# mateomarin/two_towers

Hardware: AMD Instinct MI355X
Metric: training pairs/sec at global batch=8192, 1/2/4/8 GPUs; MRR@10 match (higher is better)
Workload: dtype bf16; 1 GPU; BASELINE configs[2]: EnhancedTwoTowerModel(300, 256), seq_len 64, batch 8192 per GPU, bf16, hard-negative mining k=5 + margin 0.2, dropout 0.1, Adam; global_batch=8192, seq_len=64, hidden=256, embedding_dim=300, parallelism=dp1, loss=hardneg_margin

## Files before the change

include/tt_hip.h:

```cpp
#ifndef TT_HIP_H
#define TT_HIP_H
#include <stdint.h>

#ifdef __cplusplus
extern "C" {
#endif

#define TT_OK 0
#define TT_EINVAL 1000
#define TT_DT_F32 0
#define TT_DT_BF16 1

const char* tt_version(void);
const char* tt_last_error(void);
int tt_set_option(const char* name, int value);
int tt_get_option(const char* name, int* value);

int tt_embed_gather(int dtype, const void* table, long vocab, int ep, const int32_t* ids, long n,
                    void* out, void* stream);

int tt_pack_rows(int dtype, const float* src, long n, int e, int ep, void* out, void* stream);
typedef struct {
  const float* src;
  const float* src2;
  void* dst;
  int rows, cols, dcols;
  long lds, ldd;
  int dst_bf16;
} tt_pack_job;
int tt_pack_multi(const tt_pack_job* jobs, int njobs, void* stream);

int tt_cast(int dtype, const float* x, long n, void* y, void* stream);

int tt_colsum(const float* x, long rows, int cols, long ld, float* out, int accumulate, void* stream);

typedef struct {
  const void* a[4];
  const void* b[4];
  void* c[4];
  const float* bias[4];
  int bshift[4];
  const void* a_hi[4];
  int a_split;
  uint32_t drop_row0;
} tt_gemm_batch;

int tt_gemm(int dtype, int out_dtype, int a_kouter, int b_kouter, int m, int n, int k,
            const tt_gemm_batch* batch, int nbatch, long lda, long ldb, long ldc, float alpha,
            int beta_accum, int relu, int seq_t, uint32_t drop_seed, float drop_p, int splits,
            float* splitk_ws, void* stream);
int tt_gemm_ct(int dtype, int out_dtype, int a_kouter, int b_kouter, int m, int n, int k,
               const tt_gemm_batch* batch, int nbatch, long lda, long ldb, long ldc, float alpha,
               int beta_accum, int relu, int seq_t, uint32_t drop_seed, float drop_p, int splits,
               float* splitk_ws, int c_trans, void* stream);
long tt_gemm_ws_size(int m, int n, int nbatch, int splits);
int tt_gemm_pick_splits(int m, int n, int k, int nbatch);
int tt_gemm_bres_form(int m, int n, int k, int nbatch, long lda, long ldc);
int tt_gemm_tall_form(int dtype, int out_dtype, int a_kouter, int b_kouter, int m, int n, int k, long lda,
                      long ldb, int splits, int extras);

typedef struct {
  const void* g;
  const void* whh;
  const float* bhn;
  void* y;
  void* x1;
  void* save;
  float* hstate;
  int dir;
  uint32_t drop_seed;
  int drop_col0;
  uint32_t drop_row0;
} tt_gru_fwd_rec;

int tt_gru_fwd(int dtype, const tt_gru_fwd_rec* recs, int nrec, int B, int T, int H, long ldg,
               long ldy, float drop_p, void* ws, long ws_bytes, void* stream);
int tt_gru_fwd_launches(int dtype, int T, int H);
long tt_gru_fwd_ws_size(int dtype, int nrec, int B, int T, int H, long ldg, long ldy);
int tt_gru_fwd_launches_for(int dtype, int nrec, int B, int T, int H, long ldg, long ldy);

typedef struct {
  const void* g; const void* whh; const float* bhn;
  void* y;
  void* hfinal;
  void* scratch;
  int dir;
} tt_gru_infer_rec;
int  tt_gru_fwd_infer(int dtype, const tt_gru_infer_rec* recs, int nrec, int B, int T, int H, long ldg,
                      long ldy, long ldf, void* ws, long ws_bytes, void* stream);
long tt_gru_infer_scratch_size(int dtype, int B, int T, int H, int final_only);

typedef struct {
  const void* save;
  const void* y;
  const void* dy;
  const float* dfinal;
  const void* whh;
  void* dgx;
  void* dgh;
  void* dhstate;
  float* dbias_part;
  int dir;
} tt_gru_bwd_rec;

int tt_gru_bwd(int dtype, const tt_gru_bwd_rec* recs, int nrec, int B, int T, int H, long ldy,
               long ldd, long ldf, void* stream);
int tt_gru_bwd_launches(int dtype, int T, int H);
int tt_gru_bwd_carry_on_chip(int dtype, int T, int H);
int tt_gru_bias_rows(int B);

int tt_gru_yprev_supported(int dtype, int nrec, int B, int T, int H, long ldg, long ldy);
int tt_gru_fwd_yprev(int dtype, const tt_gru_fwd_rec* recs, void* const* hfinal, int nrec, int B, int T, int H,
                     long ldg, long ldy, long ldf, float drop_p, void* ws, long ws_bytes, void* stream);
int tt_gru_bwd_yprev(int dtype, const tt_gru_bwd_rec* recs, int nrec, int B, int T, int H, long ldy,
                     long ldd, long ldf, void* stream);

typedef struct {
  const void* w1; const float* b1; const float* ln_g; const float* ln_b;
  const void* w2; const float* b2;
  const void* x;
  void* p1;
  float* mean;
  float* rstd;
  void* u;
  float* out;
} tt_head_fwd_io;

int tt_proj_head_fwd(int dtype, const tt_head_fwd_io* io, int ntower, int B, int h, float ln_eps,
                     void* stream);

typedef struct {
  const void* w1; const float* ln_g; const float* ln_b; const void* w2;
  const void* x; const void* p1; const float* mean; const float* rstd; const void* u;
  const float* dout;
  float* dx;
  float* dw1; float* db1; float* dg; float* dbeta; float* dw2; float* db2;
  void* ws;
} tt_head_bwd_io;

int tt_proj_head_bwd(int dtype, const tt_head_bwd_io* io, int ntower, int B, int h, float ln_eps,
                     void* stream);
long tt_proj_head_bwd_ws_size(int dtype, int B, int h);

typedef struct {
  const void* x;
  const void* w1; const float* b1; const float* ln_g; const float* ln_b;
  void* p1;
  float* mean;
  float* rstd;
  float* out;
} tt_head1_fwd_io;

int tt_proj_head1_fwd(int dtype, const tt_head1_fwd_io* io, long rows, int C, float ln_eps, float drop_p,
                      uint32_t drop_seed, void* stream);

typedef struct {
  const void* x; const void* w1; const float* ln_g; const float* ln_b;
  const void* p1; const float* mean; const float* rstd;
  const float* dout;
  float* dx;
  float* dw1; float* db1; float* dg; float* dbeta;
  void* ws;
} tt_head1_bwd_io;

int tt_proj_head1_bwd(int dtype, const tt_head1_bwd_io* io, long rows, int C, float drop_p, uint32_t drop_seed,
                      void* stream);
long tt_proj_head1_bwd_ws_size(int dtype, long rows, int C);

int tt_l2norm_fwd(int dtype, const float* x, long rows, int cols, float eps, void* y, float* y32,
                  float* norm, void* stream);
int tt_l2norm_bwd(const float* dy, const float* y32, const float* norm, long rows, int cols,
                  float eps, float* dx, int accumulate, void* stream);

int tt_infonce_fwd(int dtype, const void* qn, long bq, const void* dn, long nd, int h,
                   float inv_tau, float offdiag_sub, long label_offset, float* lse,
                   float* row_loss, void* ws, void* stream);
long tt_infonce_fwd_ws_size(long bq, long nd);
int tt_infonce_bwd(int dtype, const void* qn, long bq, const void* dn, long nd, int h,
                   float inv_tau, float offdiag_sub, long label_offset, const float* lse,
                   const float* gscale, float* dqn, float* ddn, void* ws, void* stream);
long tt_infonce_bwd_ws_size(int dtype, long bq, long nd, int h);

int tt_infonce_sym_fwd(int dtype, const void* qn, const void* dn, long n, int h, float inv_tau,
                       float* lse_row, float* lse_col, float* row_loss, void* ws, void* stream);
long tt_infonce_sym_fwd_ws_size(long n, int h);
int tt_infonce_sym_bwd(int dtype, const void* qn, const void* dn, long n, int h, float inv_tau,
                       const float* lse_row, const float* lse_col, const float* gscale,
                       float* dqn, float* ddn, void* ws, void* stream);
long tt_infonce_sym_bwd_ws_size(int dtype, long n, int h);

int tt_hardneg_topk(int dtype, const void* qn, long bq, const void* dn, long nd, int h,
                    long label_offset, int k, int32_t* idx, float* val, void* ws, void* stream);
long tt_hardneg_ws_size(int dtype, long bq, long nd, int h, int k);

int tt_search_topk(int dtype, const float* qn, long Q, const void* dn, long N, int h, int k,
                   int32_t* idx, float* val, void* ws, void* stream);
long tt_search_ws_size(int dtype, long Q, long N, int h, int k);

int tt_topk_max(void);
int tt_topk_rows(const float* S, long rows, long cols, long ld, long label_offset, int k,
                 int32_t* idx, float* val, void* ws, void* stream);
long tt_topk_rows_ws_size(long rows, long cols, int k);

int tt_margin_fwd(const float* qn, long bq, const float* dn, long nd, int h, long label_offset,
                  const int32_t* idx, int k, float margin, float* row_loss, void* stream);
int tt_margin_bwd(const float* qn, long bq, const float* dn, long nd, int h, long label_offset,
                  const int32_t* idx, int k, float margin, const float* gscale, float* dqn, float* ddn,
                  void* ws, void* stream);
long tt_margin_bwd_ws_size(long bq, long nd, int h, int k);

int tt_sum(const float* x, long n, float scale, float* out, void* stream);

int tt_adam_multi(float* const* params, const float* const* grads, float* const* exp_avg,
                  float* const* exp_avg_sq, const long* sizes, int ntensors, float lr, float beta1,
                  float beta2, float eps, float weight_decay, int step, const int32_t* skip, void* stream);
int tt_adamw_multi(float* const* params, const float* const* grads, float* const* exp_avg,
                   float* const* exp_avg_sq, const long* sizes, int ntensors, float lr, float beta1,
                   float beta2, float eps, float weight_decay, int step, const int32_t* skip, void* stream);

int tt_grad_norm_multi(const float* const* grads, const long* sizes, int ntensors, int accumulate,
                       float* sumsq, void* ws, void* stream);
long tt_grad_norm_ws_size(const long* sizes, int ntensors);
int tt_clip_scale_multi(float* const* grads, const long* sizes, int ntensors, const float* sumsq,
                        float max_norm, float* total_norm_out, void* stream);

#ifdef __cplusplus
}
#endif
#endif
```

two_towers_amd/_lib.py:

```python
from __future__ import annotations

import contextlib
import ctypes
import os
from ctypes import POINTER, c_float, c_int, c_long, c_uint32, c_void_p

import torch

_HERE = os.path.dirname(os.path.abspath(__file__))
LIB_PATH = os.environ.get("TT_HIP_LIB", os.path.join(_HERE, "lib", "libtt_hip.so"))

DT_F32 = 0
DT_BF16 = 1
TT_EINVAL = 1000


class TTError(RuntimeError):
    pass


class GruTimeoutError(TTError):
    """A column-split GRU forward launch gave up waiting for one of its member workgroups
    (tt_gru_fwd's status word): that launch's outputs are invalid."""


class GemmBatch(ctypes.Structure):
    _fields_ = [
        ("a", c_void_p * 4),
        ("b", c_void_p * 4),
        ("c", c_void_p * 4),
        ("bias", c_void_p * 4),
        ("bshift", c_int * 4),
        ("a_hi", c_void_p * 4),
        ("a_split", c_int),
        ("drop_row0", c_uint32),
    ]


class PackJob(ctypes.Structure):
    _fields_ = [
        ("src", c_void_p),
        ("src2", c_void_p),
        ("dst", c_void_p),
        ("rows", c_int),
        ("cols", c_int),
        ("dcols", c_int),
        ("lds", c_long),
        ("ldd", c_long),
        ("dst_bf16", c_int),
    ]


class GruFwdRec(ctypes.Structure):
    _fields_ = [
        ("g", c_void_p), ("whh", c_void_p), ("bhn", c_void_p), ("y", c_void_p), ("x1", c_void_p),
        ("save", c_void_p), ("hstate", c_void_p), ("dir", c_int), ("drop_seed", c_uint32),
        ("drop_col0", c_int), ("drop_row0", c_uint32),
    ]


class GruInferRec(ctypes.Structure):
    _fields_ = [
        ("g", c_void_p), ("whh", c_void_p), ("bhn", c_void_p), ("y", c_void_p), ("hfinal", c_void_p),
        ("scratch", c_void_p), ("dir", c_int),
    ]


class GruBwdRec(ctypes.Structure):
    _fields_ = [
        ("save", c_void_p), ("y", c_void_p), ("dy", c_void_p), ("dfinal", c_void_p), ("whh", c_void_p),
        ("dgx", c_void_p), ("dgh", c_void_p), ("dhstate", c_void_p), ("dbias_part", c_void_p),
        ("dir", c_int),
    ]


class HeadFwdIO(ctypes.Structure):
    _fields_ = [
        ("w1", c_void_p), ("b1", c_void_p), ("ln_g", c_void_p), ("ln_b", c_void_p), ("w2", c_void_p),
        ("b2", c_void_p), ("x", c_void_p), ("p1", c_void_p), ("mean", c_void_p), ("rstd", c_void_p),
        ("u", c_void_p), ("out", c_void_p),
    ]


class HeadBwdIO(ctypes.Structure):
    _fields_ = [
        ("w1", c_void_p), ("ln_g", c_void_p), ("ln_b", c_void_p), ("w2", c_void_p), ("x", c_void_p),
        ("p1", c_void_p), ("mean", c_void_p), ("rstd", c_void_p), ("u", c_void_p), ("dout", c_void_p),
        ("dx", c_void_p), ("dw1", c_void_p), ("db1", c_void_p), ("dg", c_void_p), ("dbeta", c_void_p),
        ("dw2", c_void_p), ("db2", c_void_p), ("ws", c_void_p),
    ]


class Head1FwdIO(ctypes.Structure):
    _fields_ = [
        ("x", c_void_p), ("w1", c_void_p), ("b1", c_void_p), ("ln_g", c_void_p), ("ln_b", c_void_p),
        ("p1", c_void_p), ("mean", c_void_p), ("rstd", c_void_p), ("out", c_void_p),
    ]


class Head1BwdIO(ctypes.Structure):
    _fields_ = [
        ("x", c_void_p), ("w1", c_void_p), ("ln_g", c_void_p), ("ln_b", c_void_p), ("p1", c_void_p),
        ("mean", c_void_p), ("rstd", c_void_p), ("dout", c_void_p), ("dx", c_void_p), ("dw1", c_void_p),
        ("db1", c_void_p), ("dg", c_void_p), ("dbeta", c_void_p), ("ws", c_void_p),
    ]


_SIGS = {
    "tt_version": (ctypes.c_char_p, []),
    "tt_last_error": (ctypes.c_char_p, []),
    "tt_set_option": (c_int, [ctypes.c_char_p, c_int]),
    "tt_get_option": (c_int, [ctypes.c_char_p, POINTER(c_int)]),
    "tt_embed_gather": (c_int, [c_int, c_void_p, c_long, c_int, c_void_p, c_long, c_void_p, c_void_p]),
    "tt_pack_rows": (c_int, [c_int, c_void_p, c_long, c_int, c_int, c_void_p, c_void_p]),
    "tt_pack_multi": (c_int, [c_void_p, c_int, c_void_p]),
    "tt_cast": (c_int, [c_int, c_void_p, c_long, c_void_p, c_void_p]),
    "tt_colsum": (c_int, [c_void_p, c_long, c_int, c_long, c_void_p, c_int, c_void_p]),
    "tt_gemm": (c_int, [c_int, c_int, c_int, c_int, c_int, c_int, c_int, POINTER(GemmBatch), c_int, c_long,
                        c_long, c_long, c_float, c_int, c_int, c_int, c_uint32, c_float, c_int, c_void_p,
                        c_void_p]),
    "tt_gemm_ct": (c_int, [c_int, c_int, c_int, c_int, c_int, c_int, c_int, POINTER(GemmBatch), c_int, c_long,
                           c_long, c_long, c_float, c_int, c_int, c_int, c_uint32, c_float, c_int, c_void_p,
                           c_int, c_void_p]),
    "tt_gemm_ws_size": (c_long, [c_int, c_int, c_int, c_int]),
    "tt_gemm_pick_splits": (c_int, [c_int, c_int, c_int, c_int]),
    "tt_gemm_bres_form": (c_int, [c_int, c_int, c_int, c_int, c_long, c_long]),
    "tt_gemm_tall_form": (c_int, [c_int, c_int, c_int, c_int, c_int, c_int, c_int, c_long, c_long, c_int, c_int]),
    "tt_gru_fwd": (c_int, [c_int, POINTER(GruFwdRec), c_int, c_int, c_int, c_int, c_long, c_long, c_float,
                           c_void_p, c_long, c_void_p]),
    "tt_gru_bwd": (c_int, [c_int, POINTER(GruBwdRec), c_int, c_int, c_int, c_int, c_long, c_long, c_long,
                           c_void_p]),
    "tt_gru_bias_rows": (c_int, [c_int]),
    "tt_gru_bwd_launches": (c_int, [c_int, c_int, c_int]),
    "tt_gru_bwd_carry_on_chip": (c_int, [c_int, c_int, c_int]),
    "tt_gru_fwd_launches": (c_int, [c_int, c_int, c_int]),
    "tt_gru_fwd_ws_size": (c_long, [c_int, c_int, c_int, c_int, c_int, c_long, c_long]),
    "tt_gru_fwd_launches_for": (c_int, [c_int, c_int, c_int, c_int, c_int, c_long, c_long]),
    "tt_gru_fwd_infer": (c_int, [c_int, POINTER(GruInferRec), c_int, c_int, c_int, c_int, c_long, c_long, c_long,
                                 c_void_p, c_long, c_void_p]),
    "tt_gru_infer_scratch_size": (c_long, [c_int, c_int, c_int, c_int, c_int]),
    "tt_gru_yprev_supported": (c_int, [c_int, c_int, c_int, c_int, c_int, c_long, c_long]),
    "tt_gru_fwd_yprev": (c_int, [c_int, POINTER(GruFwdRec), POINTER(c_void_p), c_int, c_int, c_int, c_int, c_long,
                                 c_long, c_long, c_float, c_void_p, c_long, c_void_p]),
    "tt_gru_bwd_yprev": (c_int, [c_int, POINTER(GruBwdRec), c_int, c_int, c_int, c_int, c_long, c_long, c_long,
                                 c_void_p]),
    "tt_proj_head_fwd": (c_int, [c_int, POINTER(HeadFwdIO), c_int, c_int, c_int, c_float, c_void_p]),
    "tt_proj_head_bwd": (c_int, [c_int, POINTER(HeadBwdIO), c_int, c_int, c_int, c_float, c_void_p]),
    "tt_proj_head_bwd_ws_size": (c_long, [c_int, c_int, c_int]),
    "tt_proj_head1_fwd": (c_int, [c_int, POINTER(Head1FwdIO), c_long, c_int, c_float, c_float, c_uint32,
                                  c_void_p]),
    "tt_proj_head1_bwd": (c_int, [c_int, POINTER(Head1BwdIO), c_long, c_int, c_float, c_uint32, c_void_p]),
    "tt_proj_head1_bwd_ws_size": (c_long, [c_int, c_long, c_int]),
    "tt_l2norm_fwd": (c_int, [c_int, c_void_p, c_long, c_int, c_float, c_void_p, c_void_p, c_void_p, c_void_p]),
    "tt_l2norm_bwd": (c_int, [c_void_p, c_void_p, c_void_p, c_long, c_int, c_float, c_void_p, c_int, c_void_p]),
    "tt_infonce_fwd": (c_int, [c_int, c_void_p, c_long, c_void_p, c_long, c_int, c_float, c_float, c_long,
                               c_void_p, c_void_p, c_void_p, c_void_p]),
    "tt_infonce_fwd_ws_size": (c_long, [c_long, c_long]),
    "tt_infonce_bwd": (c_int, [c_int, c_void_p, c_long, c_void_p, c_long, c_int, c_float, c_float, c_long,
                               c_void_p, c_void_p, c_void_p, c_void_p, c_void_p, c_void_p]),
    "tt_infonce_bwd_ws_size": (c_long, [c_int, c_long, c_long, c_int]),
    "tt_infonce_sym_fwd": (c_int, [c_int, c_void_p, c_void_p, c_long, c_int, c_float, c_void_p, c_void_p, c_void_p,
                                   c_void_p, c_void_p]),
    "tt_infonce_sym_fwd_ws_size": (c_long, [c_long, c_int]),
    "tt_infonce_sym_bwd": (c_int, [c_int, c_void_p, c_void_p, c_long, c_int, c_float, c_void_p, c_void_p, c_void_p,
                                   c_void_p, c_void_p, c_void_p, c_void_p]),
    "tt_infonce_sym_bwd_ws_size": (c_long, [c_int, c_long, c_int]),
    "tt_hardneg_topk": (c_int, [c_int, c_void_p, c_long, c_void_p, c_long, c_int, c_long, c_int, c_void_p,
                                c_void_p, c_void_p, c_void_p]),
    "tt_hardneg_ws_size": (c_long, [c_int, c_long, c_long, c_int, c_int]),
    "tt_search_topk": (c_int, [c_int, c_void_p, c_long, c_void_p, c_long, c_int, c_int, c_void_p, c_void_p,
                               c_void_p, c_void_p]),
    "tt_search_ws_size": (c_long, [c_int, c_long, c_long, c_int, c_int]),
    "tt_topk_max": (c_int, []),
    "tt_topk_rows": (c_int, [c_void_p, c_long, c_long, c_long, c_long, c_int, c_void_p, c_void_p, c_void_p,
                             c_void_p]),
    "tt_topk_rows_ws_size": (c_long, [c_long, c_long, c_int]),
    "tt_margin_fwd": (c_int, [c_void_p, c_long, c_void_p, c_long, c_int, c_long, c_void_p, c_int, c_float,
                              c_void_p, c_void_p]),
    "tt_margin_bwd": (c_int, [c_void_p, c_long, c_void_p, c_long, c_int, c_long, c_void_p, c_int, c_float,
                              c_void_p, c_void_p, c_void_p, c_void_p, c_void_p]),
    "tt_margin_bwd_ws_size": (c_long, [c_long, c_long, c_int, c_int]),
    "tt_sum": (c_int, [c_void_p, c_long, c_float, c_void_p, c_void_p]),
    "tt_adam_multi": (c_int, [POINTER(c_void_p), POINTER(c_void_p), POINTER(c_void_p), POINTER(c_void_p),
                              POINTER(c_long), c_int, c_float, c_float, c_float, c_float, c_float, c_int,
                              c_void_p, c_void_p]),
    "tt_adamw_multi": (c_int, [POINTER(c_void_p), POINTER(c_void_p), POINTER(c_void_p), POINTER(c_void_p),
                               POINTER(c_long), c_int, c_float, c_float, c_float, c_float, c_float, c_int,
                               c_void_p, c_void_p]),
    "tt_grad_norm_multi": (c_int, [POINTER(c_void_p), POINTER(c_long), c_int, c_int, c_void_p, c_void_p, c_void_p]),
    "tt_grad_norm_ws_size": (c_long, [POINTER(c_long), c_int]),
    "tt_clip_scale_multi": (c_int, [POINTER(c_void_p), POINTER(c_long), c_int, c_void_p, c_float, c_void_p,
                                    c_void_p]),
}

EXPORTED = tuple(_SIGS)

_lib = None
_load_error: str | None = None


def load():
    global _lib, _load_error
    if _lib is not None:
        return _lib
    if _load_error is not None:
        raise TTError(_load_error)
    if not os.path.exists(LIB_PATH):
        _load_error = (f"two_towers_amd: native library not found at {LIB_PATH}; "
                       "build it with `python -c 'import __graft_entry__ as g; g.build()'` (hipcc, gfx950)")
        raise TTError(_load_error)
    lib = ctypes.CDLL(LIB_PATH, mode=ctypes.RTLD_GLOBAL)
    for name, (res, args) in _SIGS.items():
        fn = getattr(lib, name)
        fn.restype = res
        fn.argtypes = args
    _lib = lib
    return lib


def check(rc: int, what: str = ""):
    if rc != 0:
        msg = _lib.tt_last_error().decode(errors="replace") if _lib is not None else ""
        raise TTError(f"{what or 'tt_hip'} failed (rc={rc}): {msg}")


def call(name: str, *args):
    lib = load()
    check(getattr(lib, name)(*args), name)


_topk_max: int | None = None


def topk_max() -> int:
    global _topk_max
    if _topk_max is None:
        _topk_max = int(load().tt_topk_max())
    return _topk_max


def get_option(name: str) -> int:
    v = c_int(0)
    call("tt_get_option", name.encode(), ctypes.byref(v))
    return v.value


def set_option(name: str, value: int) -> int:
    old = get_option(name)
    call("tt_set_option", name.encode(), int(value))
    return old


@contextlib.contextmanager
def option(name: str, value: int):
    torch.cuda.synchronize()
    old = set_option(name, value)
    try:
        yield
    finally:
        torch.cuda.synchronize()
        set_option(name, old)


def ptr(t: torch.Tensor | None) -> int | None:
    if t is None:
        return None
    return t.data_ptr()


def stream_ptr(device: torch.device | None = None) -> int:
    return torch.cuda.current_stream(device).cuda_stream


def require_gpu(*tensors: torch.Tensor):
    load()
    for t in tensors:
        if t is not None and t.device.type != "cuda":
            raise TTError(
                "two_towers_amd runs only on an AMD GPU (HIP, gfx950); got a tensor on "
                f"'{t.device}'. There is deliberately no CPU fallback: move the model and "
                "inputs to the GPU (`.to('cuda')`).")


def dtype_code(dt: torch.dtype) -> int:
    if dt == torch.float32:
        return DT_F32
    if dt == torch.bfloat16:
        return DT_BF16
    raise TTError(f"unsupported compute dtype {dt}; use torch.float32 or torch.bfloat16")
```

two_towers_amd/csrc/tt_api.h:

```cpp
#pragma once
#include <hip/hip_runtime.h>
#include <stdio.h>
#include <string.h>

#include "../../include/tt_hip.h"

namespace tt {
void set_error(const char* fmt, ...);

enum Opt {
  OPT_GRU_STEP,
  OPT_GRU_DEPTH,
  OPT_GRU_BWD_ROWS,
  OPT_GRU_BWD_BIG,
  OPT_GRU_BWD_STREAMS,
  OPT_GEMM_PERSIST,
  OPT_GEMM_A3,
  OPT_GEMM_REGSTAGE,
  OPT_GEMM_STREAM_OUT,
  OPT_HN_GEMM,
  OPT_GRU_BWD_PERSIST,
  OPT_GRU_FWD_STEP_ROWS,
  OPT_INFONCE_FLASH,
  OPT_HN_MAP,
  OPT_GEMM_SKEW,
  OPT_GEMM_PERSIST_MAXK,
  OPT_GRU_FWD_XC,
  OPT_GRU_XC_SKIP,
  OPT_GRU_XC_SPINS,
  OPT_GRU_BWD_SKEW,
  OPT_GRU_FWD_SKEW,
  OPT_GEMM_BRES,
  OPT_GRU_XC_COOP,
  OPT_GEMM_BUF,
  OPT_GEMM_ORDER,
  OPT_GRU_STEP_RING,
  OPT_GRU_FWD_XS,
  OPT_HN_SCAN_GEMM,
  OPT_GEMM_IEPI,
  OPT_BRES_ROWS,
  OPT_HN_SCAN_V,
  OPT_GEMM_W4,
  OPT_BRES_FORM,
  OPT_WGRAD_TALL,
  OPT_GRU_YPREV,
  OPT_N
};
int opt(Opt o);
int tt_hn_scan_gemm(const void* q, long bq, const void* d, long nd, int h, long label_off, float* cm, long nch,
                    hipStream_t st);
}

#define TT_CHECK_ARG(cond, ...)            \
  do {                                     \
    if (!(cond)) {                         \
      tt::set_error(__VA_ARGS__);          \
      return TT_EINVAL;                    \
    }                                      \
  } while (0)

#define TT_CHECK_LAUNCH(what)                                                        \
  do {                                                                               \
    hipError_t e_ = hipGetLastError();                                               \
    if (e_ != hipSuccess) {                                                          \
      tt::set_error("%s: %s", what, hipGetErrorString(e_));                          \
      return (int)e_;                                                                \
    }                                                                                \
  } while (0)

#define TT_CHECK_HIP(expr)                                                           \
  do {                                                                               \
    hipError_t e_ = (expr);                                                          \
    if (e_ != hipSuccess) {                                                          \
      tt::set_error("%s: %s", #expr, hipGetErrorString(e_));                         \
      return (int)e_;                                                                \
    }                                                                                \
  } while (0)

#define TT_PROPAGATE(expr)     \
  do {                         \
    int rc_ = (expr);          \
    if (rc_ != 0) return rc_;  \
  } while (0)

static inline int tt_ceil_div(long a, long b) { return (int)((a + b - 1) / b); }
```

two_towers_amd/csrc/tt_common.h:

```cpp
#pragma once
#include <hip/hip_runtime.h>
#include <stdint.h>

#define TT_F32 0
#define TT_BF16 1

typedef uint16_t bf16_t;
typedef short bf16x8 __attribute__((ext_vector_type(8)));
typedef short bf16x4 __attribute__((ext_vector_type(4)));
typedef float f32x4 __attribute__((ext_vector_type(4)));

#define TT_DEV __device__ __forceinline__

TT_DEV float bf2f(bf16_t b) { return __uint_as_float(((uint32_t)b) << 16); }
TT_DEV bf16_t f2bf(float f) { __bf16 h = (__bf16)f; return __builtin_bit_cast(bf16_t, h); }

template <typename T> struct Elt;
template <> struct Elt<float> {
  static constexpr int EPC = 4;
  TT_DEV static float ld(const float* p) { return *p; }
  TT_DEV static void st(float* p, float v) { *p = v; }
  TT_DEV static float cvt(float v) { return v; }
};
template <> struct Elt<bf16_t> {
// ... 2 lines not shown
  TT_DEV static void st(bf16_t* p, float v) { *p = f2bf(v); }
  TT_DEV static bf16_t cvt(float v) { return f2bf(v); }
};

TT_DEV void ld8(const float* p, float (&f)[8]) {
  const float4 a = *reinterpret_cast<const float4*>(p), b = *reinterpret_cast<const float4*>(p + 4);
  f[0] = a.x; f[1] = a.y; f[2] = a.z; f[3] = a.w; f[4] = b.x; f[5] = b.y; f[6] = b.z; f[7] = b.w;
}
TT_DEV void ld8(const bf16_t* p, float (&f)[8]) {
  const uint4 u = *reinterpret_cast<const uint4*>(p);
  const uint32_t w[4] = {u.x, u.y, u.z, u.w};
#pragma unroll
  for (int i = 0; i < 4; ++i) {
    f[2 * i] = __uint_as_float(w[i] << 16);
    f[2 * i + 1] = __uint_as_float(w[i] & 0xFFFF0000u);
  }
}
TT_DEV void st8(float* p, const float (&f)[8]) {
  *reinterpret_cast<float4*>(p) = make_float4(f[0], f[1], f[2], f[3]);
  *reinterpret_cast<float4*>(p + 4) = make_float4(f[4], f[5], f[6], f[7]);
}
TT_DEV void st8(bf16_t* p, const float (&f)[8]) {
  uint32_t w[4];
#pragma unroll
  for (int i = 0; i < 4; ++i) w[i] = (uint32_t)f2bf(f[2 * i]) | ((uint32_t)f2bf(f[2 * i + 1]) << 16);
  *reinterpret_cast<uint4*>(p) = make_uint4(w[0], w[1], w[2], w[3]);
}

typedef unsigned tt_u32x4 __attribute__((vector_size(16)));
TT_DEV __amdgpu_buffer_rsrc_t tt_rsrc(const void* base) {
  return __builtin_amdgcn_make_buffer_rsrc(const_cast<void*>(base), (short)0, 0x7fffffff, 0x00020000);
}
TT_DEV uint4 pack8bf(const float (&f)[8]) {
  uint32_t w[4];
#pragma unroll
  for (int i = 0; i < 4; ++i) w[i] = (uint32_t)f2bf(f[2 * i]) | ((uint32_t)f2bf(f[2 * i + 1]) << 16);
  return make_uint4(w[0], w[1], w[2], w[3]);
}
TT_DEV void st16_buf(__amdgpu_buffer_rsrc_t r, uint32_t voff, int soff, uint4 v) {
  tt_u32x4 w = {v.x, v.y, v.z, v.w};
  __builtin_amdgcn_raw_buffer_store_b128(w, r, (int)(voff + (uint32_t)soff), 0, 0);
}
TT_DEV void st16_buf_sc1(__amdgpu_buffer_rsrc_t r, uint32_t voff, int soff, uint4 v) {
  tt_u32x4 w = {v.x, v.y, v.z, v.w};
  __builtin_amdgcn_raw_buffer_store_b128(w, r, (int)(voff + (uint32_t)soff), 0, 16);
}
TT_DEV __amdgpu_buffer_rsrc_t tt_rsrc_n(const void* base, bool on) {
  return __builtin_amdgcn_make_buffer_rsrc(const_cast<void*>(base), (short)0, on ? 0x7fffffff : 0, 0x00020000);
}
template <int AUX = 0>
TT_DEV uint4 ld16_buf(__amdgpu_buffer_rsrc_t r, uint32_t voff, int soff) {
  const tt_u32x4 v = __builtin_amdgcn_raw_buffer_load_b128(r, (int)voff, soff, AUX);
  return make_uint4(v[0], v[1], v[2], v[3]);
}
template <int AUX>
TT_DEV void st16_buf_aux(__amdgpu_buffer_rsrc_t r, int off, uint4 v) {
  tt_u32x4 w = {v.x, v.y, v.z, v.w};
  __builtin_amdgcn_raw_buffer_store_b128(w, r, off, 0, AUX);
}
TT_DEV void st16_sc1(__amdgpu_buffer_rsrc_t r, int off, uint4 v) {
  tt_u32x4 w = {v.x, v.y, v.z, v.w};
  __builtin_amdgcn_raw_buffer_store_b128(w, r, off, 0, 16);
}
TT_DEV void st8_sc1(__amdgpu_buffer_rsrc_t r, int off, const float (&f)[8], float*) {
  st16_sc1(r, off, make_uint4(__float_as_uint(f[0]), __float_as_uint(f[1]), __float_as_uint(f[2]), __float_as_uint(f[3])));
  st16_sc1(r, off + 16, make_uint4(__float_as_uint(f[4]), __float_as_uint(f[5]), __float_as_uint(f[6]), __float_as_uint(f[7])));
}
TT_DEV void st8_sc1(__amdgpu_buffer_rsrc_t r, int off, const float (&f)[8], bf16_t*) {
  uint32_t w[4];
#pragma unroll
  for (int i = 0; i < 4; ++i) w[i] = (uint32_t)f2bf(f[2 * i]) | ((uint32_t)f2bf(f[2 * i + 1]) << 16);
  st16_sc1(r, off, make_uint4(w[0], w[1], w[2], w[3]));
}

TT_DEV uint32_t dpp_ror8(uint32_t x) {
  return (uint32_t)__builtin_amdgcn_mov_dpp((int)x, 0x128 , 0xF, 0xF, false);
}
TT_DEV void row_pair(const uint4& v0, const uint4& v1, uint4& da, uint4& db) {
  const bool lo = (threadIdx.x & 8) == 0;
  uint4 s = lo ? v1 : v0, r;
  r.x = dpp_ror8(s.x);
  r.y = dpp_ror8(s.y);
  r.z = dpp_ror8(s.z);
  r.w = dpp_ror8(s.w);
  da = lo ? v0 : r;
  db = lo ? r : v1;
}

template <typename T>
struct Raw8 {
  uint4 a, b;
  TT_DEV void load(const T* p) {
    a = *reinterpret_cast<const uint4*>(p);
    if constexpr (sizeof(T) == 4) b = *reinterpret_cast<const uint4*>(p + 4);
  }
  TT_DEV void zero() { a = b = make_uint4(0, 0, 0, 0); }
  TT_DEV void get(float (&f)[8]) const {
    if constexpr (sizeof(T) == 4) {
      f[0] = __uint_as_float(a.x); f[1] = __uint_as_float(a.y); f[2] = __uint_as_float(a.z); f[3] = __uint_as_float(a.w);
      f[4] = __uint_as_float(b.x); f[5] = __uint_as_float(b.y); f[6] = __uint_as_float(b.z); f[7] = __uint_as_float(b.w);
    } else {
      const uint32_t w[4] = {a.x, a.y, a.z, a.w};
#pragma unroll
      for (int i = 0; i < 4; ++i) {
        f[2 * i] = __uint_as_float(w[i] << 16);
        f[2 * i + 1] = __uint_as_float(w[i] & 0xFFFF0000u);
      }
    }
  }
};

TT_DEV float tt_rcp(float x) { return __builtin_amdgcn_rcpf(x); }
TT_DEV float tt_sigmoid(float x) { return tt_rcp(1.0f + __expf(-x)); }
TT_DEV float tt_tanh(float x) {
  float e = __expf(2.0f * x);
  return 1.0f - 2.0f * tt_rcp(e + 1.0f);
}

TT_DEV float tt_sech2(float x) {
  const float e = __expf(-2.0f * fabsf(x));
  const float r = tt_rcp(1.0f + e);
  return 4.0f * e * r * r;
}

TT_DEV void tt_sigmoid_pair(float x, float& s, float& sm) {
  const float e = __expf(-fabsf(x));
  const float p = tt_rcp(1.0f + e);
  const float q = e * p;
  s = x >= 0.f ? p : q;
  sm = x >= 0.f ? q : p;
}
TT_DEV void tt_tanh_sech2(float x, float& th, float& sech2) {
  const float e = __expf(-2.0f * fabsf(x));
  const float r = tt_rcp(1.0f + e);
  const float t = (1.0f - e) * r;
  th = x >= 0.f ? t : -t;
  sech2 = 4.0f * e * r * r;
}

TT_DEV uint32_t tt_hash3(uint32_t seed, uint32_t row, uint32_t col) {
  uint32_t h = seed * 0x9E3779B1u ^ (row * 0x85EBCA77u) ^ (col * 0xC2B2AE3Du + 0x27D4EB2Fu);
  h ^= h >> 16; h *= 0x7FEB352Du; h ^= h >> 15; h *= 0x846CA68Bu; h ^= h >> 16;
  return h;
}
TT_DEV float tt_dropout_scale(uint32_t seed, uint32_t row, uint32_t col, uint32_t thresh, float inv_keep) {
  return ((tt_hash3(seed, row, col) >> 8) < thresh) ? 0.0f : inv_keep;
}

TT_DEV float wave_sum(float v) {
#pragma unroll
  for (int o = 32; o > 0; o >>= 1) v += __shfl_xor(v, o, 64);
  return v;
}
TT_DEV float wave_max(float v) {
#pragma unroll
  for (int o = 32; o > 0; o >>= 1) v = fmaxf(v, __shfl_xor(v, o, 64));
  return v;
}
TT_DEV float sum16(float v) {
#pragma unroll
  for (int o = 8; o > 0; o >>= 1) v += __shfl_xor(v, o, 64);
  return v;
}
TT_DEV float max16(float v) {
#pragma unroll
  for (int o = 8; o > 0; o >>= 1) v = fmaxf(v, __shfl_xor(v, o, 64));
  return v;
}
```

two_towers_amd/csrc/tt_elem.hip:

```cpp
#include <algorithm>

#include "tt_api.h"
#include "tt_common.h"

namespace {

__global__ __launch_bounds__(256) void embed_gather_kernel(const uint4* __restrict__ table, long vocab,
                                                           int cpr, const int32_t* __restrict__ ids,
                                                           long n, uint4* __restrict__ out) {
  const long total = n * cpr;
  for (long e = (long)blockIdx.x * 256 + threadIdx.x; e < total; e += (long)gridDim.x * 256) {
    const long row = e / cpr;
    const int c = (int)(e - row * cpr);
    const int id = ids[row];
    uint4 v = make_uint4(0, 0, 0, 0);
    if (id >= 0 && id < vocab) v = table[(long)id * cpr + c];
    out[e] = v;
  }
}

template <typename T>
__global__ __launch_bounds__(256) void pack_rows_kernel(const float* __restrict__ src, long n, int e, int ep,
                                                        T* __restrict__ out) {
  const long total = n * ep;
  for (long i = (long)blockIdx.x * 256 + threadIdx.x; i < total; i += (long)gridDim.x * 256) {
    const long r = i / ep;
    const int c = (int)(i - r * ep);
    Elt<T>::st(out + i, c < e ? src[r * e + c] : 0.f);
  }
}

template <typename T>
__global__ __launch_bounds__(256) void cast_kernel(const float* __restrict__ x, long n, T* __restrict__ y) {
  for (long i = (long)blockIdx.x * 256 + threadIdx.x; i < n; i += (long)gridDim.x * 256) Elt<T>::st(y + i, x[i]);
}

__global__ __launch_bounds__(1024) void colsum_kernel(const float* __restrict__ x, long rows, int cols, long ld,
                                                      int accumulate, float* __restrict__ out) {
  __shared__ float red[16][64];
  const int wave = threadIdx.x >> 6, lane = threadIdx.x & 63;
  const int c = blockIdx.x * 64 + lane;
  float s = 0.f;
  if (c < cols)
    for (long r = wave; r < rows; r += 16) s += x[r * ld + c];
  red[wave][lane] = s;
  __syncthreads();
  if (wave == 0 && c < cols) {
    float t = 0.f;
#pragma unroll
    for (int w = 0; w < 16; ++w) t += red[w][lane];
    out[c] = accumulate ? out[c] + t : t;
  }
}

__global__ __launch_bounds__(256) void sum_kernel(const float* __restrict__ x, long n, float scale,
                                                  float* __restrict__ out) {
  __shared__ float part[4];
  float s = 0.f;
  for (long i = threadIdx.x; i < n; i += 256) s += x[i];
  s = wave_sum(s);
  if ((threadIdx.x & 63) == 0) part[threadIdx.x >> 6] = s;
  __syncthreads();
  if (threadIdx.x == 0) out[0] = scale * (part[0] + part[1] + part[2] + part[3]);
}

struct PackArgs {
  tt_pack_job j[16];
  long start[17];
  int n;
};
__global__ __launch_bounds__(256) void pack_multi_kernel(PackArgs a) {
  const long total = a.start[a.n];
  for (long i = blockIdx.x * 256L + threadIdx.x; i < total; i += (long)gridDim.x * 256) {
    int k = 0;
    while (k + 1 < a.n && i >= a.start[k + 1]) ++k;
    const tt_pack_job& J = a.j[k];
    const long q = i - a.start[k];
    const int g4 = J.dcols / 4;
    const long r = q / g4;
    const int c = (int)(q - r * g4) * 4;
    float4 v = make_float4(0.f, 0.f, 0.f, 0.f);
    if (c < J.cols) {
      v = *reinterpret_cast<const float4*>(J.src + r * J.lds + c);
      if (J.src2) {
        const float4 w = *reinterpret_cast<const float4*>(J.src2 + r * J.lds + c);
        v.x += w.x; v.y += w.y; v.z += w.z; v.w += w.w;
      }
    }
    if (J.dst_bf16) {
      const uint2 o = make_uint2((uint32_t)f2bf(v.x) | ((uint32_t)f2bf(v.y) << 16),
                                 (uint32_t)f2bf(v.z) | ((uint32_t)f2bf(v.w) << 16));
      *reinterpret_cast<uint2*>(static_cast<bf16_t*>(J.dst) + r * J.ldd + c) = o;
    } else {
      *reinterpret_cast<float4*>(static_cast<float*>(J.dst) + r * J.ldd + c) = v;
    }
  }
}

inline unsigned grid_for(long work, int per_block = 256, int cap = 8192) {
  long g = (work + per_block - 1) / per_block;
  if (g < 1) g = 1;
  return (unsigned)std::min<long>(g, cap);
}

}

extern "C" int tt_embed_gather(int dtype, const void* table, long vocab, int ep, const int32_t* ids, long n,
                               void* out, void* stream) {
  TT_CHECK_ARG(dtype == TT_DT_F32 || dtype == TT_DT_BF16, "tt_embed_gather: bad dtype");
  const int esz = dtype == TT_DT_BF16 ? 2 : 4;
  TT_CHECK_ARG((ep * esz) % 16 == 0, "tt_embed_gather: ep*sizeof(dtype) must be a multiple of 16 (ep=%d)", ep);
  if (n == 0) return 0;
  const int cpr = ep * esz / 16;
  hipLaunchKernelGGL(embed_gather_kernel, dim3(grid_for(n * cpr)), dim3(256), 0, (hipStream_t)stream,
                     (const uint4*)table, vocab, cpr, ids, n, (uint4*)out);
  TT_CHECK_LAUNCH("embed_gather_kernel");
  return 0;
}

extern "C" int tt_pack_rows(int dtype, const float* src, long n, int e, int ep, void* out, void* stream) {
  TT_CHECK_ARG(ep >= e, "tt_pack_rows: ep < e");
  if (n == 0) return 0;
  dim3 g(grid_for(n * ep));
  if (dtype == TT_DT_BF16)
    hipLaunchKernelGGL(pack_rows_kernel<bf16_t>, g, dim3(256), 0, (hipStream_t)stream, src, n, e, ep, (bf16_t*)out);
  else
    hipLaunchKernelGGL(pack_rows_kernel<float>, g, dim3(256), 0, (hipStream_t)stream, src, n, e, ep, (float*)out);
  TT_CHECK_LAUNCH("pack_rows_kernel");
  return 0;
}

extern "C" int tt_pack_multi(const tt_pack_job* jobs, int njobs, void* stream) {
  TT_CHECK_ARG(njobs >= 0 && njobs <= 16 && (njobs == 0 || jobs), "tt_pack_multi: njobs %d not in [0,16]", njobs);
  PackArgs a{};
  a.n = njobs;
  a.start[0] = 0;
  for (int k = 0; k < njobs; ++k) {
    const tt_pack_job& J = jobs[k];
    TT_CHECK_ARG(J.src && J.dst && J.rows >= 0 && J.cols >= 0 && J.dcols >= J.cols, "tt_pack_multi: job %d", k);
    TT_CHECK_ARG(J.cols % 4 == 0 && J.dcols % 4 == 0 && J.lds % 4 == 0 && J.ldd % 4 == 0 && J.lds >= J.cols &&
                     J.ldd >= J.dcols,
                 "tt_pack_multi: job %d: cols, dcols and leading dimensions must be multiples of 4", k);
    const bool src_ok = ((uintptr_t)J.src | (uintptr_t)J.src2) % 16 == 0;
    TT_CHECK_ARG(src_ok && (uintptr_t)J.dst % (J.dst_bf16 ? 8 : 16) == 0, "tt_pack_multi: job %d: misaligned operand", k);
    a.j[k] = J;
    a.start[k + 1] = a.start[k] + (long)J.rows * (J.dcols / 4);
  }
  if (a.start[njobs] == 0) return 0;
  hipLaunchKernelGGL(pack_multi_kernel, dim3(grid_for(a.start[njobs], 256, 4096)), dim3(256), 0, (hipStream_t)stream, a);
  TT_CHECK_LAUNCH("pack_multi_kernel");
  return 0;
}

extern "C" int tt_cast(int dtype, const float* x, long n, void* y, void* stream) {
  if (n == 0) return 0;
  dim3 g(grid_for(n));
  if (dtype == TT_DT_BF16)
    hipLaunchKernelGGL(cast_kernel<bf16_t>, g, dim3(256), 0, (hipStream_t)stream, x, n, (bf16_t*)y);
  else
    hipLaunchKernelGGL(cast_kernel<float>, g, dim3(256), 0, (hipStream_t)stream, x, n, (float*)y);
  TT_CHECK_LAUNCH("cast_kernel");
  return 0;
}

extern "C" int tt_colsum(const float* x, long rows, int cols, long ld, float* out, int accumulate, void* stream) {
  hipStream_t st = (hipStream_t)stream;
  if (cols == 0) return 0;
  if (rows == 0) {
    if (!accumulate) TT_CHECK_HIP(hipMemsetAsync(out, 0, sizeof(float) * cols, st));
    return 0;
  }
  hipLaunchKernelGGL(colsum_kernel, dim3(tt_ceil_div(cols, 64)), dim3(1024), 0, st, x, rows, cols, ld, accumulate,
                     out);
  TT_CHECK_LAUNCH("colsum_kernel");
  return 0;
}

extern "C" int tt_sum(const float* x, long n, float scale, float* out, void* stream) {
  hipLaunchKernelGGL(sum_kernel, dim3(1), dim3(256), 0, (hipStream_t)stream, x, n, scale, out);
  TT_CHECK_LAUNCH("sum_kernel");
  return 0;
}
```

two_towers_amd/csrc/tt_gemm.hip:

```cpp
#include <float.h>
#include <stdarg.h>
#include <stdlib.h>

#include <atomic>
#include <type_traits>

#include "tt_api.h"
#include "tt_gemm_core.h"

namespace tt {
static thread_local char g_err[512];
void set_error(const char* fmt, ...) {
  va_list ap;
  va_start(ap, fmt);
  vsnprintf(g_err, sizeof(g_err), fmt, ap);
  va_end(ap);
}
}

namespace tt {
namespace {
struct OptDef {
  const char* name;
  const char* env;
  int dflt;
};
constexpr OptDef kOpts[OPT_N] = {
    {"gru_step", "TT_GRU_STEP", 0},               {"gru_depth", "TT_GRU_DEPTH", 4},
    {"gru_bwd_rows", "TT_GRU_BWD_ROWS", 0},     {"gru_bwd_big", "TT_GRU_BWD_BIG", 1},
    {"gru_bwd_streams", "TT_GRU_BWD_STREAMS", 2}, {"gemm_persist", "TT_GEMM_PERSIST", 1},
    {"gemm_a3", "TT_GEMM_A3", 1},                 {"gemm_regstage", "TT_GEMM_REGSTAGE", 0},
    {"gemm_stream_out", "TT_GEMM_STREAM_OUT", 1}, {"hn_gemm", "TT_HN_GEMM", 0},
    {"gru_bwd_persist", "TT_GRU_BWD_PERSIST", 1}, {"gru_fwd_step_rows", "TT_GRU_FWD_STEP_ROWS", 0},
    {"infonce_flash", "TT_INFONCE_FLASH", 1},     {"hn_map", "TT_HN_MAP", 2},
    {"gemm_skew", "TT_GEMM_SKEW", 0},             {"gemm_persist_maxk", "TT_GEMM_PERSIST_MAXK", 24},
    {"gru_fwd_xc", "TT_GRU_FWD_XC", 1},           {"gru_xc_skip", "TT_GRU_XC_SKIP", 0},
    {"gru_xc_spins", "TT_GRU_XC_SPINS", 22},      {"gru_bwd_skew", "TT_GRU_BWD_SKEW", 14},
    {"gru_fwd_skew", "TT_GRU_FWD_SKEW", 0},       {"gemm_bres", "TT_GEMM_BRES", 1},
    {"gru_xc_coop", "TT_GRU_XC_COOP", 0},         {"gemm_buf", "TT_GEMM_BUF", 1},
    {"gemm_order", "TT_GEMM_ORDER", 0},           {"gru_step_ring", "TT_GRU_STEP_RING", 4},
    {"gru_fwd_xs", "TT_GRU_FWD_XS", 1},           {"hn_scan_gemm", "TT_HN_SCAN_GEMM", 0},
    {"gemm_iepi", "TT_GEMM_IEPI", 1},             {"bres_rows", "TT_BRES_ROWS", 32},
    {"hn_scan_v", "TT_HN_SCAN_V", 5},             {"gemm_w4", "TT_GEMM_W4", 0},
    {"bres_form", "TT_BRES_FORM", 1},             {"wgrad_tall", "TT_WGRAD_TALL", 1},
    {"gru_yprev", "TT_GRU_YPREV", 1},
};
struct OptTable {
  std::atomic<int> v[OPT_N];
  OptTable() {
    for (int i = 0; i < OPT_N; ++i) {
      const char* e = getenv(kOpts[i].env);
      v[i].store(e && *e ? atoi(e) : kOpts[i].dflt, std::memory_order_relaxed);
    }
  }
};
OptTable& opts() {
  static OptTable t;
  return t;
}
int find_opt(const char* name) {
  for (int i = 0; name && i < OPT_N; ++i)
    if (strcmp(name, kOpts[i].name) == 0) return i;
  return -1;
}
}
int opt(Opt o) { return opts().v[o].load(std::memory_order_relaxed); }
}

extern "C" const char* tt_version(void) { return "tt_hip 0.2.0 gfx950"; }
extern "C" const char* tt_last_error(void) { return tt::g_err; }
extern "C" int tt_set_option(const char* name, int value) {
  const int i = tt::find_opt(name);
  TT_CHECK_ARG(i >= 0, "tt_set_option: unknown option '%s'", name ? name : "(null)");
  tt::opts().v[i].store(value, std::memory_order_relaxed);
  return 0;
}
extern "C" int tt_get_option(const char* name, int* value) {
  const int i = tt::find_opt(name);
  TT_CHECK_ARG(i >= 0 && value, "tt_get_option: unknown option '%s'", name ? name : "(null)");
  *value = tt::opt((tt::Opt)i);
  return 0;
}

namespace {

struct GemmArgs {
  const void* a[4];
  const void* b[4];
  void* c[4];
  const float* bias[4];
  int bshift[4];
  const void* a_hi[4];
  int a_split;
  long lda, ldb, ldc;
  int M, N, K;
  int splits, kt_per_split;
  float alpha;
  int beta, relu, seq_t;
  uint32_t drop_seed, drop_thresh, drop_row0;
  float drop_inv_keep;
  long part_stride;
  int vec_ok;
  int force_regstage;
  int skew;
  int bias_vec_ok;
  int stream_out;
  int walk_g, walk_x;
  int nbatch;
  int c_trans;
  float* cm;
  long nch, label_off;
};

constexpr int BM = 128, BN = 128;

#ifndef TT_TAIL_SKIP
#define TT_TAIL_SKIP 1
#endif
using ttg::xcd_remap;
#ifndef PERSIST_IEPI
#define PERSIST_IEPI 1
#endif
#ifndef PERSIST_BAL
#define PERSIST_BAL 1
#endif
#ifndef TT_EPI_PAIR
#define TT_EPI_PAIR 1
#endif
#ifndef TT_GEMM_BAL
#define TT_GEMM_BAL true
#endif

template <typename T, bool AKO, bool BKO, bool SHIFT, typename TO, int TBM, int TBN, int WGM, int WGN, bool DMA,
          bool A3 = false, bool BUF = false>
__global__ __launch_bounds__(64 * WGM * WGN) void gemm_kernel(GemmArgs g) {
  using ML = std::conditional_t<
      DMA,
      std::conditional_t<TBM == 256 && TBN == 256 && WGM == 2 && WGN == 4,
                         ttg::Loop8<T, AKO, BKO, TT_GEMM_BAL, A3, false, BUF>,
                         ttg::DLoop<T, AKO, BKO, TBM, TBN, WGM, WGN>>,
      ttg::MainLoop<T, AKO, BKO, TBM, TBN>>;
  static_assert(DMA || (TBM == 128 && TBN == 128 && WGM == 2 && WGN == 2), "register path is 128x128");
  constexpr int NT = 64 * WGM * WGN;
  constexpr int LDSB = ML::LDS_BYTES > 64 * (TBN + 4) * 4 ? ML::LDS_BYTES : 64 * (TBN + 4) * 4;
  __shared__ __attribute__((aligned(16))) char lds[LDSB];
  const int ntn = (g.N + TBN - 1) / TBN, ntm = (g.M + TBM - 1) / TBM;
  const int id = xcd_remap(blockIdx.x, gridDim.x);
  const int bs = id / (ntm * ntn), tile = id - bs * (ntm * ntn);
  const int mt = tile / ntn, nt = tile - mt * ntn;
  const int bi = bs / g.splits, s = bs - bi * g.splits;
  const int m0 = mt * TBM, n0 = nt * TBN;
  const T* A = static_cast<const T*>(g.a[bi]);
  const T* B = static_cast<const T*>(g.b[bi]);

  f32x4 acc[ML::TM][ML::TN];
#pragma unroll
  for (int i = 0; i < ML::TM; ++i)
#pragma unroll
    for (int j = 0; j < ML::TN; ++j) acc[i][j] = f32x4{0.f, 0.f, 0.f, 0.f};

  const int nk = (g.K * (int)sizeof(T) + ttg::KTB - 1) / ttg::KTB;
  const int kt0 = s * g.kt_per_split;
  const int kt1 = min(nk, kt0 + g.kt_per_split);

  constexpr bool L8T = DMA && TBM == 256 && TBN == 256 && WGM == 2 && WGN == 4;
  const bool mm = !L8T || !TT_TAIL_SKIP || __builtin_amdgcn_readfirstlane((int)(m0 + (int)(threadIdx.x >> 8) * 128 < g.M));
  auto lrun = [&](const auto& la, const auto& lb) {
    if constexpr (L8T) ML::run(la, lb, g.K, kt0, kt1, lds, acc, mm);
    else ML::run(la, lb, g.K, kt0, kt1, lds, acc);
  };
  auto run = [&](const auto& la) {
    if constexpr (!BKO) {
      lrun(la, ttg::KCPlain<T>{B, g.ldb, n0, g.N});
    } else if constexpr (SHIFT) {
      lrun(la, ttg::KOShift<T>{B, g.ldb, n0, g.N - n0, g.seq_t, g.bshift[bi]});
    } else {
      lrun(la, ttg::KOPlain<T>{B, g.ldb, n0, g.N - n0});
    }
  };
  if constexpr (AKO) {
    ttg::KOPlain<T> la{A, g.lda, m0, g.M - m0};
    if (g.a_split > 0) {
      la.base1 = static_cast<const T*>(g.a_hi[bi]);
      la.csplit = g.a_split;
    }
    run(la);
  } else {
    run(ttg::KCPlain<T>{A, g.lda, m0, g.M});
  }

#ifdef TT_DIAG
  if (g.force_regstage == 9) {
    float sum = 0.f;
#pragma unroll
    for (int i = 0; i < ML::TM; ++i)
#pragma unroll
      for (int j = 0; j < ML::TN; ++j) sum += acc[i][j][0] + acc[i][j][3];
    if (sum == 12345.f) static_cast<float*>(g.c[bi])[0] = 1.f;
    return;
  }
#endif
  const bool partial = g.splits > 1;
  TO* C = partial ? nullptr : static_cast<TO*>(g.c[bi]);
  float* P = partial ? static_cast<float*>(g.c[bi]) + (long)s * g.part_stride : nullptr;
  const long ldc = partial ? (long)g.N : g.ldc;
  const float* bias = partial ? nullptr : g.bias[bi];
  const int wave = threadIdx.x >> 6, lane = threadIdx.x & 63, tid = threadIdx.x;
  constexpr int WTM = TBM / WGM, WTN = TBN / WGN;
  const int wm = wave / WGN * WTM, wn = wave % WGN * WTN;
  constexpr int CLD = TBN + 4;
  constexpr int TPR = TBN / 8;
  constexpr int RPP = NT / TPR;
  float* L = reinterpret_cast<float*>(lds);
  const int cg = (tid % TPR) * 8;
  const __amdgpu_buffer_rsrc_t crs = tt_rsrc(partial ? (const void*)P : (const void*)(C + (long)m0 * ldc + n0));
  float bv[8];
#pragma unroll
  for (int e = 0; e < 8; ++e) bv[e] = 0.f;
  if (bias) {
    if (n0 + cg + 8 <= g.N && g.bias_vec_ok) ld8(bias + n0 + cg, bv);
    else
      for (int e = 0; e < 8; ++e)
        if (n0 + cg + e < g.N) bv[e] = bias[n0 + cg + e];
  }
  for (int hf = 0; hf < TBM / 64; ++hf) {
    if (wm <= hf * 64 && hf * 64 < wm + WTM) {
      const int i0 = (hf * 64 - wm) / 16;
#pragma unroll
      for (int i = 0; i < ML::TM; ++i)
        if (i >= i0 && i < i0 + 4)
#pragma unroll
          for (int j = 0; j < ML::TN; ++j)
#pragma unroll
            for (int r = 0; r < 4; ++r)
              L[(16 * (i - i0) + 4 * (lane >> 4) + r) * CLD + wn + 16 * j + (lane & 15)] = acc[i][j][r];
    }
    __syncthreads();
#pragma unroll
    for (int k = 0; k < 64 / RPP; ++k) {
      const int rl = tid / TPR + RPP * k;
      const int gm = m0 + hf * 64 + rl, gn = n0 + cg;
      if (gm < g.M && gn < g.N) {
        float v[8];
#pragma unroll
        for (int e = 0; e < 8; ++e) v[e] = L[rl * CLD + cg + e];
        const bool full = gn + 8 <= g.N && g.vec_ok;
        if (partial) {
          float* dst = P + (long)gm * ldc + gn;
          if (full) st8(dst, v);
          else
            for (int e = 0; e < 8 && gn + e < g.N; ++e) dst[e] = v[e];
        } else {
#pragma unroll
          for (int e = 0; e < 8; ++e) {
            float x = v[e] * g.alpha + bv[e];
            if (g.relu) x = fmaxf(x, 0.f);
            if (g.drop_thresh) x *= tt_dropout_scale(g.drop_seed, g.drop_row0 + (uint32_t)gm, gn + e, g.drop_thresh, g.drop_inv_keep);
            v[e] = x;
          }
          TO* dst = C + (long)gm * ldc + gn;
          if (full) {
            if (g.beta) {
// ... 877 lines not shown
      iepi(C1{}, C1{});
      iepi(C1{}, C0{});
    }
  }
  if constexpr (A3)
    if (!late) __builtin_amdgcn_s_barrier();
  asm volatile("s_waitcnt vmcnt(0)" ::: "memory");
}

namespace tall {
constexpr int AW = 8192, AN = 4096;
constexpr int BOFF = 2 * AW + AN;
constexpr int SLOT = BOFF + 2 * AW;
constexpr int NS = 4;
constexpr int NDMA = SLOT / 1024;
constexpr int KS = 32;
}

template <bool HALF>
__global__ __launch_bounds__(512) void gemm_tall(GemmArgs g, int u0) {
  using namespace tall;
  constexpr int NA = HALF ? 5 : 10;
  __shared__ __attribute__((aligned(16))) char lds[NS * SLOT];
  const int ntn = (g.N + 255) / 256;
  const int id = xcd_remap(blockIdx.x, gridDim.x);
  const int hf = HALF ? id & 1 : 0;
  const int u = u0 + (HALF ? id >> 1 : id);
  const int bs = u / ntn, nt = u - bs * ntn;
  const int bi = bs / g.splits, s = bs - bi * g.splits;
  const int n0 = nt * 256;
  const bf16_t* A = static_cast<const bf16_t*>(g.a[bi]);
  const bf16_t* B = static_cast<const bf16_t*>(g.b[bi]);
  const int wave = __builtin_amdgcn_readfirstlane(threadIdx.x >> 6), lane = threadIdx.x & 63;
  const int wr = wave >> 2, wn = (wave & 3) * 64;
  auto a_sub = [&](int a) { return HALF ? a >> 1 : a / 5; };
  auto a_col = [&](int a) {
    if (HALF) return a == 4 ? 32 * hf + 16 * wr : 64 * hf + 32 * wr + 16 * (a & 1);
    return a % 5 == 4 ? 32 * wr + 16 * (a / 5) : 64 * wr + 16 * (a % 5);
  };

  f32x4 acc[NA][4];
#pragma unroll
  for (int i = 0; i < NA; ++i)
#pragma unroll
    for (int j = 0; j < 4; ++j) acc[i][j] = f32x4{0.f, 0.f, 0.f, 0.f};

  const int nk = (g.K * 2 + ttg::KTB - 1) / ttg::KTB;
  const int kt0 = s * g.kt_per_split;
  const int kt1 = min(nk, kt0 + g.kt_per_split);
  if (kt0 < kt1) {
    const int nst = 2 * (kt1 - kt0);
    const long k0 = (long)kt0 * 64;
    const long krows = min((long)g.K, (long)kt1 * 64) - k0;
    const ttg::tt_rsrc4 ra = ttg::make_rsrc4(A + k0 * g.lda, (uint32_t)(((krows - 1) * g.lda + g.M) * 2));
    const ttg::tt_rsrc4 rb = ttg::make_rsrc4(B + k0 * g.ldb, (uint32_t)(((krows - 1) * g.ldb + g.N) * 2));
    const uint32_t da = (uint32_t)(KS * g.lda * 2), db = (uint32_t)(KS * g.ldb * 2);
    uint32_t voff[5];
#pragma unroll
    for (int t = 0; t < 5; ++t) {
      const int j = wave + 8 * t;
      long e;
      if (j < 16) {
        const int p = (j & 7) * 64 + lane, kl = p >> 4, c = (p & 15) ^ (ttg::ko_v(kl) << 1);
        e = (long)kl * g.lda + (j >> 3) * 128 + c * 8;
      } else if (j < 20) {
        const int p = (j - 16) * 64 + lane, kl = p >> 3, c = (p & 7) ^ (ttg::kon_v(kl) << 1);
        e = (long)kl * g.lda + 256 + c * 8;
      } else {
        const int b = j - 20, p = (b & 7) * 64 + lane, kl = p >> 4, c = (p & 15) ^ (ttg::ko_v(kl) << 1);
        e = (long)kl * g.ldb + n0 + (b >> 3) * 128 + c * 8;
      }
      voff[t] = (uint32_t)(e * 2);
    }
    const uint32_t base = __builtin_amdgcn_readfirstlane(ttg::lds_addr_of(lds));
    const bool a2 = wave < 4;
    ttg::tt_rsrc4 r2;
    r2.x = a2 ? ra.x : rb.x;
    r2.y = a2 ? ra.y : rb.y;
    r2.z = a2 ? ra.z : rb.z;
    r2.w = ra.w;
    const uint32_t d2 = a2 ? da : db;
    auto issue = [&](int st) {
      const uint32_t sl = base + (uint32_t)(st & (NS - 1)) * SLOT + (uint32_t)wave * 1024u;
      const uint32_t sa = (uint32_t)st * da, sb = (uint32_t)st * db;
      ttg::dma16_buf(ra, voff[0] + sa, 0u, sl);
      ttg::dma16_buf(ra, voff[1] + sa, 0u, sl + 8 * 1024u);
      ttg::dma16_buf(r2, voff[2] + (uint32_t)st * d2, 0u, sl + 16 * 1024u);
      ttg::dma16_buf(rb, voff[3] + sb, 0u, sl + 24 * 1024u);
      if (a2) ttg::dma16_buf(rb, voff[4] + sb, 0u, sl + 32 * 1024u);
    };
    auto step = [&](const char* sl) {
      uint4 fb[4];
#pragma unroll
      for (int j = 0; j < 4; ++j) fb[j] = ttg::frag<bf16_t, true>(sl + BOFF + (wn >> 7) * AW, (wn & 127) + 16 * j, 0);
#pragma unroll
      for (int h = 0; h < NA / 5; ++h) {
        uint4 fa[5];
#pragma unroll
        for (int i = 0; i < 4; ++i) fa[i] = ttg::frag<bf16_t, true>(sl + a_sub(5 * h + i) * AW, a_col(5 * h + i), 0);
        fa[4] = ttg::frag_ko16n(sl + 2 * AW, a_col(5 * h + 4));
#pragma unroll
        for (int i = 0; i < 5; ++i)
#pragma unroll
          for (int j = 0; j < 4; ++j) acc[5 * h + i][j] = ttg::mma<bf16_t>(fb[j], fa[i], acc[5 * h + i][j]);
        __builtin_amdgcn_sched_barrier(0);
      }
    };
    issue(0);
    issue(1);
    issue(2);
    for (int st = 0; st < nst; ++st) {
      if (wave < 4) asm volatile("s_waitcnt vmcnt(10)" ::: "memory");
      else asm volatile("s_waitcnt vmcnt(8)" ::: "memory");
      __builtin_amdgcn_s_barrier();
      issue(st + 3);
      const char* sl = lds + (st & (NS - 1)) * SLOT;
      step(sl);
    }
    asm volatile("s_waitcnt vmcnt(0)" ::: "memory");
  }

  const bool partial = g.splits > 1;
  float* C = partial ? static_cast<float*>(g.c[bi]) + (long)s * g.part_stride : static_cast<float*>(g.c[bi]);
  const long ldc = partial ? (long)g.N : g.ldc;
  const int q = lane >> 4, lr = lane & 15;
#pragma unroll
  for (int i = 0; i < NA; ++i) {
    const int gm = (i % 5 < 4 ? 128 * a_sub(i) : 256) + a_col(i) + lr;
#pragma unroll
    for (int j = 0; j < 4; ++j) {
      const int c = n0 + wn + 16 * j + 4 * q;
      if (gm >= g.M || c >= g.N) continue;
      float v[4];
#pragma unroll
      for (int e = 0; e < 4; ++e) v[e] = partial ? acc[i][j][e] : acc[i][j][e] * g.alpha + 0.f;
      float* dst = C + (long)gm * ldc + c;
      if (c + 4 <= g.N && g.vec_ok) *reinterpret_cast<float4*>(dst) = make_float4(v[0], v[1], v[2], v[3]);
      else
        for (int e = 0; e < 4 && c + e < g.N; ++e) dst[e] = v[e];
    }
  }
}

template <typename TO, int V>
__global__ __launch_bounds__(256) void splitk_reduce_kernel(const float* ws, long part_stride, int splits,
                                                            int M, int N, GemmArgs g) {
  const int bi = blockIdx.y;
  const float* P = ws + (long)bi * splits * part_stride;
  TO* C = static_cast<TO*>(g.c[bi]);
  const float* bias = g.bias[bi];
  const long total = (long)M * N / V;
  for (long e = (long)blockIdx.x * 256 + threadIdx.x; e < total; e += (long)gridDim.x * 256) {
    float v[V];
    if constexpr (V == 4) {
      float4 a = make_float4(0.f, 0.f, 0.f, 0.f);
      for (int s = 0; s < splits; ++s) {
        const float4 b = reinterpret_cast<const float4*>(P + (long)s * part_stride)[e];
        a.x += b.x;
        a.y += b.y;
        a.z += b.z;
        a.w += b.w;
      }
      v[0] = a.x, v[1] = a.y, v[2] = a.z, v[3] = a.w;
    } else {
      v[0] = 0.f;
      for (int s = 0; s < splits; ++s) v[0] += P[(long)s * part_stride + e];
    }
    const int m = (int)(e * V / N), n0 = (int)(e * V % N);
#pragma unroll
    for (int u = 0; u < V; ++u) {
      float x = v[u] * g.alpha;
      if (bias) x += bias[n0 + u];
      TO* p = g.c_trans ? C + (long)(n0 + u) * g.ldc + m : C + (long)m * g.ldc + n0 + u;
      if (g.beta) x += Elt<TO>::ld(p);
      Elt<TO>::st(p, x);
    }
  }
}

template <typename T, typename TO, int TBM, int TBN, int WGM, int WGN, bool DMA, bool A3 = false, bool BUF = false>
int launch_t(int akout, int bkout, bool shift, const GemmArgs& g, long nwg, hipStream_t st) {
  dim3 grid((unsigned)nwg), blk(64 * WGM * WGN);
#define TT_L(AK, BK, SH) \
  hipLaunchKernelGGL((gemm_kernel<T, AK, BK, SH, TO, TBM, TBN, WGM, WGN, DMA, A3, BUF>), grid, blk, 0, st, g)
  if (!akout && !bkout) TT_L(false, false, false);
  else if (!akout && bkout && !shift) TT_L(false, true, false);
  else if (!akout && bkout && shift) TT_L(false, true, true);
  else if (akout && !bkout) TT_L(true, false, false);
  else if (akout && bkout && !shift) TT_L(true, true, false);
  else TT_L(true, true, true);
#undef TT_L
  TT_CHECK_LAUNCH("gemm_kernel");
  return 0;
}

inline bool use_big(int m, int n, long tiles256) { return m >= 256 && n >= 256 && tiles256 >= 256; }

template <typename T, typename TO>
int launch_persist(int akout, int bkout, bool shift, const GemmArgs& g0, int ntiles, bool buf, hipStream_t st) {
  dim3 grid((unsigned)std::min(ntiles, 256)), blk(512);
  GemmArgs g = g0;
  g.walk_g = g.walk_x = 0;
  if (tt::opt(tt::OPT_GEMM_ORDER) && ntiles % 256 == 0 && ((g.N + 255) / 256) % 4 == 0) {
    g.walk_g = 4;
    g.walk_x = 8;
  }
#define TT_L(AK, BK, SH, A3, BUF) \
  hipLaunchKernelGGL((gemm_persist<T, AK, BK, SH, TO, A3, BUF>), grid, blk, 0, st, g, ntiles)
#define TT_L2(AK, BK, SH) \
  do {                     \
    if (a3 && buf) TT_L(AK, BK, SH, true, true); \
    else if (a3) TT_L(AK, BK, SH, true, false); \
    else TT_L(AK, BK, SH, false, false);   \
  } while (0)
  const bool a3 = tt::opt(tt::OPT_GEMM_A3) != 0;
  if constexpr (std::is_same<TO, bf16_t>::value) {
    if (PERSIST_IEPI && tt::opt(tt::OPT_GEMM_IEPI) && !akout && !bkout && !shift && a3 && buf && g.M % 256 == 0 &&
        g.N % 256 == 0 && g.vec_ok && g.bias_vec_ok && g.alpha == 1.f && !g.relu && !g.drop_thresh && !g.beta &&
        g.stream_out <= 2 && g.force_regstage == 0) {
      hipLaunchKernelGGL((gemm_persist<T, false, false, false, TO, true, true, false, true>), grid, blk, 0, st, g, ntiles);
      TT_CHECK_LAUNCH("gemm_persist");
      return 0;
    }
  }
  if (!akout && !bkout) TT_L2(false, false, false);
  else if (!akout && bkout && !shift) TT_L2(false, true, false);
  else if (!akout && bkout && shift) TT_L2(false, true, true);
  else if (akout && !bkout) TT_L2(true, false, false);
  else if (akout && bkout && !shift) TT_L2(true, true, false);
  else TT_L2(true, true, true);
#undef TT_L2
#undef TT_L
  TT_CHECK_LAUNCH("gemm_persist");
  return 0;
}

#ifndef W4_LEAD
#define W4_LEAD 2
#endif
namespace w4 {
constexpr int SLOT = 32768;
constexpr int NS = 4;
struct Frags {
  uint4 a[8], b[8];
};
TT_DEV uint4 frag(const char* img, int r0) {
  const int lane = threadIdx.x & 63;
  const int row = r0 + (lane & 15);
  return *reinterpret_cast<const uint4*>(img + row * 64 + (((lane >> 4) ^ ((row >> 1) & 3)) << 4));
}
}

template <bool RS>
__global__ __launch_bounds__(256, 1) void gemm_w4(GemmArgs g, int ntm, int ntn) {
  constexpr int NSL = RS ? 3 : w4::NS;
  __shared__ __attribute__((aligned(16))) char lds[NSL * w4::SLOT];
  const int id = ttg::xcd_remap(blockIdx.x, gridDim.x);
  const int per = ntm * ntn;
  const int bi = id / per, tile = id - bi * per;
  const int mt = tile / ntn, nt = tile - mt * ntn;
  const int m0 = mt * 256, n0 = nt * 256;
  const int wave = __builtin_amdgcn_readfirstlane(threadIdx.x >> 6), lane = threadIdx.x & 63;
  const int wr = wave >> 1, wc = wave & 1;
  const bf16_t* A = static_cast<const bf16_t*>(g.a[bi]);
  const bf16_t* B = static_cast<const bf16_t*>(g.b[bi]);
  const uint32_t base = __builtin_amdgcn_readfirstlane(ttg::lds_addr_of(lds));
  const bool isA = wave < 2;
  const long ld = isA ? g.lda : g.ldb;
  const long r0 = isA ? m0 : n0;
  const long rows_left = (isA ? g.M : g.N) - r0;
  const long nrec = rows_left * ld * 2;
  const uint32_t nrec32 = (uint32_t)(nrec > 0xFFFFFFFFL ? 0xFFFFFFFFL : nrec);
  const ttg::tt_rsrc4 rs = ttg::make_rsrc4((isA ? A : B) + r0 * ld, nrec32);
  const __amdgpu_buffer_rsrc_t rsb = __builtin_amdgcn_make_buffer_rsrc(
      const_cast<bf16_t*>((isA ? A : B) + r0 * ld), (short)0, (int)(nrec32 > 0x7fffffffu ? 0x7fffffffu : nrec32), 0x00020000);
  const int prow = 16 * (wave & 1) * 8 + (lane >> 2);
  const uint32_t voff = (uint32_t)(prow * ld * 2 + (((lane & 3) ^ ((lane >> 3) & 3)) << 4));
  const uint32_t pstep = (uint32_t)(16 * ld * 2);
  const uint32_t pbase = (uint32_t)wave * 8u * 1024u;
  auto dma = [&](int kt, int j) {
    ttg::dma16_buf(rs, voff, (uint32_t)kt * 64u + (uint32_t)j * pstep,
                   base + (uint32_t)(kt % NSL) * w4::SLOT + pbase + (uint32_t)j * 1024u);
  };
  auto gload = [&](int kt, int j) { return ld16_buf(rsb, voff, (int)((uint32_t)kt * 64u + (uint32_t)j * pstep)); };
  auto lput = [&](int kt, int j, const uint4& v) {
    *reinterpret_cast<uint4*>(lds + (kt % NSL) * w4::SLOT + pbase + j * 1024 + lane * 16) = v;
  };
  const int nk = g.K / 32;
  f32x4 acc[8][8];
#pragma unroll
  for (int i = 0; i < 8; ++i)
#pragma unroll
    for (int j = 0; j < 8; ++j) acc[i][j] = f32x4{0.f, 0.f, 0.f, 0.f};
  if constexpr (RS) {
    uint4 S0[8], S1[8];
#pragma unroll
    for (int j = 0; j < 8; ++j) S0[j] = gload(0, j);
#pragma unroll
    for (int j = 0; j < 8; ++j) S1[j] = gload(1, j);
#pragma unroll
    for (int j = 0; j < 8; ++j) lput(0, j, S0[j]);
#pragma unroll
    for (int j = 0; j < 8; ++j) lput(1, j, S1[j]);
#pragma unroll
    for (int j = 0; j < 8; ++j) S0[j] = gload(2, j);
    __syncthreads();
// ... 52 lines not shown
      for (int i = 0; i < 8; ++i) {
        Fn.a[i] = w4::frag(img, wr * 128 + 16 * i);
        Fn.b[i] = w4::frag(img + 16384, wc * 128 + 16 * i);
        dma(kt + W4_LEAD + 1, i);
#pragma unroll
        for (int j = 0; j < 8; ++j) acc[i][j] = ttg::mma<bf16_t>(Fc.b[j], Fc.a[i], acc[i][j]);
        __builtin_amdgcn_sched_barrier(0);
      }
    };
    for (int kt = 0; kt < nk; kt += 2) {
      step(F0, F1, kt);
      step(F1, F0, kt + 1);
    }
    asm volatile("s_waitcnt vmcnt(0)" ::: "memory");
  }
  bf16_t* C = static_cast<bf16_t*>(g.c[bi]);
  const float* bias = g.bias[bi];
  const int q = lane >> 4, lr = lane & 15;
  const __amdgpu_buffer_rsrc_t crs = tt_rsrc(C + (long)m0 * g.ldc + n0);
#pragma unroll
  for (int jp = 0; jp < 4; ++jp) {
    float bv[2][4];
#pragma unroll
    for (int h = 0; h < 2; ++h) {
      const float4 b4 = bias ? *reinterpret_cast<const float4*>(bias + n0 + wc * 128 + 16 * (2 * jp + h) + 4 * q)
                             : make_float4(0.f, 0.f, 0.f, 0.f);
      bv[h][0] = b4.x; bv[h][1] = b4.y; bv[h][2] = b4.z; bv[h][3] = b4.w;
    }
    const int cs = wc * 128 + 16 * (2 * jp + (q & 1)) + 8 * (q >> 1);
#pragma unroll
    for (int i = 0; i < 8; ++i) {
      uint32_t w[2][2];
#pragma unroll
      for (int h = 0; h < 2; ++h) {
        const f32x4 a = acc[i][2 * jp + h];
        w[h][0] = (uint32_t)f2bf(a[0] + bv[h][0]) | ((uint32_t)f2bf(a[1] + bv[h][1]) << 16);
        w[h][1] = (uint32_t)f2bf(a[2] + bv[h][2]) | ((uint32_t)f2bf(a[3] + bv[h][3]) << 16);
      }
      const auto s0 = __builtin_amdgcn_permlane16_swap(w[0][0], w[1][0], false, false);
      const auto s1 = __builtin_amdgcn_permlane16_swap(w[0][1], w[1][1], false, false);
      const uint4 v = make_uint4(s0[0], s1[0], s0[1], s1[1]);
      const int off = (int)(((long)(wr * 128 + 16 * i + lr) * g.ldc + cs) * 2L);
      if (g.stream_out) st16_sc1(crs, off, v);
      else st16_buf(crs, (uint32_t)off, 0, v);
    }
  }
}

int bres_form_for(int M, int N, int K, int nbatch, long lda, long ldc) {
  if (tt::opt(tt::OPT_GEMM_BRES) == 0 || K % 32 || K < 32 || K > 384 || (lda * 2) % 16) return 0;
  if ((long)M * lda * 2 >= (1L << 31)) return 0;
  constexpr int nwg = 256;
  if (tt::opt(tt::OPT_BRES_FORM) == 1 && tt::opt(tt::OPT_BRES_ROWS) != 64 && N % WR_COLS == 0 && K <= 32 * WR_MAXKS) {
    const int ptot = N / WR_COLS * nbatch;
    if (ptot <= nwg) {
      const int ngrp = nwg / ptot;
      const long mg = ((long)(M + ngrp - 1) / ngrp + WR_TR - 1) / WR_TR * WR_TR;
      if ((long)M >= (long)ngrp * (WR_TR / 4) && (mg * ldc + N) * 2 < (1L << 31)) return 2;
    }
  }
  if (N % BR_COLS) return 0;
  const int ptot = N / BR_COLS * nbatch;
  if (ptot > nwg || nwg % ptot) return 0;
  if ((long)M < (long)(nwg / ptot) * 256) return 0;
  return 1;
}

template <typename T, typename TO>
bool try_bres(int akout, int bkout, bool shift, const GemmArgs& g, int nbatch, hipStream_t st, int* rc) {
  *rc = 0;
  if constexpr (!std::is_same<T, bf16_t>::value || !std::is_same<TO, bf16_t>::value) {
    return false;
  } else {
    if (akout || bkout || shift || g.splits != 1 || g.beta || g.relu || g.drop_thresh || g.alpha != 1.f ||
        g.force_regstage || !g.vec_ok)
      return false;
    for (int b = 0; b < nbatch; ++b)
      if (g.bias[b] && (uintptr_t)g.bias[b] % 16) return false;
    const int form = bres_form_for(g.M, g.N, g.K, nbatch, g.lda, g.ldc);
    if (form == 0) return false;
    const bool r64 = tt::opt(tt::OPT_BRES_ROWS) == 64;
    const int npan = g.N / (form == 2 ? WR_COLS : BR_COLS);
    const int nwg = form == 2 ? npan * nbatch * (256 / (npan * nbatch)) : 256;
    const dim3 grid(nwg), blk(form == 1 && r64 ? 256 : 512);
    switch (g.K / 32) {
#define TT_BR(n)                                                                   \
  case n:                                                                          \
    if (r64)                                                                       \
      hipLaunchKernelGGL((gemm_bres<n, 4>), grid, blk, 0, st, g, npan, nbatch);    \
    else                                                                           \
      hipLaunchKernelGGL((gemm_bres<n, 2>), grid, blk, 0, st, g, npan, nbatch);    \
    break;
#define TT_WR(n)                                                                   \
  case n:                                                                          \
    if (form == 2)                                                                 \
      hipLaunchKernelGGL((gemm_wreg<n>), grid, blk, 0, st, g, npan, nbatch);       \
    else if (r64)                                                                  \
      hipLaunchKernelGGL((gemm_bres<n, 4>), grid, blk, 0, st, g, npan, nbatch);    \
    else                                                                           \
      hipLaunchKernelGGL((gemm_bres<n, 2>), grid, blk, 0, st, g, npan, nbatch);    \
    break;
      TT_WR(1) TT_WR(2) TT_WR(3) TT_WR(4) TT_WR(5) TT_WR(6) TT_WR(7) TT_WR(8) TT_WR(9) TT_WR(10) TT_BR(11) TT_BR(12)
#undef TT_WR
#undef TT_BR
      default: return false;
    }
    const hipError_t e = hipGetLastError();
    if (e != hipSuccess) {
      tt::set_error("%s: %s", form == 2 ? "gemm_wreg" : "gemm_bres", hipGetErrorString(e));
      *rc = (int)e;
    }
    return true;
  }
}

bool tall_form_for(bool bf16_in, bool f32_out, int akout, int bkout, bool plain, int M, int N, long lda, long ldb,
                   int kt_per_split) {
  if (tt::opt(tt::OPT_WGRAD_TALL) == 0 || !bf16_in || !f32_out || !akout || !bkout || !plain) return false;
  if (M <= 256 || M > 320 || M % 8 || N % 8 || N <= 0) return false;
  if (tt::opt(tt::OPT_GEMM_REGSTAGE) != 0) return false;
  const long span = ((long)kt_per_split * 64 + 4 * tall::KS) * 2;
  return span * lda < (1L << 32) && span * ldb < (1L << 32);
}
bool gemm_args_plain(const GemmArgs& g, bool shift, int nbatch) {
  if (shift || g.a_split > 0 || g.beta || g.relu || g.drop_thresh) return false;
  for (int b = 0; b < nbatch; ++b)
    if (g.bias[b]) return false;
  return true;
}

template <typename T, typename TO>
int launch_gemm(int akout, int bkout, bool shift, GemmArgs& g, int nbatch, hipStream_t st) {
  constexpr int EPC = 16 / (int)sizeof(T);
  {
    int rc = 0;
    if (try_bres<T, TO>(akout, bkout, shift, g, nbatch, st, &rc)) return rc;
  }
  if (tall_form_for(std::is_same<T, bf16_t>::value, std::is_same<TO, float>::value, akout, bkout,
                    gemm_args_plain(g, shift, nbatch), g.M, g.N, g.lda, g.ldb, g.kt_per_split)) {
    const long units = (long)tt_ceil_div(g.N, 256) * nbatch * g.splits;
    const int mode = tt::opt(tt::OPT_WGRAD_TALL);
    long nfull = units;
    if (mode == 3) nfull = 0;
    else if (mode != 2 && units % 256 > 0 && units % 256 <= 128) nfull = units - units % 256;
    if (nfull > 0) hipLaunchKernelGGL(gemm_tall<false>, dim3((unsigned)nfull), dim3(512), 0, st, g, 0);
    if (units > nfull)
      hipLaunchKernelGGL(gemm_tall<true>, dim3((unsigned)(2 * (units - nfull))), dim3(512), 0, st, g, (int)nfull);
    TT_CHECK_LAUNCH("gemm_tall");
    return 0;
  }
  const bool dma = (akout ? g.M % EPC == 0 : g.K % EPC == 0) && (bkout ? g.N % EPC == 0 : g.K % EPC == 0) &&
                   g.force_regstage != 1;
  const long t256 = (long)tt_ceil_div(g.M, 256) * tt_ceil_div(g.N, 256) * nbatch * g.splits;
  const bool persist_ok = tt::opt(tt::OPT_GEMM_PERSIST) != 0;
  const int nk = (g.K * (int)sizeof(T) + ttg::KTB - 1) / ttg::KTB;
  bool buf = tt::opt(tt::OPT_GEMM_BUF) != 0 && g.K % (ttg::KTB / (int)sizeof(T)) == 0;
  {
    const long span = (long)(g.kt_per_split + 2) * (ttg::KTB / (int)sizeof(T)) * (long)sizeof(T);
    if (akout && span * g.lda >= (1L << 32)) buf = false;
    if (bkout && span * g.ldb >= (1L << 32)) buf = false;
    if (shift && g.seq_t % (ttg::KTB / (int)sizeof(T)) != 0) buf = false;
    if (!akout && (long)256 * g.lda * (long)sizeof(T) >= (1L << 31)) buf = false;
    if (!bkout && (long)256 * g.ldb * (long)sizeof(T) >= (1L << 31)) buf = false;
    for (int b = 0; b < 4 && g.a_split > 0; ++b) {
      if (!g.a[b]) continue;
      const long d = (long)((const char*)g.a_hi[b] - (const char*)g.a[b]) / (long)sizeof(T);
      if (d < 0 || d + (g.M - g.a_split) > g.lda) buf = false;
    }
  }
  if constexpr (std::is_same<T, bf16_t>::value && std::is_same<TO, bf16_t>::value) {
    if (tt::opt(tt::OPT_GEMM_W4) && !akout && !bkout && !shift && g.splits == 1 && !g.beta && !g.relu &&
        !g.drop_thresh && g.alpha == 1.f && g.force_regstage == 0 && g.M % 256 == 0 && g.N % 256 == 0 && g.K % 64 == 0 &&
        g.K >= 32 && g.vec_ok && g.bias_vec_ok && (g.lda * 2) % 16 == 0 && (g.ldb * 2) % 16 == 0 &&
        256L * g.lda * 2 < (1L << 31) && 256L * g.ldb * 2 < (1L << 31) && 256L * g.ldc * 2 < (1L << 31)) {
      const int ntm = g.M / 256, ntn = g.N / 256;
      if (tt::opt(tt::OPT_GEMM_W4) == 2)
        hipLaunchKernelGGL(gemm_w4<true>, dim3((unsigned)(ntm * ntn * nbatch)), dim3(256), 0, st, g, ntm, ntn);
      else
        hipLaunchKernelGGL(gemm_w4<false>, dim3((unsigned)(ntm * ntn * nbatch)), dim3(256), 0, st, g, ntm, ntn);
      TT_CHECK_LAUNCH("gemm_w4");
      return 0;
    }
  }
  if (dma && persist_ok && !shift && (g.force_regstage == 0 || g.force_regstage >= 9) && g.splits == 1 && !g.beta && nk >= 2 && nk <= tt::opt(tt::OPT_GEMM_PERSIST_MAXK) && t256 >= 512 &&
      use_big(g.M, g.N, t256))
    return launch_persist<T, TO>(akout, bkout, shift, g, (int)t256, buf, st);
  if (dma && g.force_regstage != 2 && use_big(g.M, g.N, t256)) {
    if (tt::opt(tt::OPT_GEMM_A3) && buf)
      return launch_t<T, TO, 256, 256, 2, 4, true, true, true>(akout, bkout, shift, g, t256, st);
    if (tt::opt(tt::OPT_GEMM_A3)) return launch_t<T, TO, 256, 256, 2, 4, true, true>(akout, bkout, shift, g, t256, st);
    return launch_t<T, TO, 256, 256, 2, 4, true>(akout, bkout, shift, g, t256, st);
  }
  const long t128 = (long)tt_ceil_div(g.M, 128) * tt_ceil_div(g.N, 128) * nbatch * g.splits;
  if (dma) return launch_t<T, TO, 128, 128, 2, 2, true>(akout, bkout, shift, g, t128, st);
  return launch_t<T, TO, 128, 128, 2, 2, false>(akout, bkout, shift, g, t128, st);
}

}

int tt::tt_hn_scan_gemm(const void* q, long bq, const void* d, long nd, int h, long label_off, float* cm, long nch,
                    hipStream_t st) {
  TT_CHECK_ARG(h % 64 == 0 && h <= 1024 && bq > 0 && nd > 0 && bq < (1L << 31) && nd < (1L << 31),
               "tt_hn_scan_gemm: h %d, bq %ld, nd %ld", h, bq, nd);
  GemmArgs g{};
  g.a[0] = q;
  g.b[0] = d;
  g.lda = g.ldb = h;
  g.M = (int)bq;
  g.N = (int)nd;
  g.K = h;
  g.alpha = 1.f;
  g.splits = 1;
  g.kt_per_split = h / 64;
  g.nbatch = 1;
  g.cm = cm;
  g.nch = nch;
  g.label_off = label_off;
  const long ntm = (bq + 255) / 256, ntn = (nd + 255) / 256, ntiles = ntm * ntn;
  TT_CHECK_ARG(ntiles < (1L << 31), "tt_hn_scan_gemm: too many tiles");
  if (ntiles % 256 == 0 && ntn % 4 == 0) {
    g.walk_g = 4;
    g.walk_x = 8;
  }
  hipLaunchKernelGGL((gemm_persist<bf16_t, false, false, false, float, true, true, true>),
                     dim3((unsigned)std::min<long>(ntiles, 256)), dim3(512), 0, st, g, (int)ntiles);
  TT_CHECK_LAUNCH("gemm_persist (hard-negative scan)");
  return 0;
}

extern "C" int tt_gemm_bres_form(int m, int n, int k, int nbatch, long lda, long ldc) {
  return bres_form_for(m, n, k, nbatch, lda, ldc);
}

static void split_plan(int k, int esz, int* splits, int* kt_per_split) {
  const int nk = tt_ceil_div((long)k * esz, 128);
  int s = *splits < 1 ? 1 : *splits;
  if (s > nk) s = nk > 0 ? nk : 1;
  *kt_per_split = nk > 0 ? tt_ceil_div(nk, s) : 1;
  *splits = nk > 0 ? tt_ceil_div(nk, *kt_per_split) : 1;
}

extern "C" int tt_gemm_tall_form(int dtype, int out_dtype, int a_kouter, int b_kouter, int m, int n, int k, long lda,
                                 long ldb, int splits, int extras) {
  int ktps = 1;
  split_plan(k, dtype == TT_DT_BF16 ? 2 : 4, &splits, &ktps);
  return tall_form_for(dtype == TT_DT_BF16, out_dtype == TT_DT_F32, a_kouter, b_kouter, extras == 0, m, n, lda, ldb, ktps)
             ? 1
             : 0;
}

extern "C" long tt_gemm_ws_size(int m, int n, int nbatch, int splits) {
  (void)m;
  return splits > 1 ? (long)m * n * nbatch * splits : 0;
}

extern "C" int tt_gemm_pick_splits(int m, int n, int k, int nbatch) {
  const bool big = m >= 256 && n >= 256;
  const long tiles = big ? (long)tt_ceil_div(m, 256) * tt_ceil_div(n, 256) * nbatch
                         : (long)tt_ceil_div(m, BM) * tt_ceil_div(n, BN) * nbatch;
  const long target = big ? 512 : 1024;
  if (tiles >= target) return 1;
  const int smax = std::max(1, std::min(64, tt_ceil_div(k, 64) / 8));
  int best = 1;
  double best_eff = 0.0;
  const int s_lo = (int)std::min<long>(smax, std::max<long>(1, target / tiles));
  for (int s = s_lo; s <= std::min<long>(smax, 3 * target / tiles + 1); ++s) {
    const long w = tiles * s;
    const double eff = (double)w / (256.0 * (double)tt_ceil_div(w, 256));
    if (eff > best_eff + 1e-9) { best_eff = eff; best = s; }
  }
  return std::min(best, smax);
}

extern "C" int tt_gemm(int dtype, int out_dtype, int a_kouter, int b_kouter, int m, int n, int k,
                       const tt_gemm_batch* batch, int nbatch, long lda, long ldb, long ldc,
                       float alpha, int beta_accum, int relu, int seq_t, uint32_t drop_seed,
                       float drop_p, int splits, float* splitk_ws, void* stream) {
  return tt_gemm_ct(dtype, out_dtype, a_kouter, b_kouter, m, n, k, batch, nbatch, lda, ldb, ldc, alpha, beta_accum, relu,
                    seq_t, drop_seed, drop_p, splits, splitk_ws, 0, stream);
}

extern "C" int tt_gemm_ct(int dtype, int out_dtype, int a_kouter, int b_kouter, int m, int n, int k,
                          const tt_gemm_batch* batch, int nbatch, long lda, long ldb, long ldc,
                          float alpha, int beta_accum, int relu, int seq_t, uint32_t drop_seed,
                          float drop_p, int splits, float* splitk_ws, int c_trans, void* stream) {
  TT_CHECK_ARG(dtype == TT_DT_F32 || dtype == TT_DT_BF16, "tt_gemm: bad dtype %d", dtype);
  TT_CHECK_ARG(out_dtype == TT_DT_F32 || out_dtype == dtype, "tt_gemm: bad out_dtype %d", out_dtype);
  TT_CHECK_ARG(nbatch >= 1 && nbatch <= 4, "tt_gemm: nbatch %d not in [1,4]", nbatch);
  TT_CHECK_ARG(m >= 0 && n >= 0 && k >= 0, "tt_gemm: negative dims");
  if (m == 0 || n == 0) return 0;
  const int esz = dtype == TT_DT_BF16 ? 2 : 4;
  const int epc = 16 / esz;
  (void)epc;
  TT_CHECK_ARG((lda * esz) % 16 == 0 && (ldb * esz) % 16 == 0,
               "tt_gemm: leading dimensions must be 16-byte multiples (lda=%ld ldb=%ld)", lda, ldb);
  if (splits < 1) splits = 1;
  TT_CHECK_ARG(splits == 1 || (relu == 0 && drop_p == 0.f), "tt_gemm: split-K excludes relu/dropout");
  TT_CHECK_ARG(splits == 1 || splitk_ws != nullptr, "tt_gemm: split-K needs a workspace");
  TT_CHECK_ARG(drop_p >= 0.f && drop_p < 1.f, "tt_gemm: drop_p %f", drop_p);
  bool shift = false;
  GemmArgs g{};
  for (int b = 0; b < nbatch; ++b) {
    TT_CHECK_ARG(batch->a[b] && batch->b[b] && batch->c[b], "tt_gemm: null operand in batch %d", b);
    TT_CHECK_ARG(((uintptr_t)batch->a[b] | (uintptr_t)batch->b[b]) % 16 == 0,
                 "tt_gemm: operands must be 16-byte aligned (batch %d)", b);
    g.a[b] = batch->a[b];
    g.b[b] = batch->b[b];
    g.c[b] = batch->c[b];
    g.bias[b] = batch->bias[b];
    g.bshift[b] = batch->bshift[b];
    g.a_hi[b] = batch->a_hi[b];
    if (batch->a_split > 0)
      TT_CHECK_ARG(batch->a_hi[b] && (uintptr_t)batch->a_hi[b] % 16 == 0, "tt_gemm: a_hi[%d] null or misaligned", b);
    if (batch->bshift[b] != 0) shift = true;
  }
  TT_CHECK_ARG(!shift || (b_kouter && seq_t > 0), "tt_gemm: bshift needs b_kouter and seq_t");
  TT_CHECK_ARG(batch->a_split >= 0 && (batch->a_split == 0 || (a_kouter && batch->a_split % (16 / esz) == 0)),
               "tt_gemm: a_split %d needs a_kouter and a 16-byte multiple", batch->a_split);
  g.a_split = batch->a_split;
  g.lda = lda; g.ldb = ldb; g.ldc = ldc;
  g.M = m; g.N = n; g.K = k;
  g.alpha = alpha; g.beta = beta_accum; g.relu = relu; g.seq_t = seq_t;
  g.force_regstage = tt::opt(tt::OPT_GEMM_REGSTAGE);
  g.nbatch = nbatch;
  g.skew = tt::opt(tt::OPT_GEMM_SKEW);
  g.drop_seed = drop_seed;
  g.drop_row0 = batch->drop_row0;
  g.drop_thresh = drop_p > 0.f ? (uint32_t)(drop_p * 16777216.0f + 0.5f) : 0u;
  g.drop_inv_keep = drop_p > 0.f ? 1.0f / (1.0f - drop_p) : 1.0f;
  split_plan(k, esz, &splits, &g.kt_per_split);
  g.splits = splits;
  TT_CHECK_ARG(!c_trans || splits > 1, "tt_gemm_ct: a transposed C needs split-K (splits %d)", splits);
  g.c_trans = c_trans != 0;
  {
    const int osz = out_dtype == TT_DT_BF16 ? 2 : 4;
    bool ok = (ldc * osz) % 16 == 0;
    for (int b = 0; b < nbatch; ++b) ok = ok && ((uintptr_t)batch->c[b] % 16 == 0);
    g.vec_ok = ok;
    bool bok = true;
    for (int b = 0; b < nbatch; ++b) bok = bok && ((uintptr_t)batch->bias[b] % 16 == 0);
    g.bias_vec_ok = bok;
    g.stream_out = ok && (long)m * n * osz >= (64L << 20) && (long)256 * ldc * osz < (1L << 31);
    g.stream_out = g.stream_out ? tt::opt(tt::OPT_GEMM_STREAM_OUT) : 0;
  }
  hipStream_t st = static_cast<hipStream_t>(stream);
  TT_CHECK_ARG((long)tt_ceil_div(m, 128) * tt_ceil_div(n, 128) * nbatch * splits < (1L << 31), "tt_gemm: too many tiles");

  if (splits > 1) {
    GemmArgs gp = g;
    gp.part_stride = (long)m * n;
    gp.vec_ok = (n % 4 == 0);
    for (int b = 0; b < nbatch; ++b) gp.c[b] = splitk_ws + (long)b * splits * gp.part_stride;
    int rc = dtype == TT_DT_BF16 ? launch_gemm<bf16_t, float>(a_kouter, b_kouter, shift, gp, nbatch, st)
                                 : launch_gemm<float, float>(a_kouter, b_kouter, shift, gp, nbatch, st);
    if (rc) return rc;
    const bool v4 = n % 4 == 0 && (uintptr_t)splitk_ws % 16 == 0;
    const long total = (long)m * n / (v4 ? 4 : 1);
    dim3 rg((unsigned)std::min<long>(tt_ceil_div(total, 256), 2048), nbatch);
#define TT_RED(TO, V) hipLaunchKernelGGL((splitk_reduce_kernel<TO, V>), rg, dim3(256), 0, st, splitk_ws, gp.part_stride, splits, m, n, g)
    if (out_dtype == TT_DT_F32) {
      if (v4) TT_RED(float, 4); else TT_RED(float, 1);
    } else {
      if (v4) TT_RED(bf16_t, 4); else TT_RED(bf16_t, 1);
    }
#undef TT_RED
    TT_CHECK_LAUNCH("splitk_reduce_kernel");
    return 0;
  }
  if (dtype == TT_DT_BF16) {
    return out_dtype == TT_DT_BF16 ? launch_gemm<bf16_t, bf16_t>(a_kouter, b_kouter, shift, g, nbatch, st)
                                   : launch_gemm<bf16_t, float>(a_kouter, b_kouter, shift, g, nbatch, st);
  }
  return launch_gemm<float, float>(a_kouter, b_kouter, shift, g, nbatch, st);
}
```

two_towers_amd/csrc/tt_gru.hip:

```cpp
#include <algorithm>
#include <cstdlib>
#include <mutex>
#include <type_traits>

#include "tt_api.h"
#include "tt_gemm_core.h"

namespace {

struct FwdRec {
  const void* g; const void* whh; const float* bhn; void* y; void* x1; void* save; float* hs;
  int dir; uint32_t seed; int col0;
  uint32_t row0;
};
struct FwdArgs {
  FwdRec r[4];
  int B, T, H;
  long ldg, ldy;
  int s;
  uint32_t drop_thresh;
  float inv_keep;
#ifdef TT_DIAG
  int dbg;
#endif
// ... 2210 lines not shown
  a.inv_keep = drop_p > 0.f ? 1.0f / (1.0f - drop_p) : 1.0f;
#ifdef TT_DIAG
  if (const char* e = getenv("TT_GRU_DBG")) a.dbg = atoi(e);
#endif
  hipStream_t st = (hipStream_t)stream;
  if (dtype == TT_DT_BF16) {
    bool used = false;
    TT_PROPAGATE(gru_fwd_xc_launch(a, nrec, B, T, H, ldg, ldy, ws, ws_bytes, st, &used));
    if (used) return 0;
  }
  if (gru_fwd_persistent(dtype, H)) return launch_fwd_seq(a, nrec, B, H, st);
  return launch_fwd_steps(dtype, a, nrec, B, T, H, ldg, ldy, st);
}

namespace {
struct YpZeroArgs {
  void* y[4];
  int dir[4];
  int B, T, H;
  long ldy;
};
__global__ __launch_bounds__(256) void gru_yprev_zero_rows(YpZeroArgs a) {
  const int per = a.H / 8;
  const long i = (long)blockIdx.x * 256 + threadIdx.x;
  if (i >= (long)a.B * per) return;
  const int rz = blockIdx.y;
  const long b = i / per;
  const int j = (int)(i - b * per) * 8;
  const int t = a.dir[rz] ? a.T - 1 : 0;
  *reinterpret_cast<uint4*>(static_cast<bf16_t*>(a.y[rz]) + (b * a.T + t) * a.ldy + j) = make_uint4(0u, 0u, 0u, 0u);
}
}

extern "C" int tt_gru_yprev_supported(int dtype, int nrec, int B, int T, int H, long ldg, long ldy) {
  if (!gru_bwd_persistent(dtype, H) || H > 512) return 0;
  XcGeo g;
  bool ok = false;
  if (xc_plan(dtype, nrec, B, T, H, ldg, ldy, true, g, &ok, false, true) != 0 || !ok) return 0;
  return 1;
}

extern "C" int tt_gru_fwd_yprev(int dtype, const tt_gru_fwd_rec* recs, void* const* hfinal, int nrec, int B, int T,
                                int H, long ldg, long ldy, long ldf, float drop_p, void* ws, long ws_bytes,
                                void* stream) {
  TT_CHECK_ARG(dtype == TT_DT_BF16, "tt_gru_fwd_yprev: bf16 only (tt_gru_yprev_supported)");
  TT_CHECK_ARG(nrec >= 1 && nrec <= 4, "tt_gru_fwd_yprev: nrec %d", nrec);
  TT_CHECK_ARG(B > 0 && T > 0 && (H == 256 || H == 512), "tt_gru_fwd_yprev: bad shape (H 256 or 512)");
  TT_CHECK_ARG(ws != nullptr && ws_bytes > 0, "tt_gru_fwd_yprev: needs the tt_gru_fwd_ws_size workspace");
  TT_CHECK_ARG((ldy * 2) % 16 == 0 && ldy >= H, "tt_gru_fwd_yprev: ldy=%ld misaligned or below H", ldy);
  TT_CHECK_ARG(drop_p >= 0.f && drop_p < 1.f, "tt_gru_fwd_yprev: drop_p");
  TT_CHECK_ARG(128L * T * std::max({4L * H, ldy, ldg}) * 2 < (1L << 31), "tt_gru_fwd_yprev: tile byte offsets exceed 2 GiB");
  TT_CHECK_ARG(!hfinal || (ldf >= H && (ldf * 2) % 16 == 0 && 256L * ldf * 2 < (1L << 31)),
               "tt_gru_fwd_yprev: ldf=%ld misaligned or below H", ldf);
  YpArgs a{};
  YpZeroArgs z{};
  for (int i = 0; i < nrec; ++i) {
    const tt_gru_fwd_rec& r = recs[i];
    TT_CHECK_ARG(r.g && r.whh && r.bhn && r.y && r.save, "tt_gru_fwd_yprev: null pointer in rec %d", i);
    TT_CHECK_ARG(((uintptr_t)r.y & 15) == 0, "tt_gru_fwd_yprev: y of rec %d is not 16-byte aligned", i);
    TT_CHECK_ARG(!hfinal || (hfinal[i] && ((uintptr_t)hfinal[i] & 15) == 0),
                 "tt_gru_fwd_yprev: hfinal[%d] null or not 16-byte aligned", i);
    a.r[i] = FwdRec{r.g, r.whh, r.bhn, r.y, r.x1, r.save, r.hstate, r.dir, r.drop_seed, r.drop_col0, r.drop_row0};
    a.hfin[i] = hfinal ? hfinal[i] : nullptr;
    z.y[i] = r.y;
    z.dir[i] = r.dir;
  }
  a.B = B; a.T = T; a.H = H; a.ldg = ldg; a.ldy = ldy; a.ldf = hfinal ? ldf : 0;
  a.drop_thresh = drop_p > 0.f ? (uint32_t)(drop_p * 16777216.0f + 0.5f) : 0u;
  a.inv_keep = drop_p > 0.f ? 1.0f / (1.0f - drop_p) : 1.0f;
  z.B = B; z.T = T; z.H = H; z.ldy = ldy;
  hipStream_t st = (hipStream_t)stream;
  bool used = false;
  TT_PROPAGATE(gru_fwd_xc_launch(a, nrec, B, T, H, ldg, ldy, ws, ws_bytes, st, &used));
  TT_CHECK_ARG(used, "tt_gru_fwd_yprev: the column-split forward does not apply to this call (tt_gru_yprev_supported)");
  hipLaunchKernelGGL(gru_yprev_zero_rows, dim3((unsigned)tt_ceil_div((long)B * (H / 8), 256), (unsigned)nrec), dim3(256), 0,
                     st, z);
  TT_CHECK_LAUNCH("gru_yprev_zero_rows");
  return 0;
}

extern "C" long tt_gru_infer_scratch_size(int dtype, int B, int T, int H, int final_only) {
  if ((dtype != TT_DT_F32 && dtype != TT_DT_BF16) || B <= 0 || T <= 0 || H <= 0) return 0;
  if (gru_fwd_persistent(dtype, H)) return 0;
  const long esz = dtype == TT_DT_BF16 ? 2 : 4;
  return 2L * B * H * 4 + (final_only ? 2L * B * H * esz : 0);
}

extern "C" int tt_gru_fwd_infer(int dtype, const tt_gru_infer_rec* recs, int nrec, int B, int T, int H, long ldg,
                                long ldy, long ldf, void* ws, long ws_bytes, void* stream) {
  TT_CHECK_ARG(dtype == TT_DT_F32 || dtype == TT_DT_BF16, "tt_gru_fwd_infer: bad dtype");
  TT_CHECK_ARG(nrec >= 1 && nrec <= 4, "tt_gru_fwd_infer: nrec %d", nrec);
  TT_CHECK_ARG(B > 0 && T > 0 && H > 0, "tt_gru_fwd_infer: bad shape");
  TT_CHECK_ARG(ws_bytes >= 0 && (ws != nullptr || ws_bytes == 0), "tt_gru_fwd_infer: ws / ws_bytes");
  const int esz = dtype == TT_DT_BF16 ? 2 : 4;
  TT_CHECK_ARG(H % 8 == 0 && (ldy * esz) % 16 == 0, "tt_gru_fwd_infer: H=%d (multiple of 8)/ldy=%ld misaligned", H, ldy);
  TT_CHECK_ARG(tt_ceil_div(B, 128) <= 65535, "tt_gru_fwd_infer: B too large");
  TT_CHECK_ARG(128L * T * std::max({4L * H, ldy, ldg}) * esz < (1L << 31),
               "tt_gru_fwd_infer: tile byte offsets exceed 2 GiB");
  const bool has_y = recs[0].y != nullptr, has_f = recs[0].hfinal != nullptr;
  TT_CHECK_ARG(has_y || has_f, "tt_gru_fwd_infer: neither y nor hfinal given");
  TT_CHECK_ARG(!has_f || (ldf >= H && (ldf * esz) % 16 == 0 && 256L * ldf * esz < (1L << 31)),
               "tt_gru_fwd_infer: ldf=%ld misaligned or below H", ldf);
  const bool persistent = gru_fwd_persistent(dtype, H);
  const long state = 2L * B * H * 4;
  InfArgs a{};
  for (int i = 0; i < nrec; ++i) {
    const tt_gru_infer_rec& r = recs[i];
    TT_CHECK_ARG(r.g && r.whh && r.bhn, "tt_gru_fwd_infer: null pointer in rec %d", i);
    TT_CHECK_ARG((r.y != nullptr) == has_y && (r.hfinal != nullptr) == has_f,
                 "tt_gru_fwd_infer: rec %d disagrees with rec 0 on y / hfinal", i);
    TT_CHECK_ARG(persistent || (r.scratch && ((uintptr_t)r.scratch & 15) == 0),
                 "tt_gru_fwd_infer: rec %d needs 16-byte aligned scratch (tt_gru_infer_scratch_size)", i);
    a.r[i] = FwdRec{r.g, r.whh, r.bhn, r.y, nullptr, nullptr, static_cast<float*>(r.scratch), r.dir, 0u, 0, 0u};
    for (int k = nrec; k < 4; ++k) a.hfin[k] = a.himg[k] = nullptr;
    a.hfin[i] = r.hfinal;
    a.himg[i] = r.scratch && !has_y ? static_cast<char*>(r.scratch) + state : nullptr;
  }
  a.B = B; a.T = T; a.H = H; a.ldg = ldg; a.ldy = ldy; a.ldf = ldf;
  a.inv_keep = 1.0f;
  hipStream_t st = (hipStream_t)stream;
  if (dtype == TT_DT_BF16) {
    bool used = false;
    TT_PROPAGATE(gru_fwd_xc_launch(a, nrec, B, T, H, ldg, ldy, ws, ws_bytes, st, &used));
    if (used) return 0;
  }
  if (persistent) return launch_fwd_seq(a, nrec, B, H, st);
  return launch_fwd_steps(dtype, a, nrec, B, T, H, ldg, ldy, st);
}

template <typename T, int BMR>
static void launch_bwd_step(int ring, dim3 grid, hipStream_t st, const BwdArgs& a) {
  if (ring >= 4) hipLaunchKernelGGL((gru_bwd_step<T, BMR, 4>), grid, dim3(256), 0, st, a);
  else if (ring == 3) hipLaunchKernelGGL((gru_bwd_step<T, BMR, 3>), grid, dim3(256), 0, st, a);
  else hipLaunchKernelGGL((gru_bwd_step<T, BMR>), grid, dim3(256), 0, st, a);
}

static int gru_bwd_impl(int dtype, const tt_gru_bwd_rec* recs, int nrec, int B, int T, int H, long ldy, long ldd,
                        long ldf, void* stream, int yprev) {
  TT_CHECK_ARG(dtype == TT_DT_F32 || dtype == TT_DT_BF16, "tt_gru_bwd: bad dtype");
  TT_CHECK_ARG(nrec >= 1 && nrec <= 4, "tt_gru_bwd: nrec %d", nrec);
  TT_CHECK_ARG(B > 0 && T > 0 && H > 0, "tt_gru_bwd: bad shape");
  const int esz = dtype == TT_DT_BF16 ? 2 : 4;
  TT_CHECK_ARG(H % 8 == 0 && (ldd * esz) % 16 == 0, "tt_gru_bwd: H=%d (multiple of 8)/ldd=%ld misaligned", H, ldd);
  TT_CHECK_ARG(256L * T * std::max({ldd, ldy, 4L * H}) * esz < (1L << 31), "tt_gru_bwd: tile byte offsets exceed 2 GiB");
  TT_CHECK_ARG(!yprev || (gru_bwd_persistent(dtype, H) && H <= 512),
               "tt_gru_bwd_yprev: the row-owning backward does not apply to this call (tt_gru_yprev_supported)");
  hipStream_t st = (hipStream_t)stream;
  BwdArgs a{};
  for (int i = 0; i < nrec; ++i) {
    const tt_gru_bwd_rec& r = recs[i];
    TT_CHECK_ARG(r.save && r.y && r.whh && r.dgx && r.dgh && r.dhstate && r.dbias_part,
                 "tt_gru_bwd: null pointer in rec %d", i);
    a.r[i] = BwdRec{r.save, r.y, r.dy, r.dfinal, r.whh, r.dgx, r.dgh, r.dhstate, r.dbias_part, r.dir};
    TT_CHECK_HIP(hipMemsetAsync(r.dbias_part, 0, sizeof(float) * 4L * H * tt_gru_bias_rows(B), st));
  }
  a.B = B; a.T = T; a.H = H; a.ldy = ldy; a.ldd = ldd; a.ldf = ldf;
  a.skew = tt::opt(tt::OPT_GRU_BWD_SKEW);
  a.yprev = yprev;
#ifdef TT_DIAG
  if (const char* e = getenv("TT_GRU_DBG")) a.dbg = atoi(e);
#endif
  const int bmr = bwd_rows(B, H, nrec);
  if (gru_bwd_persistent(dtype, H)) {
    TT_CHECK_ARG(128L * T * std::max({ldd, ldy, 4L * H}) * esz < (1L << 31), "tt_gru_bwd: tile offsets exceed 2 GiB");
    const dim3 grid(tt_ceil_div(B, 128) * nrec);
    if (H == 1024) hipLaunchKernelGGL(gru_bwd_rows<1024>, grid, dim3(512), 0, st, a);
    else if (H == 512) hipLaunchKernelGGL(gru_bwd_rows<512>, grid, dim3(512), 0, st, a);
    else hipLaunchKernelGGL(gru_bwd_rows<256>, grid, dim3(512), 0, st, a);
    TT_CHECK_LAUNCH("gru_bwd_rows");
    return 0;
  }
  if (dtype == TT_DT_BF16 && H % 256 == 0 && bmr == 128 && tt::opt(tt::OPT_GRU_BWD_BIG) != 0) {
    const dim3 grid((H / 256) * tt_ceil_div(B, 256) * nrec);
    for (int s = T - 1; s >= 0; --s) {
      a.s = s;
      hipLaunchKernelGGL(gru_bwd_big, grid, dim3(512), 0, st, a);
      TT_CHECK_LAUNCH("gru_bwd_big");
    }
    return 0;
  }
  const int ngrp = (nrec >= 2 && tt::opt(tt::OPT_GRU_BWD_STREAMS) != 1) ? 2 : 1;
  BwdArgs ga[2] = {a, a};
  int gn[2] = {nrec, 0};
  if (ngrp == 2) {
    gn[0] = nrec / 2;
    gn[1] = nrec - gn[0];
    for (int i = 0; i < gn[1]; ++i) ga[1].r[i] = a.r[gn[0] + i];
  }
  hipStream_t gs[2] = {st, st};
  SideStream* side = nullptr;
  if (ngrp == 2) {
    TT_PROPAGATE(side_stream(&side));
    gs[1] = side->s;
    TT_CHECK_HIP(hipEventRecord(side->fork, st));
    TT_CHECK_HIP(hipStreamWaitEvent(side->s, side->fork, 0));
  }
  XcDev* xd = nullptr;
  TT_PROPAGATE(xc_device(&xd));
  long wgs = 0;
  for (int g = 0; g < ngrp; ++g) wgs += (long)tt_ceil_div(H, 128) * tt_ceil_div(B, bmr) * gn[g];
  const int ring = wgs <= xd->cus ? tt::opt(tt::OPT_GRU_STEP_RING) : 2;
  for (int s = T - 1; s >= 0; --s) {
    for (int g = 0; g < ngrp; ++g) {
      ga[g].s = s;
      const dim3 grid(tt_ceil_div(H, 128) * tt_ceil_div(B, bmr) * gn[g]);
      if (dtype == TT_DT_BF16) {
        if (bmr == 64) launch_bwd_step<bf16_t, 64>(ring, grid, gs[g], ga[g]);
        else launch_bwd_step<bf16_t, 128>(ring, grid, gs[g], ga[g]);
      } else {
        if (bmr == 64) launch_bwd_step<float, 64>(ring, grid, gs[g], ga[g]);
        else launch_bwd_step<float, 128>(ring, grid, gs[g], ga[g]);
      }
      TT_CHECK_LAUNCH("gru_bwd_step");
    }
  }
  if (ngrp == 2) {
    TT_CHECK_HIP(hipEventRecord(side->join, side->s));
    TT_CHECK_HIP(hipStreamWaitEvent(st, side->join, 0));
  }
  return 0;
}

extern "C" int tt_gru_bwd(int dtype, const tt_gru_bwd_rec* recs, int nrec, int B, int T, int H, long ldy,
                          long ldd, long ldf, void* stream) {
  return gru_bwd_impl(dtype, recs, nrec, B, T, H, ldy, ldd, ldf, stream, 0);
}

extern "C" int tt_gru_bwd_yprev(int dtype, const tt_gru_bwd_rec* recs, int nrec, int B, int T, int H, long ldy,
                                long ldd, long ldf, void* stream) {
  return gru_bwd_impl(dtype, recs, nrec, B, T, H, ldy, ldd, ldf, stream, 1);
}
```

two_towers_amd/csrc/tt_head.hip:

```cpp
#include <algorithm>
#include <climits>

#include "tt_api.h"
#include "tt_common.h"

namespace {

constexpr int LN_MAXC = 16;

template <typename T, typename TO>
__global__ __launch_bounds__(256) void ln_relu_fwd_kernel(const T* __restrict__ x, long rows, int C,
                                                          const float* __restrict__ gam,
                                                          const float* __restrict__ bet, float eps,
                                                          TO* __restrict__ u, float* __restrict__ mean,
                                                          float* __restrict__ rstd, uint32_t drop_seed,
                                                          uint32_t drop_thresh, float inv_keep) {
  const long row = (long)blockIdx.x * 4 + (threadIdx.x >> 6);
  const int lane = threadIdx.x & 63;
  if (row >= rows) return;
  const T* xr = x + row * C;
  float v[LN_MAXC];
  float s = 0.f;
#pragma unroll
  for (int q = 0; q < LN_MAXC; ++q) {
    const int c = lane + 64 * q;
    v[q] = c < C ? Elt<T>::ld(xr + c) : 0.f;
    s += v[q];
  }
  const float mu = wave_sum(s) / C;
  float ss = 0.f;
#pragma unroll
  for (int q = 0; q < LN_MAXC; ++q) {
    const int c = lane + 64 * q;
    const float d = c < C ? v[q] - mu : 0.f;
    ss += d * d;
  }
  const float rs = rsqrtf(wave_sum(ss) / C + eps);
#pragma unroll
  for (int q = 0; q < LN_MAXC; ++q) {
    const int c = lane + 64 * q;
    if (c < C) {
      float o = fmaxf((v[q] - mu) * rs * gam[c] + bet[c], 0.f);
      if (drop_thresh) o *= tt_dropout_scale(drop_seed, (uint32_t)row, (uint32_t)c, drop_thresh, inv_keep);
      Elt<TO>::st(u + row * C + c, o);
    }
  }
  if (lane == 0) {
    mean[row] = mu;
    rstd[row] = rs;
  }
}

template <typename T, int NP>
__global__ __launch_bounds__(256) void ln_relu_bwd_kernel(const float* __restrict__ du, const T* __restrict__ x,
                                                          const float* __restrict__ gam,
                                                          const float* __restrict__ bet,
                                                          const float* __restrict__ mean,
                                                          const float* __restrict__ rstd, long rows, int C,
                                                          int rows_per_block, T* __restrict__ dx,
                                                          float* __restrict__ part, uint32_t drop_seed,
                                                          uint32_t drop_thresh, float inv_keep,
                                                          const float* __restrict__ dout2, int C2) {
  __shared__ float red[4][NP][LN_MAXC * 64];
  const int wave = threadIdx.x >> 6, lane = threadIdx.x & 63;
  float pg[LN_MAXC], pb[LN_MAXC], pd[LN_MAXC], p2[LN_MAXC];
#pragma unroll
  for (int q = 0; q < LN_MAXC; ++q) pg[q] = pb[q] = pd[q] = p2[q] = 0.f;
  const long r0 = (long)blockIdx.x * rows_per_block;
  for (long row = r0 + wave; row < std::min(rows, r0 + rows_per_block); row += 4) {
    if constexpr (NP == 4) {
#pragma unroll
      for (int q = 0; q < LN_MAXC; ++q) {
        const int c = lane + 64 * q;
        if (c < C2) p2[q] += dout2[row * C2 + c];
      }
    }
    const float mu = mean[row], rs = rstd[row];
    float xh[LN_MAXC], da[LN_MAXC];
    float s1 = 0.f, s2 = 0.f;
#pragma unroll
    for (int q = 0; q < LN_MAXC; ++q) {
      const int c = lane + 64 * q;
      xh[q] = 0.f;
      da[q] = 0.f;
      if (c < C) {
        xh[q] = (Elt<T>::ld(x + row * C + c) - mu) * rs;
        const float a = xh[q] * gam[c] + bet[c];
        da[q] = a > 0.f ? du[row * C + c] : 0.f;
        if (drop_thresh) da[q] *= tt_dropout_scale(drop_seed, (uint32_t)row, (uint32_t)c, drop_thresh, inv_keep);
        const float dxh = da[q] * gam[c];
        s1 += dxh;
        s2 += dxh * xh[q];
        pg[q] += da[q] * xh[q];
        pb[q] += da[q];
      }
    }
    s1 = wave_sum(s1) / C;
    s2 = wave_sum(s2) / C;
#pragma unroll
    for (int q = 0; q < LN_MAXC; ++q) {
      const int c = lane + 64 * q;
      if (c < C) {
        const float d = rs * (da[q] * gam[c] - s1 - xh[q] * s2);
        Elt<T>::st(dx + row * C + c, d);
        pd[q] += d;
      }
    }
  }
#pragma unroll
  for (int q = 0; q < LN_MAXC; ++q) {
    red[wave][0][lane + 64 * q] = pg[q];
    red[wave][1][lane + 64 * q] = pb[q];
    red[wave][2][lane + 64 * q] = pd[q];
    if constexpr (NP == 4) red[wave][NP - 1][lane + 64 * q] = p2[q];
  }
  __syncthreads();
  for (int e = threadIdx.x; e < NP * C; e += 256) {
    const int k = e / C, c = e % C;
    part[(long)blockIdx.x * NP * C + e] = red[0][k][c] + red[1][k][c] + red[2][k][c] + red[3][k][c];
  }
}

constexpr int LN_ROWS_PER_BLOCK = 16;

inline long head_ws_layout(int dtype, int B, int h, long* o_dout, long* o_du, long* o_dp1, long* o_part,
                           long* o_sk) {
  const int esz = dtype == TT_DT_BF16 ? 2 : 4;
  auto al = [](long x) { return (x + 255) & ~255L; };
  long off = 0;
  *o_dout = off; off = al(off + (long)B * h * esz);
  *o_du = off;   off = al(off + (long)B * 2 * h * 4);
  *o_dp1 = off;  off = al(off + (long)B * 2 * h * esz);
  const long nblk = tt_ceil_div(B, LN_ROWS_PER_BLOCK);
  *o_part = off; off = al(off + nblk * 4L * 2 * h * 4);
  const int s2 = tt_gemm_pick_splits(h, 2 * h, B, 1);
  const int s1 = tt_gemm_pick_splits(2 * h, 4 * h, B, 1);
  const long sk = std::max(tt_gemm_ws_size(h, 2 * h, 1, s2), tt_gemm_ws_size(2 * h, 4 * h, 1, s1));
  *o_sk = off; off = al(off + sk * 4);
  return off;
}

}

extern "C" long tt_proj_head_bwd_ws_size(int dtype, int B, int h) {
  long a, b, c, d, e;
  return head_ws_layout(dtype, B, h, &a, &b, &c, &d, &e);
}

extern "C" int tt_proj_head_fwd(int dtype, const tt_head_fwd_io* io, int ntower, int B, int h, float ln_eps,
                                void* stream) {
  TT_CHECK_ARG(ntower >= 1 && ntower <= 4, "tt_proj_head_fwd: ntower");
  TT_CHECK_ARG(2 * h <= 64 * LN_MAXC, "tt_proj_head_fwd: h=%d too large", h);
  hipStream_t st = (hipStream_t)stream;
  tt_gemm_batch g1{}, g2{};
  for (int i = 0; i < ntower; ++i) {
    g1.a[i] = io[i].x; g1.b[i] = io[i].w1; g1.c[i] = io[i].p1; g1.bias[i] = io[i].b1;
    g2.a[i] = io[i].u; g2.b[i] = io[i].w2; g2.c[i] = io[i].out; g2.bias[i] = io[i].b2;
  }
  TT_PROPAGATE(tt_gemm(dtype, dtype, 0, 0, B, 2 * h, 4 * h, &g1, ntower, 4 * h, 4 * h, 2 * h, 1.f, 0, 0, 0, 0,
                       0.f, 1, nullptr, stream));
  for (int i = 0; i < ntower; ++i) {
    dim3 grid(tt_ceil_div(B, 4));
    if (dtype == TT_DT_BF16)
      hipLaunchKernelGGL((ln_relu_fwd_kernel<bf16_t, bf16_t>), grid, dim3(256), 0, st, (const bf16_t*)io[i].p1,
                         (long)B, 2 * h, io[i].ln_g, io[i].ln_b, ln_eps, (bf16_t*)io[i].u, io[i].mean, io[i].rstd,
                         0u, 0u, 1.f);
    else
      hipLaunchKernelGGL((ln_relu_fwd_kernel<float, float>), grid, dim3(256), 0, st, (const float*)io[i].p1,
                         (long)B, 2 * h, io[i].ln_g, io[i].ln_b, ln_eps, (float*)io[i].u, io[i].mean, io[i].rstd,
                         0u, 0u, 1.f);
    TT_CHECK_LAUNCH("ln_relu_fwd_kernel");
  }
  TT_PROPAGATE(tt_gemm(dtype, TT_DT_F32, 0, 0, B, h, 2 * h, &g2, ntower, 2 * h, 2 * h, h, 1.f, 0, 0, 0, 0, 0.f, 1,
                       nullptr, stream));
  return 0;
}

extern "C" int tt_proj_head_bwd(int dtype, const tt_head_bwd_io* io, int ntower, int B, int h, float ln_eps,
                                void* stream) {
  (void)ln_eps;
  TT_CHECK_ARG(ntower >= 1 && ntower <= 4, "tt_proj_head_bwd: ntower");
  TT_CHECK_ARG(2 * h <= 64 * LN_MAXC, "tt_proj_head_bwd: h=%d too large", h);
  hipStream_t st = (hipStream_t)stream;
  long o_dout, o_du, o_dp1, o_part, o_sk;
  head_ws_layout(dtype, B, h, &o_dout, &o_du, &o_dp1, &o_part, &o_sk);
  const int C = 2 * h;
  const long nblk = tt_ceil_div(B, LN_ROWS_PER_BLOCK);
  for (int i = 0; i < ntower; ++i) {
    const tt_head_bwd_io& q = io[i];
    char* ws = static_cast<char*>(q.ws);
    void* dout_t = ws + o_dout;
    float* du = reinterpret_cast<float*>(ws + o_du);
    void* dp1 = ws + o_dp1;
    float* part = reinterpret_cast<float*>(ws + o_part);
    float* sk = reinterpret_cast<float*>(ws + o_sk);
    TT_PROPAGATE(tt_cast(dtype, q.dout, (long)B * h, dout_t, stream));
    {
      tt_gemm_batch g{};
      g.a[0] = dout_t; g.b[0] = q.u; g.c[0] = q.dw2;
      const int sp = tt_gemm_pick_splits(h, C, B, 1);
      TT_PROPAGATE(tt_gemm(dtype, TT_DT_F32, 1, 1, h, C, B, &g, 1, h, C, C, 1.f, 0, 0, 0, 0, 0.f, sp, sk, stream));
    }
    {
      tt_gemm_batch g{};
      g.a[0] = dout_t; g.b[0] = q.w2; g.c[0] = du;
      TT_PROPAGATE(tt_gemm(dtype, TT_DT_F32, 0, 1, B, C, h, &g, 1, h, C, C, 1.f, 0, 0, 0, 0, 0.f, 1, nullptr, stream));
    }
    if (dtype == TT_DT_BF16)
      hipLaunchKernelGGL((ln_relu_bwd_kernel<bf16_t, 4>), dim3(nblk), dim3(256), 0, st, du, (const bf16_t*)q.p1,
                         q.ln_g, q.ln_b, q.mean, q.rstd, (long)B, C, LN_ROWS_PER_BLOCK, (bf16_t*)dp1, part, 0u, 0u,
                         1.f, q.dout, h);
    else
      hipLaunchKernelGGL((ln_relu_bwd_kernel<float, 4>), dim3(nblk), dim3(256), 0, st, du, (const float*)q.p1,
                         q.ln_g, q.ln_b, q.mean, q.rstd, (long)B, C, LN_ROWS_PER_BLOCK, (float*)dp1, part, 0u, 0u,
                         1.f, q.dout, h);
    TT_CHECK_LAUNCH("ln_relu_bwd_kernel");
    TT_PROPAGATE(tt_colsum(part, nblk, C, 4L * C, q.dg, 0, stream));
    TT_PROPAGATE(tt_colsum(part + C, nblk, C, 4L * C, q.dbeta, 0, stream));
    TT_PROPAGATE(tt_colsum(part + 2 * C, nblk, C, 4L * C, q.db1, 0, stream));
    TT_PROPAGATE(tt_colsum(part + 3 * C, nblk, h, 4L * C, q.db2, 0, stream));
    {
      tt_gemm_batch g{};
      g.a[0] = dp1; g.b[0] = q.x; g.c[0] = q.dw1;
      const int sp = tt_gemm_pick_splits(C, 2 * C, B, 1);
      TT_PROPAGATE(tt_gemm(dtype, TT_DT_F32, 1, 1, C, 2 * C, B, &g, 1, C, 2 * C, 2 * C, 1.f, 0, 0, 0, 0, 0.f, sp, sk,
                           stream));
    }
    {
      tt_gemm_batch g{};
      g.a[0] = dp1; g.b[0] = q.w1; g.c[0] = q.dx;
      TT_PROPAGATE(tt_gemm(dtype, TT_DT_F32, 0, 1, B, 2 * C, C, &g, 1, C, 2 * C, 2 * C, 1.f, 0, 0, 0, 0, 0.f, 1,
                           nullptr, stream));
    }
  }
  return 0;
}

namespace {

inline long head1_ws_layout(int dtype, long rows, int C, long* o_dp1, long* o_part, long* o_sk) {
  const int esz = dtype == TT_DT_BF16 ? 2 : 4;
  auto al = [](long x) { return (x + 255) & ~255L; };
  long off = 0;
  *o_dp1 = off;  off = al(off + rows * C * esz);
  const long nblk = tt_ceil_div(rows, LN_ROWS_PER_BLOCK);
  *o_part = off; off = al(off + nblk * 3L * C * 4);
  const int sp = tt_gemm_pick_splits(C, 2 * C, (int)rows, 1);
  *o_sk = off;   off = al(off + tt_gemm_ws_size(C, 2 * C, 1, sp) * 4);
  return off;
}

inline void drop_params(float p, uint32_t* thresh, float* inv_keep) {
  *thresh = p > 0.f ? (uint32_t)(p * 16777216.0f + 0.5f) : 0u;
  *inv_keep = p > 0.f ? 1.f / (1.f - p) : 1.f;
}

}

extern "C" long tt_proj_head1_bwd_ws_size(int dtype, long rows, int C) {
  long a, b, c;
  return head1_ws_layout(dtype, rows, C, &a, &b, &c);
}

extern "C" int tt_proj_head1_fwd(int dtype, const tt_head1_fwd_io* io, long rows, int C, float ln_eps,
                                 float drop_p, uint32_t drop_seed, void* stream) {
  TT_CHECK_ARG(C >= 1 && C <= 64 * LN_MAXC, "tt_proj_head1_fwd: C=%d out of range", C);
  TT_CHECK_ARG(rows >= 1 && rows <= INT_MAX, "tt_proj_head1_fwd: rows");
  TT_CHECK_ARG(drop_p >= 0.f && drop_p < 1.f, "tt_proj_head1_fwd: drop_p");
  hipStream_t st = (hipStream_t)stream;
  tt_gemm_batch g{};
  g.a[0] = io->x; g.b[0] = io->w1; g.c[0] = io->p1; g.bias[0] = io->b1;
  TT_PROPAGATE(tt_gemm(dtype, dtype, 0, 0, (int)rows, C, 2 * C, &g, 1, 2 * C, 2 * C, C, 1.f, 0, 0, 0, 0, 0.f, 1,
                       nullptr, stream));
  uint32_t thresh;
  float inv_keep;
  drop_params(drop_p, &thresh, &inv_keep);
  dim3 grid(tt_ceil_div(rows, 4));
  if (dtype == TT_DT_BF16)
    hipLaunchKernelGGL((ln_relu_fwd_kernel<bf16_t, float>), grid, dim3(256), 0, st, (const bf16_t*)io->p1, rows, C,
                       io->ln_g, io->ln_b, ln_eps, io->out, io->mean, io->rstd, drop_seed, thresh, inv_keep);
  else
    hipLaunchKernelGGL((ln_relu_fwd_kernel<float, float>), grid, dim3(256), 0, st, (const float*)io->p1, rows, C,
                       io->ln_g, io->ln_b, ln_eps, io->out, io->mean, io->rstd, drop_seed, thresh, inv_keep);
  TT_CHECK_LAUNCH("ln_relu_fwd_kernel");
  return 0;
}

extern "C" int tt_proj_head1_bwd(int dtype, const tt_head1_bwd_io* io, long rows, int C, float drop_p,
                                 uint32_t drop_seed, void* stream) {
  TT_CHECK_ARG(C >= 1 && C <= 64 * LN_MAXC, "tt_proj_head1_bwd: C=%d out of range", C);
  TT_CHECK_ARG(rows >= 1 && rows <= INT_MAX, "tt_proj_head1_bwd: rows");
  TT_CHECK_ARG(drop_p >= 0.f && drop_p < 1.f, "tt_proj_head1_bwd: drop_p");
  hipStream_t st = (hipStream_t)stream;
  long o_dp1, o_part, o_sk;
  head1_ws_layout(dtype, rows, C, &o_dp1, &o_part, &o_sk);
  char* ws = static_cast<char*>(io->ws);
  void* dp1 = ws + o_dp1;
  float* part = reinterpret_cast<float*>(ws + o_part);
  float* sk = reinterpret_cast<float*>(ws + o_sk);
  uint32_t thresh;
  float inv_keep;
  drop_params(drop_p, &thresh, &inv_keep);
  const long nblk = tt_ceil_div(rows, LN_ROWS_PER_BLOCK);
  if (dtype == TT_DT_BF16)
    hipLaunchKernelGGL((ln_relu_bwd_kernel<bf16_t, 3>), dim3(nblk), dim3(256), 0, st, io->dout,
                       (const bf16_t*)io->p1, io->ln_g, io->ln_b, io->mean, io->rstd, rows, C, LN_ROWS_PER_BLOCK,
                       (bf16_t*)dp1, part, drop_seed, thresh, inv_keep, (const float*)nullptr, 0);
  else
    hipLaunchKernelGGL((ln_relu_bwd_kernel<float, 3>), dim3(nblk), dim3(256), 0, st, io->dout,
                       (const float*)io->p1, io->ln_g, io->ln_b, io->mean, io->rstd, rows, C, LN_ROWS_PER_BLOCK,
                       (float*)dp1, part, drop_seed, thresh, inv_keep, (const float*)nullptr, 0);
  TT_CHECK_LAUNCH("ln_relu_bwd_kernel");
  TT_PROPAGATE(tt_colsum(part, nblk, C, 3L * C, io->dg, 0, stream));
  TT_PROPAGATE(tt_colsum(part + C, nblk, C, 3L * C, io->dbeta, 0, stream));
  TT_PROPAGATE(tt_colsum(part + 2 * C, nblk, C, 3L * C, io->db1, 0, stream));
  {
    tt_gemm_batch g{};
    g.a[0] = dp1; g.b[0] = io->x; g.c[0] = io->dw1;
    const int sp = tt_gemm_pick_splits(C, 2 * C, (int)rows, 1);
    TT_PROPAGATE(tt_gemm(dtype, TT_DT_F32, 1, 1, C, 2 * C, (int)rows, &g, 1, C, 2 * C, 2 * C, 1.f, 0, 0, 0, 0, 0.f,
                         sp, sk, stream));
  }
  {
    tt_gemm_batch g{};
    g.a[0] = dp1; g.b[0] = io->w1; g.c[0] = io->dx;
    TT_PROPAGATE(tt_gemm(dtype, TT_DT_F32, 0, 1, (int)rows, 2 * C, C, &g, 1, C, 2 * C, 2 * C, 1.f, 0, 0, 0, 0, 0.f, 1,
                         nullptr, stream));
  }
  return 0;
}
```

two_towers_amd/ops.py:

```python
from __future__ import annotations

import ctypes
from typing import Sequence

import torch

from . import _lib
from ._lib import GemmBatch, call, dtype_code, ptr, stream_ptr


def _esz(dt: torch.dtype) -> int:
    return 2 if dt == torch.bfloat16 else 4


def pad_cols(e: int, dt: torch.dtype) -> int:
    epc = 128 // _esz(dt)
    return (e + epc - 1) // epc * epc


def gemm(a: Sequence[torch.Tensor], b: Sequence[torch.Tensor], c: Sequence[torch.Tensor], *, m: int, n: int,
         k: int, lda: int, ldb: int, ldc: int, a_kouter: bool, b_kouter: bool, dtype: torch.dtype,
         out_dtype: torch.dtype, bias: Sequence[torch.Tensor | None] | None = None,
         bshift: Sequence[int] | None = None, alpha: float = 1.0, accumulate: bool = False,
         relu: bool = False, seq_t: int = 0, drop_seed: int = 0, drop_p: float = 0.0, drop_row0: int = 0,
         splits: int | None = None, a_hi: Sequence[torch.Tensor] | None = None, a_split: int = 0,
         c_trans: bool = False):
    nb = len(a)
    assert 1 <= nb <= 4 and len(b) == nb and len(c) == nb
    bt = GemmBatch()
    for i in range(nb):
        assert a[i].dtype == dtype and b[i].dtype == dtype, (a[i].dtype, b[i].dtype, dtype)
        assert c[i].dtype == out_dtype, (c[i].dtype, out_dtype)
        bt.a[i] = a[i].data_ptr()
        bt.b[i] = b[i].data_ptr()
        bt.c[i] = c[i].data_ptr()
        bt.bias[i] = bias[i].data_ptr() if bias is not None and bias[i] is not None else None
        bt.bshift[i] = bshift[i] if bshift is not None else 0
        if a_split:
            bt.a_hi[i] = a_hi[i].data_ptr()
    bt.a_split = a_split
    bt.drop_row0 = drop_row0 & 0xFFFFFFFF
    lib = _lib.load()
    if splits is None:
        splits = gemm_splits(m, n, k, nb, dtype)
    ws = None
    if splits > 1 and not relu and drop_p == 0.0:
        ws = torch.empty(lib.tt_gemm_ws_size(m, n, nb, splits), dtype=torch.float32, device=c[0].device)
    else:
        splits = 1
    call("tt_gemm_ct", dtype_code(dtype), dtype_code(out_dtype), int(a_kouter), int(b_kouter), m, n, k,
         ctypes.byref(bt), nb, lda, ldb, ldc, alpha, int(accumulate), int(relu), seq_t, drop_seed & 0xFFFFFFFF,
         drop_p, splits, ptr(ws), int(c_trans), stream_ptr(c[0].device))


def gemm_splits(m: int, n: int, k: int, nb: int, dtype: torch.dtype) -> int:
    s = _lib.load().tt_gemm_pick_splits(m, n, k, nb)
    nk = (k * _esz(dtype) + 127) // 128
    if nk <= 0:
        return 1
    per = (nk + min(max(s, 1), nk) - 1) // min(max(s, 1), nk)
    return (nk + per - 1) // per


def embed_gather(table: torch.Tensor, ids: torch.Tensor, out: torch.Tensor):
    assert ids.dtype == torch.int32 and ids.is_contiguous()
    assert table.dim() == 2 and out.shape[-1] == table.shape[1] and out.dtype == table.dtype
    call("tt_embed_gather", dtype_code(table.dtype), table.data_ptr(), table.shape[0], table.shape[1],
         ids.data_ptr(), ids.numel(), out.data_ptr(), stream_ptr(out.device))


def pack_rows(src: torch.Tensor, out: torch.Tensor):
    assert src.dtype == torch.float32 and src.is_contiguous()
    e = src.shape[-1]
    n = src.numel() // e
    call("tt_pack_rows", dtype_code(out.dtype), src.data_ptr(), n, e, out.shape[-1], out.data_ptr(),
         stream_ptr(out.device))


def cast(x: torch.Tensor, out: torch.Tensor):
    assert x.dtype == torch.float32 and x.is_contiguous() and out.numel() == x.numel()
    call("tt_cast", dtype_code(out.dtype), x.data_ptr(), x.numel(), out.data_ptr(), stream_ptr(out.device))


def colsum(x: torch.Tensor, rows: int, cols: int, ld: int, out: torch.Tensor, accumulate: bool = False):
    assert x.dtype == torch.float32 and out.dtype == torch.float32
    call("tt_colsum", x.data_ptr(), rows, cols, ld, out.data_ptr(), int(accumulate), stream_ptr(out.device))


def total(x: torch.Tensor, scale: float, out: torch.Tensor):
    call("tt_sum", x.data_ptr(), x.numel(), scale, out.data_ptr(), stream_ptr(out.device))


def l2norm_fwd(x: torch.Tensor, eps: float, dt: torch.dtype, want_f32: bool = True):
    assert x.dtype == torch.float32 and x.is_contiguous() and x.dim() == 2
    rows, cols = x.shape
    y = torch.empty(rows, cols, dtype=dt, device=x.device)
    y32 = y if dt == torch.float32 else (torch.empty_like(x) if want_f32 else None)
    norm = torch.empty(rows, dtype=torch.float32, device=x.device)
    call("tt_l2norm_fwd", dtype_code(dt), x.data_ptr(), rows, cols, eps, y.data_ptr(),
         None if y32 is y else ptr(y32), norm.data_ptr(), stream_ptr(x.device))
    return y, y32, norm


def l2norm_bwd(dy: torch.Tensor, y32: torch.Tensor, norm: torch.Tensor, eps: float, dx: torch.Tensor | None = None,
               accumulate: bool = False):
    assert dy.dtype == torch.float32 and dy.is_contiguous() and y32.dtype == torch.float32
    rows, cols = dy.shape
    if dx is None:
        dx = torch.empty_like(dy)
        accumulate = False
    call("tt_l2norm_bwd", dy.data_ptr(), y32.data_ptr(), norm.data_ptr(), rows, cols, eps, dx.data_ptr(),
         int(accumulate), stream_ptr(dy.device))
    return dx
```

two_towers_amd/towers.py:

```python
from __future__ import annotations

import ctypes
import os
import threading
from dataclasses import dataclass

import torch
import torch.nn.functional as F

from . import _lib, dist, ops, timing
from ._lib import GruBwdRec, GruFwdRec, GruInferRec, HeadBwdIO, HeadFwdIO, call, dtype_code, stream_ptr

PARAMS_PER_TOWER = 22
LN_EPS = 1e-5
HEAD_DT = torch.float32


def gru_param_names():
    names = []
    for layer in (0, 1):
        for sfx in ("", "_reverse"):
            for w in ("weight_ih", "weight_hh", "bias_ih", "bias_hh"):
                names.append(f"{w}_l{layer}{sfx}")
    return names
# ... 72 lines not shown
                whh.append(wh)
            self.wih.append(w)
            self.bias.append(b)
            self.whh.append(whh)
            self.bhn.append([g[f"bias_hh_l{layer}{s}"][2 * H:] for s in ("", "_reverse")])
        call("tt_pack_multi", jobs, nj, stream_ptr(dev))

    def _pack_torch(self, g, H, E, Ep, dt):
        for layer in (0, 1):
            wf, wr = g[f"weight_ih_l{layer}"], g[f"weight_ih_l{layer}_reverse"]
            w = torch.cat([wf, wr], 0)
            if layer == 0 and Ep != E:
                w = F.pad(w, (0, Ep - E))
            self.wih.append(w.to(dt).contiguous())
            bs = []
            for sfx in ("", "_reverse"):
                bi, bh = g[f"bias_ih_l{layer}{sfx}"], g[f"bias_hh_l{layer}{sfx}"]
                bs.append(torch.cat([bi[: 2 * H] + bh[: 2 * H], bi[2 * H:]]))
            self.bias.append(torch.cat(bs).float().contiguous())
            self.whh.append([g[f"weight_hh_l{layer}{s}"].to(dt).contiguous() for s in ("", "_reverse")])
            self.bhn.append([g[f"bias_hh_l{layer}{s}"][2 * H:].float().contiguous() for s in ("", "_reverse")])


def _packed(p, cfg: TowerCfg, Ep: int, cache_ok: bool) -> _Packed:
    if not cache_ok:
        return _Packed(p, cfg, Ep)
    key = (cfg.dtype, cfg.H, cfg.head, Ep, tuple(t._version for t in p), tuple(t.data_ptr() for t in p))
    hit = getattr(p[0], "_tt_pack", None)
    if hit is not None and hit[0] == key:
        return hit[1]
    pk = _Packed(p, cfg, Ep)
    p[0]._tt_pack = (key, pk)
    return pk


def _alloc(shape, dt, dev):
    return torch.empty(shape, dtype=dt, device=dev)


_status_lock = threading.Lock()
_status_pending: list = []
_step_guard: dict = {}
_guard_reset: set = set()


def step_guard(dev) -> torch.Tensor:
    dev = torch.device(dev)
    with _status_lock:
        g = _step_guard.get(dev)
        if g is None:
            g = _step_guard[dev] = torch.zeros(1, dtype=torch.int32, device=dev)
    return g


def gru_fwd_workspace(nrec, B, T, H, dt, dev):
    nb = _lib.load().tt_gru_fwd_ws_size(dtype_code(dt), nrec, B, T, H, 6 * H, 2 * H)
    if nb <= 0:
        return None
    ws = torch.empty(nb, dtype=torch.uint8, device=dev)
    if ws.data_ptr() % 256:
        raise _lib.TTError("GRU forward workspace is not 256-byte aligned")
    ws[:256].zero_()
    return ws


def reset_guard_if_reported(dev):
    dev = torch.device(dev)
    with _status_lock:
        due = dev in _guard_reset
        _guard_reset.discard(dev)
    if due:
        with torch.cuda.device(dev):
            step_guard(dev).zero_()


def watch_gru_status(ws, arm: bool = True):
    with torch.cuda.device(ws.device):
        st = torch.cuda.current_stream(ws.device)
        word = ws[:4].view(torch.int32)
        if arm:
            step_guard(ws.device).bitwise_or_(word)
        host = torch.zeros(1, dtype=torch.int32, pin_memory=True)
        host.copy_(word, non_blocking=True)
        ev = torch.cuda.Event()
        ev.record(st)
    with _status_lock:
        _status_pending.append((ev, host, torch.device(ws.device)))


def check_gru_status(wait: bool = True):
    with _status_lock:
        pend = list(_status_pending)
        _status_pending.clear()
    bad = 0
    keep = []
    bad_devs = set()
    for ev, host, dev in pend:
        if not wait and not ev.query():
            keep.append((ev, host, dev))
            continue
        ev.synchronize()
        if host.item() != 0:
            bad += 1
            bad_devs.add(dev)
    with _status_lock:
        if keep:
            _status_pending[:0] = keep
        _guard_reset.update(bad_devs)
    if bad:
        raise _lib.GruTimeoutError(
            f"{bad} column-split GRU forward launch(es) timed out waiting for a member workgroup "
            "(not all workgroups were resident); their outputs are invalid and the optimiser step "
            "that followed (two_towers_amd.Adam) left the weights unchanged. Set option gru_fwd_xc=0 "
            "(env TT_GRU_FWD_XC=0) to use the row-owning kernel.")


def _xs_selected() -> bool:
    try:
        return bool(_lib.get_option("gru_fwd_xs"))
    except _lib.TTError:
        return False


def table_cols(table, x):
    return getattr(table, "real_cols", table.shape[1])


def featurize(x: torch.Tensor, table: torch.Tensor | None, Ep: int, dt: torch.dtype) -> torch.Tensor:
    if x.dtype in (torch.int32, torch.int64):
        if table is None:
            raise _lib.TTError("integer token ids need an embedding table (model.set_embedding_table)")
        if table.dtype != dt or table.shape[1] != Ep:
            raise _lib.TTError(f"embedding table must be {dt} with {Ep} columns, got {table.dtype} {tuple(table.shape)}")
        ids = x.reshape(-1).to(torch.int32).contiguous()
        out = _alloc((ids.numel(), Ep), dt, x.device)
        esz = 2 if dt == torch.bfloat16 else 4
        gb = ids.numel() * (4 + 2 * table_cols(table, x) * esz)
        with timing.region("embed_gather", 1, gb, gb):
            ops.embed_gather(table, ids, out)
        return out
    if x.dim() != 3:
        raise ValueError(f"expected [B, T, E] embeddings or [B, T] token ids, got shape {tuple(x.shape)}")
    src = x.float().contiguous()
    out = _alloc((src.shape[0] * src.shape[1], Ep), dt, x.device)
    ops.pack_rows(src, out)
    return out


def yprev_supported(cfg, B, T) -> bool:
    H = cfg.H
    if not _lib.get_option("gru_yprev"):
        return False
    return bool(_lib.load().tt_gru_yprev_supported(dtype_code(cfg.dtype), 2 * cfg.ntowers, B, T, H, 6 * H, 2 * H))


def _gru_layer_fwd(cfg, xs, K, ldx, packs, layer, B, T, seeds, want_x1, ws, yprev=False, want_final=False):
    n, H, dt, dev = cfg.ntowers, cfg.H, cfg.dtype, xs[0].device
    BT = B * T
    G = [_alloc((BT, 6 * H), dt, dev) for _ in range(n)]
    esz = 2 if dt == torch.bfloat16 else 4
    kr = cfg.E if layer == 0 else K
    with timing.region(f"input_proj_l{layer}", 1, 2.0 * BT * 6 * H * kr * n,
                       float(n * esz * (BT * kr + 6 * H * kr + BT * 6 * H))):
        ops.gemm(xs, [p.wih[layer] for p in packs], G, m=BT, n=6 * H, k=K, lda=ldx, ldb=K, ldc=6 * H,
                 a_kouter=False, b_kouter=False, dtype=dt, out_dtype=dt, bias=[p.bias[layer] for p in packs])
    Y = [_alloc((BT, 2 * H), dt, dev) for _ in range(n)]
    X1 = [_alloc((BT, 2 * H), dt, dev) for _ in range(n)] if want_x1 else None
    S = [[_alloc((BT, 4 * H), dt, dev) for _ in range(2)] for _ in range(n)]
    hs = _alloc((n * 2, 2, B, H), torch.float32, dev)
    recs = (GruFwdRec * (2 * n))()
    for ti in range(n):
        for d in range(2):
            r = recs[ti * 2 + d]
            r.g = G[ti][:, d * 3 * H:].data_ptr()
            r.whh = packs[ti].whh[layer][d].data_ptr()
            r.bhn = packs[ti].bhn[layer][d].data_ptr()
            r.y = Y[ti][:, d * H:].data_ptr()
            r.x1 = X1[ti][:, d * H:].data_ptr() if want_x1 else None
            r.save = S[ti][d].data_ptr()
            r.hstate = hs[ti * 2 + d].data_ptr()
            r.dir = d
            r.drop_seed = seeds[ti] & 0xFFFFFFFF
            r.drop_col0 = d * H
            r.drop_row0 = (cfg.rank * B * T) & 0xFFFFFFFF
    nl = _lib.load().tt_gru_fwd_launches_for(dtype_code(dt), 2 * n, B, T, H, 6 * H, 2 * H) if ws is not None \
        else _lib.load().tt_gru_fwd_launches(dtype_code(dt), T, H)
    per = esz * (8 + (1 if want_x1 else 0)) + (0 if nl == 1 else esz + 8)
    if nl == 1 and ws is not None:
        form = "gru_fwd_xs" if H == 512 and _xs_selected() else "gru_fwd_xcp"
        kname = f"{form}<{H}, {'true' if want_x1 and cfg.drop_p > 0 else 'false'}"
    elif nl == 1:
        kname = "gru_fwd_seq<"
    else:
        kname = "gru_fwd_step<"
    hfin = [_alloc((B, 2 * H), dt, dev) for _ in range(n)] if yprev and want_final else None
    with timing.region("gru_fwd", nl, 2.0 * B * H * 3 * H * 2 * n * (T - 1), float(B * T * H * 2 * n * per),
                       kernel=kname):
        if yprev:
            fin = None
            if hfin is not None:
                fin = (ctypes.c_void_p * (2 * n))(*[hfin[ti][:, d * H:].data_ptr() for ti in range(n) for d in range(2)])
            call("tt_gru_fwd_yprev", dtype_code(dt), recs, fin, 2 * n, B, T, H, 6 * H, 2 * H, 2 * H,
                 cfg.drop_p if want_x1 else 0.0, ws.data_ptr(), ws.numel(), stream_ptr(dev))
        else:
            call("tt_gru_fwd", dtype_code(dt), recs, 2 * n, B, T, H, 6 * H, 2 * H, cfg.drop_p if want_x1 else 0.0,
                 ws.data_ptr() if ws is not None else None, ws.numel() if ws is not None else 0, stream_ptr(dev))
    del G
    return Y, X1, S, hfin


def _gru_layer_infer(cfg, xs, K, ldx, packs, layer, B, T, ws, final_only):
    n, H, dt, dev = cfg.ntowers, cfg.H, cfg.dtype, xs[0].device
    BT = B * T
    lib = _lib.load()
    G = [_alloc((BT, 6 * H), dt, dev) for _ in range(n)]
    esz = 2 if dt == torch.bfloat16 else 4
    kr = cfg.E if layer == 0 else K
    with timing.region(f"input_proj_infer_l{layer}", 1, 2.0 * BT * 6 * H * kr * n,
                       float(n * esz * (BT * kr + 6 * H * kr + BT * 6 * H))):
        ops.gemm(xs, [p.wih[layer] for p in packs], G, m=BT, n=6 * H, k=K, lda=ldx, ldb=K, ldc=6 * H,
                 a_kouter=False, b_kouter=False, dtype=dt, out_dtype=dt, bias=[p.bias[layer] for p in packs])
    out = [_alloc((B, 2 * H) if final_only else (BT, 2 * H), dt, dev) for _ in range(n)]
    nb = lib.tt_gru_infer_scratch_size(dtype_code(dt), B, T, H, int(final_only))
    scr = _alloc((2 * n, nb), torch.uint8, dev) if nb > 0 else None
    recs = (GruInferRec * (2 * n))()
    for ti in range(n):
        for d in range(2):
            r = recs[ti * 2 + d]
            r.g = G[ti][:, d * 3 * H:].data_ptr()
            r.whh = packs[ti].whh[layer][d].data_ptr()
            r.bhn = packs[ti].bhn[layer][d].data_ptr()
            r.y = None if final_only else out[ti][:, d * H:].data_ptr()
            r.hfinal = out[ti][:, d * H:].data_ptr() if final_only else None
            r.scratch = scr[ti * 2 + d].data_ptr() if scr is not None else None
            r.dir = d
    nl = lib.tt_gru_fwd_launches_for(dtype_code(dt), 2 * n, B, T, H, 6 * H, 2 * H) if ws is not None \
        else lib.tt_gru_fwd_launches(dtype_code(dt), T, H)
    per = esz * (3 if final_only else 4) + (0 if nl == 1 else esz * (2 if final_only else 1) + 8)
    if nl == 1 and ws is not None:
        kname = f"{'gru_fwd_xs' if H == 512 and _xs_selected() else 'gru_fwd_xcp'}<{H}, false, (anonymous namespace)::InfArgs>"
    elif nl == 1:
        kname = "gru_fwd_seq<"
    else:
        kname = "gru_fwd_step<"
    with timing.region("gru_infer", nl, 2.0 * B * H * 3 * H * 2 * n * (T - 1), float(B * T * H * 2 * n * per),
                       kernel=kname):
        call("tt_gru_fwd_infer", dtype_code(dt), recs, 2 * n, B, T, H, 6 * H, 2 * H, 2 * H,
             ws.data_ptr() if ws is not None else None, ws.numel() if ws is not None else 0, stream_ptr(dev))
    return out


def towers_infer(cfg: TowerCfg, table, xs, params):
    n = cfg.ntowers
    _lib.require_gpu(*xs, *params)
    check_gru_status(wait=True)
    dt, E, H, h = cfg.dtype, cfg.E, cfg.H, cfg.h
    dev = xs[0].device
    reset_guard_if_reported(dev)
    B, T = xs[0].shape[0], xs[0].shape[1]
    for x in xs:
        if x.shape[0] != B or x.shape[1] != T:
            raise ValueError("query and doc inputs must share [B, T] in one fused call")
    Ep = ops.pad_cols(E, dt)
    npt = cfg.nparams
    with torch.no_grad():
        packs = [_packed(params[i * npt:(i + 1) * npt], cfg, Ep, True) for i in range(n)]
        X0 = [featurize(x, table, Ep, dt) for x in xs]
        ws = gru_fwd_workspace(2 * n, B, T, H, dt, dev)
        Y0 = _gru_layer_infer(cfg, X0, Ep, Ep, packs, 0, B, T, ws, False)
        del X0
        hfin = _gru_layer_infer(cfg, Y0, 2 * H, 2 * H, packs, 1, B, T, ws, True)
        del Y0
        if ws is not None:
            watch_gru_status(ws, arm=False)
        hcat = [f if f.dtype == HEAD_DT else f.to(HEAD_DT) for f in hfin]
        if cfg.head == "none":
            return tuple(hcat)
        outs, keep = [], []
        io = (HeadFwdIO * n)()
        for ti in range(n):
            pk = packs[ti]
            p1 = _alloc((B, 2 * h), HEAD_DT, dev)
            u = _alloc((B, 2 * h), HEAD_DT, dev)
            mean = _alloc((B,), torch.float32, dev)
            rstd = _alloc((B,), torch.float32, dev)
            out = _alloc((B, h), torch.float32, dev)
            q = io[ti]
            q.w1, q.b1, q.ln_g, q.ln_b = pk.w1.data_ptr(), pk.b1.data_ptr(), pk.ln_g.data_ptr(), pk.ln_b.data_ptr()
            q.w2, q.b2 = pk.w2.data_ptr(), pk.b2.data_ptr()
            q.x, q.p1, q.mean, q.rstd, q.u, q.out = (hcat[ti].data_ptr(), p1.data_ptr(), mean.data_ptr(),
                                                     rstd.data_ptr(), u.data_ptr(), out.data_ptr())
            outs.append(out)
            keep += [p1, u, mean, rstd]
        call("tt_proj_head_fwd", dtype_code(HEAD_DT), io, n, B, h, LN_EPS, stream_ptr(dev))
        return tuple(outs)


def _gru_layer_bwd(cfg, layer, B, T, S, Y, dY, dfinal, packs, yprev=False):
    n, H, dt, dev = cfg.ntowers, cfg.H, cfg.dtype, Y[0].device
    BT = B * T
    lib = _lib.load()
    dG = [_alloc((BT, 8 * H), dt, dev) for _ in range(n)]
    dhs = _alloc((n * 2, 2, B, H), dt, dev)
    nbr = lib.tt_gru_bias_rows(B)
    part = _alloc((n * 2, nbr, 4 * H), torch.float32, dev)
    recs = (GruBwdRec * (2 * n))()
    for ti in range(n):
        for d in range(2):
            r = recs[ti * 2 + d]
            r.save = S[ti][d].data_ptr()
            r.y = Y[ti][:, d * H:].data_ptr()
            r.dy = dY[ti][:, d * H:].data_ptr() if dY is not None else None
            r.dfinal = dfinal[ti][:, d * H:].data_ptr() if dfinal is not None else None
            r.whh = packs[ti].whh[layer][d].data_ptr()
            r.dgx = dG[ti][:, d * 3 * H:].data_ptr()
            r.dgh = dG[ti][:, 6 * H + d * H:].data_ptr()
            r.dhstate = dhs[ti * 2 + d].data_ptr()
            r.dbias_part = part[ti * 2 + d].data_ptr()
            r.dir = d
    ldf = dfinal[0].shape[1] if dfinal is not None else 0
    esz = 2 if dt == torch.bfloat16 else 4
    nl = lib.tt_gru_bwd_launches(dtype_code(dt), T, H)
    carry = 0 if lib.tt_gru_bwd_carry_on_chip(dtype_code(dt), T, H) else 2
    per = esz * (12 + carry + (1 if dY is not None else 0))
    kname = (f"gru_bwd_rows<{H}>" if nl == 1 else
             "gru_bwd_big" if dt == torch.bfloat16 and H % 256 == 0 and _lib.get_option("gru_bwd_big") else "gru_bwd_step<")
    with timing.region("gru_bwd", nl, 2.0 * B * 3 * H * H * 2 * n * (T - 1), float(B * T * H * 2 * n * per),
                       kernel=kname):
        call("tt_gru_bwd_yprev" if yprev else "tt_gru_bwd", dtype_code(dt), recs, 2 * n, B, T, H, 2 * H, 8 * H, ldf,
             stream_ptr(dev))
    sums = _alloc((n * 2, 4 * H), torch.float32, dev)
    for i in range(2 * n):
        ops.colsum(part[i], nbr, 4 * H, 4 * H, sums[i])
    dbih = [[sums[ti * 2 + d, : 3 * H] for d in range(2)] for ti in range(n)]
    dbhh = [[torch.cat([sums[ti * 2 + d, : 2 * H], sums[ti * 2 + d, 3 * H:]]) for d in range(2)] for ti in range(n)]
    return dG, dbih, dbhh


_WGRAD_T = os.environ.get("TT_WGRAD_T", "1") != "0"
WGRAD_OVERLAP = os.environ.get("TT_WGRAD_OVERLAP", "0") == "1"
_wgrad_streams: dict = {}


def _wgrad_stream(dev) -> torch.cuda.Stream:
    dev = torch.device(dev)
    with _status_lock:
        s = _wgrad_streams.get(dev)
        if s is None:
            s = _wgrad_streams[dev] = torch.cuda.Stream(device=dev)
    return s


def _weight_grads(cfg, B, T, dG, Xin, K, ldx, Y, kr=None, yprev=False):
    n, H, dt, dev = cfg.ntowers, cfg.H, cfg.dtype, dG[0].device
    BT = B * T
    dWih = [[_alloc((3 * H, K), torch.float32, dev) for _ in range(2)] for _ in range(n)]
    dWhh = [[_alloc((3 * H, H), torch.float32, dev) for _ in range(2)] for _ in range(n)]
    a_ih, b_ih, c_ih, a_hh, a_hi, b_hh, c_hh, sh = [], [], [], [], [], [], [], []
    for ti in range(n):
        for d in range(2):
            a_ih.append(dG[ti][:, d * 3 * H:])
            b_ih.append(Xin[ti])
            c_ih.append(dWih[ti][d])
            a_hh.append(dG[ti][:, d * 3 * H:])
            a_hi.append(dG[ti][:, 6 * H + d * H:])
            b_hh.append(Y[ti][:, d * H:])
            c_hh.append(dWhh[ti][d])
            sh.append(-1 if d == 0 else 1)
    esz = 2 if dt == torch.bfloat16 else 4
    kr = K if kr is None else kr
    with timing.region("wgrad_ih", 1, 2.0 * 3 * H * kr * BT * 2 * n,
                       float(n * (esz * BT * (6 * H + kr) + 2 * 3 * H * kr * 4))):
        if _WGRAD_T and dt == torch.bfloat16 and 0 < K % 256 <= 128:
            if ops.gemm_splits(K, 3 * H, BT, len(c_ih), dt) > 1:
                ops.gemm(b_ih, a_ih, c_ih, m=K, n=3 * H, k=BT, lda=ldx, ldb=8 * H, ldc=K, a_kouter=True,
                         b_kouter=True, dtype=dt, out_dtype=torch.float32, c_trans=True)
            else:
                cT = [_alloc((K, 3 * H), torch.float32, dev) for _ in c_ih]
                ops.gemm(b_ih, a_ih, cT, m=K, n=3 * H, k=BT, lda=ldx, ldb=8 * H, ldc=3 * H, a_kouter=True,
                         b_kouter=True, dtype=dt, out_dtype=torch.float32)
                for c, ct in zip(c_ih, cT):
                    c.copy_(ct.t())
        else:
            ops.gemm(a_ih, b_ih, c_ih, m=3 * H, n=K, k=BT, lda=8 * H, ldb=ldx, ldc=K, a_kouter=True,
                     b_kouter=True, dtype=dt, out_dtype=torch.float32)
    with timing.region("wgrad_hh", 1, 2.0 * 3 * H * H * BT * 2 * n,
                       float(n * (esz * BT * (6 * H + 2 * H) + 2 * 3 * H * H * 4))):
        if yprev:
            ops.gemm(a_hh, b_hh, c_hh, m=3 * H, n=H, k=BT, lda=8 * H, ldb=2 * H, ldc=H, a_kouter=True, b_kouter=True,
                     dtype=dt, out_dtype=torch.float32, a_hi=a_hi, a_split=2 * H)
        else:
            ops.gemm(a_hh, b_hh, c_hh, m=3 * H, n=H, k=BT, lda=8 * H, ldb=2 * H, ldc=H, a_kouter=True, b_kouter=True,
                     dtype=dt, out_dtype=torch.float32, bshift=sh, seq_t=T, a_hi=a_hi, a_split=2 * H)
    return dWih, dWhh


class TowersFn(torch.autograd.Function):

    @staticmethod
    def forward(ctx, cfg: TowerCfg, table, group, cache_ok, *args):
        n = cfg.ntowers
        xs, params = args[:n], args[n:]
        _lib.require_gpu(*xs, *params)
        check_gru_status(wait=True)
        dt, E, H, h = cfg.dtype, cfg.E, cfg.H, cfg.h
        dev = xs[0].device
        reset_guard_if_reported(dev)
        B, T = xs[0].shape[0], xs[0].shape[1]
        for x in xs:
            if x.shape[0] != B or x.shape[1] != T:
                raise ValueError("query and doc inputs must share [B, T] in one fused call")
        Ep = ops.pad_cols(E, dt)
        npt = cfg.nparams
        packs = [_packed(params[i * npt:(i + 1) * npt], cfg, Ep, cache_ok) for i in range(n)]
        X0 = [featurize(x, table, Ep, dt) for x in xs]
        train_drop = cfg.drop_p > 0.0
        seeds = [int(torch.randint(0, 2 ** 31 - 1, (1,)).item()) for _ in range(n)] if train_drop else [0] * n
        ws = gru_fwd_workspace(2 * n, B, T, H, dt, dev)
        yp1 = ws is not None and yprev_supported(cfg, B, T)
        yp0 = yp1 and train_drop
        Y0, X1, S0, _ = _gru_layer_fwd(cfg, X0, Ep, Ep, packs, 0, B, T, seeds, train_drop, ws, yprev=yp0)
        Xl1 = X1 if train_drop else Y0
        Y1, _, S1, hfin = _gru_layer_fwd(cfg, Xl1, 2 * H, 2 * H, packs, 1, B, T, seeds, False, ws, yprev=yp1,
                                         want_final=True)
        if ws is not None:
            watch_gru_status(ws, arm=any(ctx.needs_input_grad))
        hcat = []
        for ti in range(n):
            if hfin is not None:
                hcat.append(hfin[ti].to(HEAD_DT))
                continue
            y = Y1[ti].view(B, T, 2 * H)
            hcat.append(torch.cat([y[:, T - 1, :H], y[:, 0, H:]], 1).to(HEAD_DT).contiguous())
        ctx.cfg = cfg
        ctx.yprev = (yp0, yp1)
        ctx.group = group
        ctx.params = params
        ctx.dims = (B, T, Ep)
        ctx.seeds = seeds
        ctx.packs = packs
        if cfg.head == "none":
            ctx.acts = (X0, Y0, X1, S0, Y1, S1, None, None, None, None, None)
            return tuple(hcat)
        outs, p1s, means, rstds, us = [], [], [], [], []
        io = (HeadFwdIO * n)()
        for ti in range(n):
            pk = packs[ti]
            p1 = _alloc((B, 2 * h), HEAD_DT, dev)
            u = _alloc((B, 2 * h), HEAD_DT, dev)
            mean = _alloc((B,), torch.float32, dev)
            rstd = _alloc((B,), torch.float32, dev)
            out = _alloc((B, h), torch.float32, dev)
            q = io[ti]
            q.w1, q.b1, q.ln_g, q.ln_b = pk.w1.data_ptr(), pk.b1.data_ptr(), pk.ln_g.data_ptr(), pk.ln_b.data_ptr()
            q.w2, q.b2 = pk.w2.data_ptr(), pk.b2.data_ptr()
            q.x, q.p1, q.mean, q.rstd, q.u, q.out = (hcat[ti].data_ptr(), p1.data_ptr(), mean.data_ptr(),
                                                     rstd.data_ptr(), u.data_ptr(), out.data_ptr())
            outs.append(out); p1s.append(p1); means.append(mean); rstds.append(rstd); us.append(u)
        call("tt_proj_head_fwd", dtype_code(HEAD_DT), io, n, B, h, LN_EPS, stream_ptr(dev))
        ctx.acts = (X0, Y0, X1, S0, Y1, S1, hcat, p1s, means, rstds, us)
        return tuple(outs)

    @staticmethod
    def backward(ctx, *gouts):
        cfg = ctx.cfg
        check_gru_status(wait=False)
        n, dt, E, H, h = cfg.ntowers, cfg.dtype, cfg.E, cfg.H, cfg.h
        B, T, Ep = ctx.dims
        yp0, yp1 = ctx.yprev
        packs = ctx.packs
        X0, Y0, X1, S0, Y1, S1, hcat, p1s, means, rstds, us = ctx.acts
        dev = Y0[0].device
        lib = _lib.load()
        st = stream_ptr(dev)
        head_grads = [[] for _ in range(n)]
        dhcat = []
        if cfg.head == "none":
            for ti in range(n):
                g = gouts[ti]
                dhcat.append(torch.zeros(B, 2 * H, dtype=torch.float32, device=dev) if g is None
                             else g.float().contiguous())
        ws = None
        if cfg.head == "proj2":
            ws = _alloc((lib.tt_proj_head_bwd_ws_size(dtype_code(HEAD_DT), B, h),), torch.uint8, dev)
        for ti in range(n if cfg.head == "proj2" else 0):
            g = gouts[ti]
            g = torch.zeros(B, h, dtype=torch.float32, device=dev) if g is None else g.float().contiguous()
            pk = packs[ti]
            dx = _alloc((B, 2 * H), torch.float32, dev)
            dw1 = _alloc(pk.w1.shape, torch.float32, dev)
            db1 = _alloc((2 * h,), torch.float32, dev)
            dg = _alloc((2 * h,), torch.float32, dev)
            dbeta = _alloc((2 * h,), torch.float32, dev)
            dw2 = _alloc(pk.w2.shape, torch.float32, dev)
            db2 = _alloc((h,), torch.float32, dev)
            io = HeadBwdIO()
            io.w1, io.ln_g, io.ln_b, io.w2 = pk.w1.data_ptr(), pk.ln_g.data_ptr(), pk.ln_b.data_ptr(), pk.w2.data_ptr()
            io.x, io.p1, io.mean, io.rstd, io.u = (hcat[ti].data_ptr(), p1s[ti].data_ptr(), means[ti].data_ptr(),
                                                   rstds[ti].data_ptr(), us[ti].data_ptr())
            io.dout, io.dx = g.data_ptr(), dx.data_ptr()
            io.dw1, io.db1, io.dg, io.dbeta, io.dw2, io.db2 = (dw1.data_ptr(), db1.data_ptr(), dg.data_ptr(),
                                                               dbeta.data_ptr(), dw2.data_ptr(), db2.data_ptr())
            io.ws = ws.data_ptr()
            call("tt_proj_head_bwd", dtype_code(HEAD_DT), ctypes.byref(io), 1, B, h, LN_EPS, st)
            head_grads[ti] = [dw1, db1, dg, dbeta, dw2, db2]
            dhcat.append(dx)
        dG1, dbih1, dbhh1 = _gru_layer_bwd(cfg, 1, B, T, S1, Y1, None, dhcat, packs, yprev=yp1)
        Xl1 = X1 if X1 is not None else Y0
        red = dist.OverlapReducer(ctx.group[0]) if ctx.group is not None else None
        gl = [{} for _ in range(n)]

        def layer1_wgrads():
            dWih1, dWhh1 = _weight_grads(cfg, B, T, dG1, Xl1, 2 * H, 2 * H, Y1, yprev=yp1)
            _layer_grads(gl, 1, E, Ep, dWih1, dWhh1, dbih1, dbhh1)
            if red is not None:
                _reduce_into(red, gl, head_grads)

        main = torch.cuda.current_stream(dev)
        side = _wgrad_stream(dev) if WGRAD_OVERLAP else None
        if side is None:
            layer1_wgrads()
        dY0 = [_alloc((B * T, 2 * H), dt, dev) for _ in range(n)]
        esz = 2 if dt == torch.bfloat16 else 4
        with timing.region("dgrad_l1", 1, 2.0 * B * T * 2 * H * 6 * H * n,
                           float(n * esz * (B * T * 6 * H + B * T * 2 * H))):
            if X1 is None:
                ops.gemm(dG1, [p.wih[1] for p in packs], dY0, m=B * T, n=2 * H, k=6 * H, lda=8 * H, ldb=2 * H,
                         ldc=2 * H, a_kouter=False, b_kouter=True, dtype=dt, out_dtype=dt)
            else:
                for ti in range(n):
                    ops.gemm([dG1[ti]], [packs[ti].wih[1]], [dY0[ti]], m=B * T, n=2 * H, k=6 * H, lda=8 * H,
                             ldb=2 * H, ldc=2 * H, a_kouter=False, b_kouter=True, dtype=dt, out_dtype=dt,
                             drop_seed=ctx.seeds[ti], drop_p=cfg.drop_p, drop_row0=cfg.rank * B * T)
        if side is not None:
            side.wait_stream(main)
            for t in (*dG1, *Xl1, *Y1, *[g for hg in head_grads for g in hg], *[x for b in dbih1 for x in b],
                      *[x for b in dbhh1 for x in b]):
                t.record_stream(side)
            with torch.cuda.stream(side):
                layer1_wgrads()
        del dG1
        dG0, dbih0, dbhh0 = _gru_layer_bwd(cfg, 0, B, T, S0, Y0, dY0, None, packs, yprev=yp0)
        del dY0
        dWih0, dWhh0 = _weight_grads(cfg, B, T, dG0, X0, Ep, Ep, Y0, kr=E, yprev=yp0)
        gl0 = [{} for _ in range(n)]
        _layer_grads(gl0, 0, E, Ep, dWih0, dWhh0, dbih0, dbhh0)
        if side is not None:
            main.wait_stream(side)
            for t in [*[v for d in gl for v in d.values()], *[g for hg in head_grads for g in hg]]:
                t.record_stream(main)
        if red is not None:
            _reduce_into(red, gl0, [[] for _ in range(n)])
            red.finish(ctx.params)
        grads = []
        for ti in range(n):
            gl[ti].update(gl0[ti])
            grads.extend(gl[ti][k] for k in GRU_NAMES)
            grads.extend(head_grads[ti])
        ctx.acts = None
        ctx.packs = None
        ctx.params = None
        return (None, None, None, None, *([None] * n), *grads)


def _layer_grads(gl, layer, E, Ep, dWih, dWhh, dbih, dbhh):
    for ti in range(len(gl)):
        for d, sfx in enumerate(("", "_reverse")):
            w = dWih[ti][d]
            if layer == 0 and Ep != E:
                w = w[:, :E].contiguous()
            gl[ti][f"weight_ih_l{layer}{sfx}"] = w
            gl[ti][f"weight_hh_l{layer}{sfx}"] = dWhh[ti][d]
            gl[ti][f"bias_ih_l{layer}{sfx}"] = dbih[ti][d].contiguous()
            gl[ti][f"bias_hh_l{layer}{sfx}"] = dbhh[ti][d]


def _reduce_into(red, gl, head_grads):
    keys = [(ti, k) for ti in range(len(gl)) for k in gl[ti]]
    heads = [(ti, j) for ti in range(len(head_grads)) for j in range(len(head_grads[ti]))]
    views = red.launch([gl[ti][k] for ti, k in keys] + [head_grads[ti][j] for ti, j in heads])
    for (ti, k), v in zip(keys, views):
        gl[ti][k] = v
    for (ti, j), v in zip(heads, views[len(keys):]):
        head_grads[ti][j] = v


def run_towers(cfg: TowerCfg, table, xs, params, reduce_group=None, reduce: bool = False):
    if cfg.H % 8:
        raise ValueError(f"GRU hidden size {cfg.H} must be a multiple of 8 on the HIP path "
                         "(the step epilogues update 8 consecutive units per thread)")
    group = (reduce_group,) if reduce and dist.active(reduce_group) else None
    cache_ok = not (torch.is_grad_enabled() and any(p.requires_grad for p in params))
    if cache_ok and cfg.drop_p == 0.0:
        return towers_infer(cfg, table, xs, params)
    return TowersFn.apply(cfg, table, group, cache_ok, *xs, *params)
```

Baseline: 162,100 pairs/s.

## Fuse GRU bias reductions, batch head backward, and trim padded wgrad rows

Adds a step_tail option that folds the per-record GRU bias column sums into one kernel, which writes dbih and dbhh directly. The same option merges the contiguous dbias memsets into one, runs the two towers' projection-head backward as a single launch, and makes the transposed split-K wgrad write only the unpadded rows (ct_rows) so a later slice copy is no longer needed. GEMM kernel selection can now use a separate sel_nbatch count. The aim is fewer small launches and copies in the backward tail, at the cost of more code paths and a new early-exit condition in the split-K reduction.

```diff
diff --git a/include/tt_hip.h b/include/tt_hip.h
--- a/include/tt_hip.h
+++ b/include/tt_hip.h
@@ -53,6 +53,10 @@
                const tt_gemm_batch* batch, int nbatch, long lda, long ldb, long ldc, float alpha,
                int beta_accum, int relu, int seq_t, uint32_t drop_seed, float drop_p, int splits,
                float* splitk_ws, int c_trans, void* stream);
+int tt_gemm_ct_rows(int dtype, int out_dtype, int a_kouter, int b_kouter, int m, int n, int k,
+                    const tt_gemm_batch* batch, int nbatch, long lda, long ldb, long ldc, float alpha,
+                    int beta_accum, int relu, int seq_t, uint32_t drop_seed, float drop_p, int splits,
+                    float* splitk_ws, int c_trans, int ct_rows, void* stream);
 long tt_gemm_ws_size(int m, int n, int nbatch, int splits);
 int tt_gemm_pick_splits(int m, int n, int k, int nbatch);
 int tt_gemm_bres_form(int m, int n, int k, int nbatch, long lda, long ldc);
@@ -108,6 +112,7 @@
 int tt_gru_bwd_launches(int dtype, int T, int H);
 int tt_gru_bwd_carry_on_chip(int dtype, int T, int H);
 int tt_gru_bias_rows(int B);
+int tt_gru_bias_sums(const float* const* part, int nrec, int nbr, int H, float* dbih, float* dbhh, void* stream);
 
 int tt_gru_yprev_supported(int dtype, int nrec, int B, int T, int H, long ldg, long ldy);
 int tt_gru_fwd_yprev(int dtype, const tt_gru_fwd_rec* recs, void* const* hfinal, int nrec, int B, int T, int H,
@@ -141,6 +146,7 @@
 int tt_proj_head_bwd(int dtype, const tt_head_bwd_io* io, int ntower, int B, int h, float ln_eps,
                      void* stream);
 long tt_proj_head_bwd_ws_size(int dtype, int B, int h);
+int tt_proj_head_bwd_splits(int B, int h, int* dw1_splits, int* dw2_splits);
 
 typedef struct {
   const void* x;
diff --git a/two_towers_amd/_lib.py b/two_towers_amd/_lib.py
--- a/two_towers_amd/_lib.py
+++ b/two_towers_amd/_lib.py
@@ -122,6 +122,9 @@
     "tt_gemm_ct": (c_int, [c_int, c_int, c_int, c_int, c_int, c_int, c_int, POINTER(GemmBatch), c_int, c_long,
                            c_long, c_long, c_float, c_int, c_int, c_int, c_uint32, c_float, c_int, c_void_p,
                            c_int, c_void_p]),
+    "tt_gemm_ct_rows": (c_int, [c_int, c_int, c_int, c_int, c_int, c_int, c_int, POINTER(GemmBatch), c_int, c_long,
+                                c_long, c_long, c_float, c_int, c_int, c_int, c_uint32, c_float, c_int, c_void_p,
+                                c_int, c_int, c_void_p]),
     "tt_gemm_ws_size": (c_long, [c_int, c_int, c_int, c_int]),
     "tt_gemm_pick_splits": (c_int, [c_int, c_int, c_int, c_int]),
     "tt_gemm_bres_form": (c_int, [c_int, c_int, c_int, c_int, c_long, c_long]),
@@ -131,6 +134,7 @@
     "tt_gru_bwd": (c_int, [c_int, POINTER(GruBwdRec), c_int, c_int, c_int, c_int, c_long, c_long, c_long,
                            c_void_p]),
     "tt_gru_bias_rows": (c_int, [c_int]),
+    "tt_gru_bias_sums": (c_int, [POINTER(c_void_p), c_int, c_int, c_int, c_void_p, c_void_p, c_void_p]),
     "tt_gru_bwd_launches": (c_int, [c_int, c_int, c_int]),
     "tt_gru_bwd_carry_on_chip": (c_int, [c_int, c_int, c_int]),
     "tt_gru_fwd_launches": (c_int, [c_int, c_int, c_int]),
@@ -147,6 +151,7 @@
     "tt_proj_head_fwd": (c_int, [c_int, POINTER(HeadFwdIO), c_int, c_int, c_int, c_float, c_void_p]),
     "tt_proj_head_bwd": (c_int, [c_int, POINTER(HeadBwdIO), c_int, c_int, c_int, c_float, c_void_p]),
     "tt_proj_head_bwd_ws_size": (c_long, [c_int, c_int, c_int]),
+    "tt_proj_head_bwd_splits": (c_int, [c_int, c_int, POINTER(c_int), POINTER(c_int)]),
     "tt_proj_head1_fwd": (c_int, [c_int, POINTER(Head1FwdIO), c_long, c_int, c_float, c_float, c_uint32,
                                   c_void_p]),
     "tt_proj_head1_bwd": (c_int, [c_int, POINTER(Head1BwdIO), c_long, c_int, c_float, c_uint32, c_void_p]),
diff --git a/two_towers_amd/csrc/tt_api.h b/two_towers_amd/csrc/tt_api.h
--- a/two_towers_amd/csrc/tt_api.h
+++ b/two_towers_amd/csrc/tt_api.h
@@ -44,9 +44,12 @@
   OPT_BRES_FORM,
   OPT_WGRAD_TALL,
   OPT_GRU_YPREV,
+  OPT_STEP_TAIL,
   OPT_N
 };
 int opt(Opt o);
+int tt_gemm_sel(int dtype, int out_dtype, int a_kouter, int b_kouter, int m, int n, int k, const tt_gemm_batch* batch,
+                int nbatch, int sel_nbatch, long lda, long ldb, long ldc, int splits, float* splitk_ws, hipStream_t st);
 int tt_hn_scan_gemm(const void* q, long bq, const void* d, long nd, int h, long label_off, float* cm, long nch,
                     hipStream_t st);
 }
diff --git a/two_towers_amd/csrc/tt_common.h b/two_towers_amd/csrc/tt_common.h
--- a/two_towers_amd/csrc/tt_common.h
+++ b/two_towers_amd/csrc/tt_common.h
@@ -178,6 +178,21 @@
   for (int o = 32; o > 0; o >>= 1) v += __shfl_xor(v, o, 64);
   return v;
 }
+
+TT_DEV float colsum64(const float* __restrict__ x, long rows, long ld, bool valid, float (*red)[64]) {
+  const int wave = threadIdx.x >> 6, lane = threadIdx.x & 63;
+  float s = 0.f;
+  if (valid)
+    for (long r = wave; r < rows; r += 16) s += x[r * ld];
+  red[wave][lane] = s;
+  __syncthreads();
+  float t = 0.f;
+  if (wave == 0 && valid) {
+#pragma unroll
+    for (int w = 0; w < 16; ++w) t += red[w][lane];
+  }
+  return t;
+}
 TT_DEV float wave_max(float v) {
 #pragma unroll
   for (int o = 32; o > 0; o >>= 1) v = fmaxf(v, __shfl_xor(v, o, 64));
diff --git a/two_towers_amd/csrc/tt_elem.hip b/two_towers_amd/csrc/tt_elem.hip
--- a/two_towers_amd/csrc/tt_elem.hip
+++ b/two_towers_amd/csrc/tt_elem.hip
@@ -38,18 +38,25 @@
 __global__ __launch_bounds__(1024) void colsum_kernel(const float* __restrict__ x, long rows, int cols, long ld,
                                                       int accumulate, float* __restrict__ out) {
   __shared__ float red[16][64];
-  const int wave = threadIdx.x >> 6, lane = threadIdx.x & 63;
-  const int c = blockIdx.x * 64 + lane;
-  float s = 0.f;
-  if (c < cols)
-    for (long r = wave; r < rows; r += 16) s += x[r * ld + c];
-  red[wave][lane] = s;
-  __syncthreads();
-  if (wave == 0 && c < cols) {
-    float t = 0.f;
-#pragma unroll
-    for (int w = 0; w < 16; ++w) t += red[w][lane];
-    out[c] = accumulate ? out[c] + t : t;
+  const int c = blockIdx.x * 64 + (threadIdx.x & 63);
+  const float t = colsum64(x + c, rows, ld, c < cols, red);
+  if (threadIdx.x < 64 && c < cols) out[c] = accumulate ? out[c] + t : t;
+}
+
+struct BiasSumArgs {
+  const float* part[8];
+};
+__global__ __launch_bounds__(1024) void gru_bias_sums_kernel(BiasSumArgs a, long rows, int H,
+                                                             float* __restrict__ dbih, float* __restrict__ dbhh) {
+  __shared__ float red[16][64];
+  const int c = blockIdx.x * 64 + (threadIdx.x & 63);
+  const int cols = 4 * H;
+  const float t = colsum64(a.part[blockIdx.y] + c, rows, cols, c < cols, red);
+  if (threadIdx.x < 64 && c < cols) {
+    const long o = (long)blockIdx.y * 3 * H;
+    if (c < 3 * H) dbih[o + c] = t;
+    if (c < 2 * H) dbhh[o + c] = t;
+    else if (c >= 3 * H) dbhh[o + c - H] = t;
   }
 }
 
@@ -176,6 +183,21 @@
   return 0;
 }
 
+extern "C" int tt_gru_bias_sums(const float* const* part, int nrec, int nbr, int H, float* dbih, float* dbhh,
+                                void* stream) {
+  TT_CHECK_ARG(part && nrec >= 1 && nrec <= 8 && nbr >= 0 && H >= 1 && dbih && dbhh,
+               "tt_gru_bias_sums: nrec %d (1..8), nbr %d, H %d", nrec, nbr, H);
+  BiasSumArgs a{};
+  for (int i = 0; i < nrec; ++i) {
+    TT_CHECK_ARG(part[i], "tt_gru_bias_sums: null partial block %d", i);
+    a.part[i] = part[i];
+  }
+  hipLaunchKernelGGL(gru_bias_sums_kernel, dim3(tt_ceil_div(4L * H, 64), nrec), dim3(1024), 0, (hipStream_t)stream, a,
+                     (long)nbr, H, dbih, dbhh);
+  TT_CHECK_LAUNCH("gru_bias_sums_kernel");
+  return 0;
+}
+
 extern "C" int tt_sum(const float* x, long n, float scale, float* out, void* stream) {
   hipLaunchKernelGGL(sum_kernel, dim3(1), dim3(256), 0, (hipStream_t)stream, x, n, scale, out);
   TT_CHECK_LAUNCH("sum_kernel");
diff --git a/two_towers_amd/csrc/tt_gemm.hip b/two_towers_amd/csrc/tt_gemm.hip
--- a/two_towers_amd/csrc/tt_gemm.hip
+++ b/two_towers_amd/csrc/tt_gemm.hip
@@ -43,7 +43,7 @@
     {"gemm_iepi", "TT_GEMM_IEPI", 1},             {"bres_rows", "TT_BRES_ROWS", 32},
     {"hn_scan_v", "TT_HN_SCAN_V", 5},             {"gemm_w4", "TT_GEMM_W4", 0},
     {"bres_form", "TT_BRES_FORM", 1},             {"wgrad_tall", "TT_WGRAD_TALL", 1},
-    {"gru_yprev", "TT_GRU_YPREV", 1},
+    {"gru_yprev", "TT_GRU_YPREV", 1},             {"step_tail", "TT_STEP_TAIL", 1},
 };
 struct OptTable {
   std::atomic<int> v[OPT_N];
@@ -108,6 +108,8 @@
   int walk_g, walk_x;
   int nbatch;
   int c_trans;
+  int ct_rows;
+  int sel_nbatch;
   float* cm;
   long nch, label_off;
 };
@@ -1291,6 +1293,7 @@
   const long total = (long)M * N / V;
   for (long e = (long)blockIdx.x * 256 + threadIdx.x; e < total; e += (long)gridDim.x * 256) {
     float v[V];
+    if (g.c_trans && e * V / N >= g.ct_rows) break;
     if constexpr (V == 4) {
       float4 a = make_float4(0.f, 0.f, 0.f, 0.f);
       for (int s = 0; s < splits; ++s) {
@@ -1649,6 +1652,7 @@
   const bool dma = (akout ? g.M % EPC == 0 : g.K % EPC == 0) && (bkout ? g.N % EPC == 0 : g.K % EPC == 0) &&
                    g.force_regstage != 1;
   const long t256 = (long)tt_ceil_div(g.M, 256) * tt_ceil_div(g.N, 256) * nbatch * g.splits;
+  const long sel256 = t256 / nbatch * g.sel_nbatch;
   const bool persist_ok = tt::opt(tt::OPT_GEMM_PERSIST) != 0;
   const int nk = (g.K * (int)sizeof(T) + ttg::KTB - 1) / ttg::KTB;
   bool buf = tt::opt(tt::OPT_GEMM_BUF) != 0 && g.K % (ttg::KTB / (int)sizeof(T)) == 0;
@@ -1679,10 +1683,10 @@
       return 0;
     }
   }
-  if (dma && persist_ok && !shift && (g.force_regstage == 0 || g.force_regstage >= 9) && g.splits == 1 && !g.beta && nk >= 2 && nk <= tt::opt(tt::OPT_GEMM_PERSIST_MAXK) && t256 >= 512 &&
-      use_big(g.M, g.N, t256))
+  if (dma && persist_ok && !shift && (g.force_regstage == 0 || g.force_regstage >= 9) && g.splits == 1 && !g.beta && nk >= 2 && nk <= tt::opt(tt::OPT_GEMM_PERSIST_MAXK) && sel256 >= 512 &&
+      use_big(g.M, g.N, sel256))
     return launch_persist<T, TO>(akout, bkout, shift, g, (int)t256, buf, st);
-  if (dma && g.force_regstage != 2 && use_big(g.M, g.N, t256)) {
+  if (dma && g.force_regstage != 2 && use_big(g.M, g.N, sel256)) {
     if (tt::opt(tt::OPT_GEMM_A3) && buf)
       return launch_t<T, TO, 256, 256, 2, 4, true, true, true>(akout, bkout, shift, g, t256, st);
     if (tt::opt(tt::OPT_GEMM_A3)) return launch_t<T, TO, 256, 256, 2, 4, true, true>(akout, bkout, shift, g, t256, st);
@@ -1777,10 +1781,40 @@
                     seq_t, drop_seed, drop_p, splits, splitk_ws, 0, stream);
 }
 
+static int gemm_impl(int dtype, int out_dtype, int a_kouter, int b_kouter, int m, int n, int k,
+                     const tt_gemm_batch* batch, int nbatch, long lda, long ldb, long ldc, float alpha, int beta_accum,
+                     int relu, int seq_t, uint32_t drop_seed, float drop_p, int splits, float* splitk_ws, int c_trans,
+                     int ct_rows, int sel_nbatch, void* stream);
+
 extern "C" int tt_gemm_ct(int dtype, int out_dtype, int a_kouter, int b_kouter, int m, int n, int k,
                           const tt_gemm_batch* batch, int nbatch, long lda, long ldb, long ldc,
                           float alpha, int beta_accum, int relu, int seq_t, uint32_t drop_seed,
                           float drop_p, int splits, float* splitk_ws, int c_trans, void* stream) {
+  return gemm_impl(dtype, out_dtype, a_kouter, b_kouter, m, n, k, batch, nbatch, lda, ldb, ldc, alpha, beta_accum, relu,
+                   seq_t, drop_seed, drop_p, splits, splitk_ws, c_trans, m, nbatch, stream);
+}
+
+extern "C" int tt_gemm_ct_rows(int dtype, int out_dtype, int a_kouter, int b_kouter, int m, int n, int k,
+                               const tt_gemm_batch* batch, int nbatch, long lda, long ldb, long ldc, float alpha,
+                               int beta_accum, int relu, int seq_t, uint32_t drop_seed, float drop_p, int splits,
+                               float* splitk_ws, int c_trans, int ct_rows, void* stream) {
+  TT_CHECK_ARG(c_trans ? (ct_rows >= 1 && ct_rows <= m && ldc >= ct_rows) : ct_rows == m,
+               "tt_gemm_ct_rows: ct_rows %d (m %d, ldc %ld, c_trans %d)", ct_rows, m, ldc, c_trans);
+  return gemm_impl(dtype, out_dtype, a_kouter, b_kouter, m, n, k, batch, nbatch, lda, ldb, ldc, alpha, beta_accum, relu,
+                   seq_t, drop_seed, drop_p, splits, splitk_ws, c_trans, ct_rows, nbatch, stream);
+}
+
+int tt::tt_gemm_sel(int dtype, int out_dtype, int a_kouter, int b_kouter, int m, int n, int k,
+                    const tt_gemm_batch* batch, int nbatch, int sel_nbatch, long lda, long ldb, long ldc, int splits,
+                    float* splitk_ws, hipStream_t st) {
+  return gemm_impl(dtype, out_dtype, a_kouter, b_kouter, m, n, k, batch, nbatch, lda, ldb, ldc, 1.f, 0, 0, 0, 0u, 0.f,
+                   splits, splitk_ws, 0, m, sel_nbatch, st);
+}
+
+static int gemm_impl(int dtype, int out_dtype, int a_kouter, int b_kouter, int m, int n, int k,
+                     const tt_gemm_batch* batch, int nbatch, long lda, long ldb, long ldc, float alpha, int beta_accum,
+                     int relu, int seq_t, uint32_t drop_seed, float drop_p, int splits, float* splitk_ws, int c_trans,
+                     int ct_rows, int sel_nbatch, void* stream) {
   TT_CHECK_ARG(dtype == TT_DT_F32 || dtype == TT_DT_BF16, "tt_gemm: bad dtype %d", dtype);
   TT_CHECK_ARG(out_dtype == TT_DT_F32 || out_dtype == dtype, "tt_gemm: bad out_dtype %d", out_dtype);
   TT_CHECK_ARG(nbatch >= 1 && nbatch <= 4, "tt_gemm: nbatch %d not in [1,4]", nbatch);
@@ -1829,6 +1863,8 @@
   g.splits = splits;
   TT_CHECK_ARG(!c_trans || splits > 1, "tt_gemm_ct: a transposed C needs split-K (splits %d)", splits);
   g.c_trans = c_trans != 0;
+  g.ct_rows = ct_rows;
+  g.sel_nbatch = sel_nbatch >= 1 ? sel_nbatch : nbatch;
   {
     const int osz = out_dtype == TT_DT_BF16 ? 2 : 4;
     bool ok = (ldc * osz) % 16 == 0;
diff --git a/two_towers_amd/csrc/tt_gru.hip b/two_towers_amd/csrc/tt_gru.hip
--- a/two_towers_amd/csrc/tt_gru.hip
+++ b/two_towers_amd/csrc/tt_gru.hip
@@ -2386,7 +2386,16 @@
     TT_CHECK_ARG(r.save && r.y && r.whh && r.dgx && r.dgh && r.dhstate && r.dbias_part,
                  "tt_gru_bwd: null pointer in rec %d", i);
     a.r[i] = BwdRec{r.save, r.y, r.dy, r.dfinal, r.whh, r.dgx, r.dgh, r.dhstate, r.dbias_part, r.dir};
-    TT_CHECK_HIP(hipMemsetAsync(r.dbias_part, 0, sizeof(float) * 4L * H * tt_gru_bias_rows(B), st));
+  }
+  {
+    const long blk = 4L * H * tt_gru_bias_rows(B);
+    bool contig = tt::opt(tt::OPT_STEP_TAIL) != 0;
+    for (int i = 1; i < nrec; ++i) contig = contig && recs[i].dbias_part == recs[0].dbias_part + i * blk;
+    if (contig) {
+      TT_CHECK_HIP(hipMemsetAsync(recs[0].dbias_part, 0, sizeof(float) * blk * nrec, st));
+    } else {
+      for (int i = 0; i < nrec; ++i) TT_CHECK_HIP(hipMemsetAsync(recs[i].dbias_part, 0, sizeof(float) * blk, st));
+    }
   }
   a.B = B; a.T = T; a.H = H; a.ldy = ldy; a.ldd = ldd; a.ldf = ldf;
   a.skew = tt::opt(tt::OPT_GRU_BWD_SKEW);
diff --git a/two_towers_amd/csrc/tt_head.hip b/two_towers_amd/csrc/tt_head.hip
--- a/two_towers_amd/csrc/tt_head.hip
+++ b/two_towers_amd/csrc/tt_head.hip
@@ -7,6 +7,46 @@
 namespace {
 
 constexpr int LN_MAXC = 16;
+
+template <typename T, typename TO>
+TT_DEV void ln_relu_fwd_rows(const T* __restrict__ x, long rows, int C, const float* __restrict__ gam,
+                             const float* __restrict__ bet, float eps, TO* __restrict__ u, float* __restrict__ mean,
+                             float* __restrict__ rstd, uint32_t drop_seed, uint32_t drop_thresh, float inv_keep) {
+  const long row = (long)blockIdx.x * 4 + (threadIdx.x >> 6);
+  const int lane = threadIdx.x & 63;
+  if (row >= rows) return;
+  const T* xr = x + row * C;
+  float v[LN_MAXC];
+  float s = 0.f;
+#pragma unroll
+  for (int q = 0; q < LN_MAXC; ++q) {
+    const int c = lane + 64 * q;
+    v[q] = c < C ? Elt<T>::ld(xr + c) : 0.f;
+    s += v[q];
+  }
+  const float mu = wave_sum(s) / C;
+  float ss = 0.f;
+#pragma unroll
+  for (int q = 0; q < LN_MAXC; ++q) {
+    const int c = lane + 64 * q;
+    const float d = c < C ? v[q] - mu : 0.f;
+    ss += d * d;
+  }
+  const float rs = rsqrtf(wave_sum(ss) / C + eps);
+#pragma unroll
+  for (int q = 0; q < LN_MAXC; ++q) {
+    const int c = lane + 64 * q;
+    if (c < C) {
+      float o = fmaxf((v[q] - mu) * rs * gam[c] + bet[c], 0.f);
+      if (drop_thresh) o *= tt_dropout_scale(drop_seed, (uint32_t)row, (uint32_t)c, drop_thresh, inv_keep);
+      Elt<TO>::st(u + row * C + c, o);
+    }
+  }
+  if (lane == 0) {
+    mean[row] = mu;
+    rstd[row] = rs;
+  }
+}
 
 template <typename T, typename TO>
 __global__ __launch_bounds__(256) void ln_relu_fwd_kernel(const T* __restrict__ x, long rows, int C,
@@ -15,41 +55,27 @@
                                                           TO* __restrict__ u, float* __restrict__ mean,
                                                           float* __restrict__ rstd, uint32_t drop_seed,
                                                           uint32_t drop_thresh, float inv_keep) {
-  const long row = (long)blockIdx.x * 4 + (threadIdx.x >> 6);
-  const int lane = threadIdx.x & 63;
-  if (row >= rows) return;
-  const T* xr = x + row * C;
-  float v[LN_MAXC];
-  float s = 0.f;
-#pragma unroll
-  for (int q = 0; q < LN_MAXC; ++q) {
-    const int c = lane + 64 * q;
-    v[q] = c < C ? Elt<T>::ld(xr + c) : 0.f;
-    s += v[q];
-  }
-  const float mu = wave_sum(s) / C;
-  float ss = 0.f;
-#pragma unroll
-  for (int q = 0; q < LN_MAXC; ++q) {
-    const int c = lane + 64 * q;
-    const float d = c < C ? v[q] - mu : 0.f;
-    ss += d * d;
-  }
-  const float rs = rsqrtf(wave_sum(ss) / C + eps);
-#pragma unroll
-  for (int q = 0; q < LN_MAXC; ++q) {
-    const int c = lane + 64 * q;
-    if (c < C) {
-      float o = fmaxf((v[q] - mu) * rs * gam[c] + bet[c], 0.f);
-      if (drop_thresh) o *= tt_dropout_scale(drop_seed, (uint32_t)row, (uint32_t)c, drop_thresh, inv_keep);
-      Elt<TO>::st(u + row * C + c, o);
-    }
-  }
-  if (lane == 0) {
-    mean[row] = mu;
-    rstd[row] = rs;
-  }
-}
+  ln_relu_fwd_rows<T, TO>(x, rows, C, gam, bet, eps, u, mean, rstd, drop_seed, drop_thresh, inv_keep);
+}
+
+template <typename T>
+struct LnFwdTowers {
+  const T* x[4];
+  const float* gam[4];
+  const float* bet[4];
+  T* u[4];
+  float* mean[4];
+  float* rstd[4];
+};
+template <typename T>
+__global__ __launch_bounds__(256) void ln_relu_fwd_towers(LnFwdTowers<T> a, long rows, int C, float eps) {
+  const int t = blockIdx.y;
+  ln_relu_fwd_rows<T, T>(a.x[t], rows, C, a.gam[t], a.bet[t], eps, a.u[t], a.mean[t], a.rstd[t], 0u, 0u, 1.f);
+}
+
+struct LnBwdTowerOffs {
+  long du[4], x[4], gam[4], bet[4], mean[4], rstd[4], dx[4], part[4], dout2[4];
+};
 
 template <typename T, int NP>
 __global__ __launch_bounds__(256) void ln_relu_bwd_kernel(const float* __restrict__ du, const T* __restrict__ x,
@@ -60,7 +86,13 @@
                                                           int rows_per_block, T* __restrict__ dx,
                                                           float* __restrict__ part, uint32_t drop_seed,
                                                           uint32_t drop_thresh, float inv_keep,
-                                                          const float* __restrict__ dout2, int C2) {
+                                                          const float* __restrict__ dout2, int C2, LnBwdTowerOffs tw) {
+  {
+    const int t = blockIdx.y;
+    du += tw.du[t]; x += tw.x[t]; gam += tw.gam[t]; bet += tw.bet[t]; mean += tw.mean[t]; rstd += tw.rstd[t];
+    dx += tw.dx[t]; part += tw.part[t];
+    if constexpr (NP == 4) dout2 += tw.dout2[t];
+  }
   __shared__ float red[4][NP][LN_MAXC * 64];
   const int wave = threadIdx.x >> 6, lane = threadIdx.x & 63;
   float pg[LN_MAXC], pb[LN_MAXC], pd[LN_MAXC], p2[LN_MAXC];
@@ -121,7 +153,25 @@
   }
 }
 
+struct HeadSumsArgs {
+  const float* part[4];
+  float* out[4][4];
+};
+__global__ __launch_bounds__(1024) void head_colsums_kernel(HeadSumsArgs a, long nblk, int C, int C2) {
+  __shared__ float red[16][64];
+  const int k = blockIdx.y, t = blockIdx.z;
+  const int cols = k == 3 ? C2 : C;
+  const int c = blockIdx.x * 64 + (threadIdx.x & 63);
+  const float s = colsum64(a.part[t] + (long)k * C + c, nblk, 4L * C, c < cols, red);
+  if (threadIdx.x < 64 && c < cols) a.out[t][k][c] = s;
+}
+
 constexpr int LN_ROWS_PER_BLOCK = 16;
+
+inline void head_bwd_splits(int B, int h, int* dw1, int* dw2) {
+  *dw1 = tt_gemm_pick_splits(2 * h, 4 * h, B, 1);
+  *dw2 = tt_gemm_pick_splits(h, 2 * h, B, 1);
+}
 
 inline long head_ws_layout(int dtype, int B, int h, long* o_dout, long* o_du, long* o_dp1, long* o_part,
                            long* o_sk) {
@@ -133,8 +183,8 @@
   *o_dp1 = off;  off = al(off + (long)B * 2 * h * esz);
   const long nblk = tt_ceil_div(B, LN_ROWS_PER_BLOCK);
   *o_part = off; off = al(off + nblk * 4L * 2 * h * 4);
-  const int s2 = tt_gemm_pick_splits(h, 2 * h, B, 1);
-  const int s1 = tt_gemm_pick_splits(2 * h, 4 * h, B, 1);
+  int s1, s2;
+  head_bwd_splits(B, h, &s1, &s2);
   const long sk = std::max(tt_gemm_ws_size(h, 2 * h, 1, s2), tt_gemm_ws_size(2 * h, 4 * h, 1, s1));
   *o_sk = off; off = al(off + sk * 4);
   return off;
@@ -159,7 +209,27 @@
   }
   TT_PROPAGATE(tt_gemm(dtype, dtype, 0, 0, B, 2 * h, 4 * h, &g1, ntower, 4 * h, 4 * h, 2 * h, 1.f, 0, 0, 0, 0,
                        0.f, 1, nullptr, stream));
-  for (int i = 0; i < ntower; ++i) {
+  const bool towers = ntower > 1 && tt::opt(tt::OPT_STEP_TAIL) != 0;
+  if (towers) {
+    dim3 grid(tt_ceil_div(B, 4), ntower);
+    if (dtype == TT_DT_BF16) {
+      LnFwdTowers<bf16_t> a{};
+      for (int i = 0; i < ntower; ++i) {
+        a.x[i] = (const bf16_t*)io[i].p1; a.gam[i] = io[i].ln_g; a.bet[i] = io[i].ln_b;
+        a.u[i] = (bf16_t*)io[i].u; a.mean[i] = io[i].mean; a.rstd[i] = io[i].rstd;
+      }
+      hipLaunchKernelGGL(ln_relu_fwd_towers<bf16_t>, grid, dim3(256), 0, st, a, (long)B, 2 * h, ln_eps);
+    } else {
+      LnFwdTowers<float> a{};
+      for (int i = 0; i < ntower; ++i) {
+        a.x[i] = (const float*)io[i].p1; a.gam[i] = io[i].ln_g; a.bet[i] = io[i].ln_b;
+        a.u[i] = (float*)io[i].u; a.mean[i] = io[i].mean; a.rstd[i] = io[i].rstd;
+      }
+      hipLaunchKernelGGL(ln_relu_fwd_towers<float>, grid, dim3(256), 0, st, a, (long)B, 2 * h, ln_eps);
+    }
+    TT_CHECK_LAUNCH("ln_relu_fwd_towers");
+  }
+  for (int i = 0; i < ntower && !towers; ++i) {
     dim3 grid(tt_ceil_div(B, 4));
     if (dtype == TT_DT_BF16)
       hipLaunchKernelGGL((ln_relu_fwd_kernel<bf16_t, bf16_t>), grid, dim3(256), 0, st, (const bf16_t*)io[i].p1,
@@ -176,12 +246,110 @@
   return 0;
 }
 
+namespace {
+
+template <typename T>
+int head_bwd_towers(int dtype, const tt_head_bwd_io* io, int nt, int B, int h, hipStream_t st) {
+  long o_dout, o_du, o_dp1, o_part, o_sk;
+  head_ws_layout(dtype, B, h, &o_dout, &o_du, &o_dp1, &o_part, &o_sk);
+  int sp1, sp2;
+  head_bwd_splits(B, h, &sp1, &sp2);
+  const int C = 2 * h;
+  const long nblk = tt_ceil_div(B, LN_ROWS_PER_BLOCK);
+  char* ws = static_cast<char*>(io[0].ws);
+  auto region = [&](long o, long o_next, int i) { return ws + nt * o + i * (o_next - o); };
+  float* sk = reinterpret_cast<float*>(ws + nt * o_sk);
+  bool direct = dtype == TT_DT_F32;
+  for (int i = 0; i < nt; ++i) direct = direct && (uintptr_t)io[i].dout % 16 == 0;
+  const void* dout_t[4];
+  float* du[4];
+  T* dp1[4];
+  float* part[4];
+  for (int i = 0; i < nt; ++i) {
+    du[i] = reinterpret_cast<float*>(region(o_du, o_dp1, i));
+    dp1[i] = reinterpret_cast<T*>(region(o_dp1, o_part, i));
+    part[i] = reinterpret_cast<float*>(region(o_part, o_sk, i));
+    dout_t[i] = io[i].dout;
+    if (!direct) {
+      void* d = region(o_dout, o_du, i);
+      TT_PROPAGATE(tt_cast(dtype, io[i].dout, (long)B * h, d, st));
+      dout_t[i] = d;
+    }
+  }
+  {
+    tt_gemm_batch g{};
+    for (int i = 0; i < nt; ++i) { g.a[i] = dout_t[i]; g.b[i] = io[i].u; g.c[i] = io[i].dw2; }
+    TT_PROPAGATE(tt::tt_gemm_sel(dtype, TT_DT_F32, 1, 1, h, C, B, &g, nt, 1, h, C, C, sp2, sk, st));
+  }
+  {
+    tt_gemm_batch g{};
+    for (int i = 0; i < nt; ++i) { g.a[i] = dout_t[i]; g.b[i] = io[i].w2; g.c[i] = du[i]; }
+    TT_PROPAGATE(tt::tt_gemm_sel(dtype, TT_DT_F32, 0, 1, B, C, h, &g, nt, 1, h, C, C, 1, nullptr, st));
+  }
+  {
+    LnBwdTowerOffs tw{};
+    HeadSumsArgs sa{};
+    const tt_head_bwd_io& q0 = io[0];
+    for (int i = 0; i < nt; ++i) {
+      const tt_head_bwd_io& q = io[i];
+      tw.du[i] = du[i] - du[0]; tw.x[i] = (const T*)q.p1 - (const T*)q0.p1; tw.gam[i] = q.ln_g - q0.ln_g;
+      tw.bet[i] = q.ln_b - q0.ln_b; tw.mean[i] = q.mean - q0.mean; tw.rstd[i] = q.rstd - q0.rstd;
+      tw.dx[i] = dp1[i] - dp1[0]; tw.part[i] = part[i] - part[0]; tw.dout2[i] = q.dout - q0.dout;
+      sa.part[i] = part[i];
+      sa.out[i][0] = q.dg; sa.out[i][1] = q.dbeta; sa.out[i][2] = q.db1; sa.out[i][3] = q.db2;
+    }
+    hipLaunchKernelGGL((ln_relu_bwd_kernel<T, 4>), dim3(nblk, nt), dim3(256), 0, st, du[0], (const T*)q0.p1, q0.ln_g,
+                       q0.ln_b, q0.mean, q0.rstd, (long)B, C, LN_ROWS_PER_BLOCK, dp1[0], part[0], 0u, 0u, 1.f, q0.dout,
+                       h, tw);
+    TT_CHECK_LAUNCH("ln_relu_bwd_kernel");
+    hipLaunchKernelGGL(head_colsums_kernel, dim3(tt_ceil_div(C, 64), 4, nt), dim3(1024), 0, st, sa, nblk, C, h);
+    TT_CHECK_LAUNCH("head_colsums_kernel");
+  }
+  {
+    tt_gemm_batch g{};
+    for (int i = 0; i < nt; ++i) { g.a[i] = dp1[i]; g.b[i] = io[i].x; g.c[i] = io[i].dw1; }
+    TT_PROPAGATE(tt::tt_gemm_sel(dtype, TT_DT_F32, 1, 1, C, 2 * C, B, &g, nt, 1, C, 2 * C, 2 * C, sp1, sk, st));
+  }
+  {
+    tt_gemm_batch g{};
+    for (int i = 0; i < nt; ++i) { g.a[i] = dp1[i]; g.b[i] = io[i].w1; g.c[i] = io[i].dx; }
+    TT_PROPAGATE(tt::tt_gemm_sel(dtype, TT_DT_F32, 0, 1, B, 2 * C, C, &g, nt, 1, C, 2 * C, 2 * C, 1, nullptr, st));
+  }
+  return 0;
+}
+
+bool head_bwd_batched(int dtype, const tt_head_bwd_io* io, int ntower, int B, int h) {
+  if (ntower < 2 || tt::opt(tt::OPT_STEP_TAIL) == 0 || !io[0].ws || (uintptr_t)io[0].ws % 256) return false;
+  const long sz = tt_proj_head_bwd_ws_size(dtype, B, h);
+  const uintptr_t esz = dtype == TT_DT_BF16 ? 2 : 4;
+  auto whole = [](const void* a, const void* b, uintptr_t e) { return ((uintptr_t)a - (uintptr_t)b) % e == 0; };
+  for (int i = 1; i < ntower; ++i) {
+    if (io[i].ws != static_cast<char*>(io[0].ws) + i * sz) return false;
+    const tt_head_bwd_io &q = io[i], &q0 = io[0];
+    if (!whole(q.p1, q0.p1, esz) || !whole(q.ln_g, q0.ln_g, 4) || !whole(q.ln_b, q0.ln_b, 4) ||
+        !whole(q.mean, q0.mean, 4) || !whole(q.rstd, q0.rstd, 4) || !whole(q.dout, q0.dout, 4))
+      return false;
+  }
+  return true;
+}
+
+}
+
+extern "C" int tt_proj_head_bwd_splits(int B, int h, int* dw1_splits, int* dw2_splits) {
+  TT_CHECK_ARG(B >= 1 && h >= 1 && dw1_splits && dw2_splits, "tt_proj_head_bwd_splits: B %d, h %d", B, h);
+  head_bwd_splits(B, h, dw1_splits, dw2_splits);
+  return 0;
+}
+
 extern "C" int tt_proj_head_bwd(int dtype, const tt_head_bwd_io* io, int ntower, int B, int h, float ln_eps,
                                 void* stream) {
   (void)ln_eps;
   TT_CHECK_ARG(ntower >= 1 && ntower <= 4, "tt_proj_head_bwd: ntower");
   TT_CHECK_ARG(2 * h <= 64 * LN_MAXC, "tt_proj_head_bwd: h=%d too large", h);
   hipStream_t st = (hipStream_t)stream;
+  if (head_bwd_batched(dtype, io, ntower, B, h))
+    return dtype == TT_DT_BF16 ? head_bwd_towers<bf16_t>(dtype, io, ntower, B, h, st)
+                               : head_bwd_towers<float>(dtype, io, ntower, B, h, st);
   long o_dout, o_du, o_dp1, o_part, o_sk;
   head_ws_layout(dtype, B, h, &o_dout, &o_du, &o_dp1, &o_part, &o_sk);
   const int C = 2 * h;
@@ -209,11 +377,11 @@
     if (dtype == TT_DT_BF16)
       hipLaunchKernelGGL((ln_relu_bwd_kernel<bf16_t, 4>), dim3(nblk), dim3(256), 0, st, du, (const bf16_t*)q.p1,
                          q.ln_g, q.ln_b, q.mean, q.rstd, (long)B, C, LN_ROWS_PER_BLOCK, (bf16_t*)dp1, part, 0u, 0u,
-                         1.f, q.dout, h);
+                         1.f, q.dout, h, LnBwdTowerOffs{});
     else
       hipLaunchKernelGGL((ln_relu_bwd_kernel<float, 4>), dim3(nblk), dim3(256), 0, st, du, (const float*)q.p1,
                          q.ln_g, q.ln_b, q.mean, q.rstd, (long)B, C, LN_ROWS_PER_BLOCK, (float*)dp1, part, 0u, 0u,
-                         1.f, q.dout, h);
+                         1.f, q.dout, h, LnBwdTowerOffs{});
     TT_CHECK_LAUNCH("ln_relu_bwd_kernel");
     TT_PROPAGATE(tt_colsum(part, nblk, C, 4L * C, q.dg, 0, stream));
     TT_PROPAGATE(tt_colsum(part + C, nblk, C, 4L * C, q.dbeta, 0, stream));
@@ -305,11 +473,11 @@
   if (dtype == TT_DT_BF16)
     hipLaunchKernelGGL((ln_relu_bwd_kernel<bf16_t, 3>), dim3(nblk), dim3(256), 0, st, io->dout,
                        (const bf16_t*)io->p1, io->ln_g, io->ln_b, io->mean, io->rstd, rows, C, LN_ROWS_PER_BLOCK,
-                       (bf16_t*)dp1, part, drop_seed, thresh, inv_keep, (const float*)nullptr, 0);
+                       (bf16_t*)dp1, part, drop_seed, thresh, inv_keep, (const float*)nullptr, 0, LnBwdTowerOffs{});
   else
     hipLaunchKernelGGL((ln_relu_bwd_kernel<float, 3>), dim3(nblk), dim3(256), 0, st, io->dout,
                        (const float*)io->p1, io->ln_g, io->ln_b, io->mean, io->rstd, rows, C, LN_ROWS_PER_BLOCK,
-                       (float*)dp1, part, drop_seed, thresh, inv_keep, (const float*)nullptr, 0);
+                       (float*)dp1, part, drop_seed, thresh, inv_keep, (const float*)nullptr, 0, LnBwdTowerOffs{});
   TT_CHECK_LAUNCH("ln_relu_bwd_kernel");
   TT_PROPAGATE(tt_colsum(part, nblk, C, 3L * C, io->dg, 0, stream));
   TT_PROPAGATE(tt_colsum(part + C, nblk, C, 3L * C, io->dbeta, 0, stream));
diff --git a/two_towers_amd/ops.py b/two_towers_amd/ops.py
--- a/two_towers_amd/ops.py
+++ b/two_towers_amd/ops.py
@@ -24,7 +24,7 @@
          bshift: Sequence[int] | None = None, alpha: float = 1.0, accumulate: bool = False,
          relu: bool = False, seq_t: int = 0, drop_seed: int = 0, drop_p: float = 0.0, drop_row0: int = 0,
          splits: int | None = None, a_hi: Sequence[torch.Tensor] | None = None, a_split: int = 0,
-         c_trans: bool = False):
+         c_trans: bool = False, c_rows: int | None = None):
     nb = len(a)
     assert 1 <= nb <= 4 and len(b) == nb and len(c) == nb
     bt = GemmBatch()
@@ -48,9 +48,13 @@
         ws = torch.empty(lib.tt_gemm_ws_size(m, n, nb, splits), dtype=torch.float32, device=c[0].device)
     else:
         splits = 1
-    call("tt_gemm_ct", dtype_code(dtype), dtype_code(out_dtype), int(a_kouter), int(b_kouter), m, n, k,
-         ctypes.byref(bt), nb, lda, ldb, ldc, alpha, int(accumulate), int(relu), seq_t, drop_seed & 0xFFFFFFFF,
-         drop_p, splits, ptr(ws), int(c_trans), stream_ptr(c[0].device))
+    args = (dtype_code(dtype), dtype_code(out_dtype), int(a_kouter), int(b_kouter), m, n, k, ctypes.byref(bt), nb, lda,
+            ldb, ldc, alpha, int(accumulate), int(relu), seq_t, drop_seed & 0xFFFFFFFF, drop_p, splits, ptr(ws),
+            int(c_trans))
+    if c_rows is not None:
+        call("tt_gemm_ct_rows", *args, c_rows, stream_ptr(c[0].device))
+    else:
+        call("tt_gemm_ct", *args, stream_ptr(c[0].device))
 
 
 def gemm_splits(m: int, n: int, k: int, nb: int, dtype: torch.dtype) -> int:
@@ -87,6 +91,15 @@
     call("tt_colsum", x.data_ptr(), rows, cols, ld, out.data_ptr(), int(accumulate), stream_ptr(out.device))
 
 
+def gru_bias_sums(parts: Sequence[torch.Tensor], nbr: int, H: int, dbih: torch.Tensor, dbhh: torch.Tensor):
+    n = len(parts)
+    for t in (*parts, dbih, dbhh):
+        assert t.dtype == torch.float32 and t.is_contiguous()
+    assert all(t.numel() == nbr * 4 * H for t in parts) and dbih.numel() == n * 3 * H == dbhh.numel()
+    ptrs = (ctypes.c_void_p * n)(*[t.data_ptr() for t in parts])
+    call("tt_gru_bias_sums", ptrs, n, nbr, H, dbih.data_ptr(), dbhh.data_ptr(), stream_ptr(dbih.device))
+
+
 def total(x: torch.Tensor, scale: float, out: torch.Tensor):
     call("tt_sum", x.data_ptr(), x.numel(), scale, out.data_ptr(), stream_ptr(out.device))
 
diff --git a/two_towers_amd/towers.py b/two_towers_amd/towers.py
--- a/two_towers_amd/towers.py
+++ b/two_towers_amd/towers.py
@@ -248,6 +248,10 @@
     if not _lib.get_option("gru_yprev"):
         return False
     return bool(_lib.load().tt_gru_yprev_supported(dtype_code(cfg.dtype), 2 * cfg.ntowers, B, T, H, 6 * H, 2 * H))
+
+
+def _step_tail() -> bool:
+    return bool(_lib.get_option("step_tail"))
 
 
 def _gru_layer_fwd(cfg, xs, K, ldx, packs, layer, B, T, seeds, want_x1, ws, yprev=False, want_final=False):
@@ -425,6 +429,12 @@
                        kernel=kname):
         call("tt_gru_bwd_yprev" if yprev else "tt_gru_bwd", dtype_code(dt), recs, 2 * n, B, T, H, 2 * H, 8 * H, ldf,
              stream_ptr(dev))
+    if _step_tail():
+        sb = _alloc((2, n * 2, 3 * H), torch.float32, dev)
+        ops.gru_bias_sums([part[i] for i in range(2 * n)], nbr, H, sb[0], sb[1])
+        dbih = [[sb[0, ti * 2 + d] for d in range(2)] for ti in range(n)]
+        dbhh = [[sb[1, ti * 2 + d] for d in range(2)] for ti in range(n)]
+        return dG, dbih, dbhh
     sums = _alloc((n * 2, 4 * H), torch.float32, dev)
     for i in range(2 * n):
         ops.colsum(part[i], nbr, 4 * H, 4 * H, sums[i])
@@ -450,7 +460,10 @@
 def _weight_grads(cfg, B, T, dG, Xin, K, ldx, Y, kr=None, yprev=False):
     n, H, dt, dev = cfg.ntowers, cfg.H, cfg.dtype, dG[0].device
     BT = B * T
-    dWih = [[_alloc((3 * H, K), torch.float32, dev) for _ in range(2)] for _ in range(n)]
+    kr = K if kr is None else kr
+    tall = _WGRAD_T and dt == torch.bfloat16 and 0 < K % 256 <= 128
+    narrow = kr < K and tall and _step_tail() and ops.gemm_splits(K, 3 * H, BT, 2 * n, dt) > 1
+    dWih = [[_alloc((3 * H, kr if narrow else K), torch.float32, dev) for _ in range(2)] for _ in range(n)]
     dWhh = [[_alloc((3 * H, H), torch.float32, dev) for _ in range(2)] for _ in range(n)]
     a_ih, b_ih, c_ih, a_hh, a_hi, b_hh, c_hh, sh = [], [], [], [], [], [], [], []
     for ti in range(n):
@@ -464,11 +477,13 @@
             c_hh.append(dWhh[ti][d])
             sh.append(-1 if d == 0 else 1)
     esz = 2 if dt == torch.bfloat16 else 4
-    kr = K if kr is None else kr
     with timing.region("wgrad_ih", 1, 2.0 * 3 * H * kr * BT * 2 * n,
                        float(n * (esz * BT * (6 * H + kr) + 2 * 3 * H * kr * 4))):
-        if _WGRAD_T and dt == torch.bfloat16 and 0 < K % 256 <= 128:
-            if ops.gemm_splits(K, 3 * H, BT, len(c_ih), dt) > 1:
+        if tall:
+            if narrow:
+                ops.gemm(b_ih, a_ih, c_ih, m=K, n=3 * H, k=BT, lda=ldx, ldb=8 * H, ldc=kr, a_kouter=True,
+                         b_kouter=True, dtype=dt, out_dtype=torch.float32, c_trans=True, c_rows=kr)
+            elif ops.gemm_splits(K, 3 * H, BT, len(c_ih), dt) > 1:
                 ops.gemm(b_ih, a_ih, c_ih, m=K, n=3 * H, k=BT, lda=ldx, ldb=8 * H, ldc=K, a_kouter=True,
                          b_kouter=True, dtype=dt, out_dtype=torch.float32, c_trans=True)
             else:
@@ -577,8 +592,12 @@
                 dhcat.append(torch.zeros(B, 2 * H, dtype=torch.float32, device=dev) if g is None
                              else g.float().contiguous())
         ws = None
+        one_call = n > 1 and _step_tail()
         if cfg.head == "proj2":
-            ws = _alloc((lib.tt_proj_head_bwd_ws_size(dtype_code(HEAD_DT), B, h),), torch.uint8, dev)
+            wsz = lib.tt_proj_head_bwd_ws_size(dtype_code(HEAD_DT), B, h)
+            ws = _alloc((wsz * n if one_call else wsz,), torch.uint8, dev)
+            ios = (HeadBwdIO * n)()
+        gs = []
         for ti in range(n if cfg.head == "proj2" else 0):
             g = gouts[ti]
             g = torch.zeros(B, h, dtype=torch.float32, device=dev) if g is None else g.float().contiguous()
@@ -590,17 +609,21 @@
             dbeta = _alloc((2 * h,), torch.float32, dev)
             dw2 = _alloc(pk.w2.shape, torch.float32, dev)
             db2 = _alloc((h,), torch.float32, dev)
-            io = HeadBwdIO()
+            io = ios[ti]
             io.w1, io.ln_g, io.ln_b, io.w2 = pk.w1.data_ptr(), pk.ln_g.data_ptr(), pk.ln_b.data_ptr(), pk.w2.data_ptr()
             io.x, io.p1, io.mean, io.rstd, io.u = (hcat[ti].data_ptr(), p1s[ti].data_ptr(), means[ti].data_ptr(),
                                                    rstds[ti].data_ptr(), us[ti].data_ptr())
+            gs.append(g)
             io.dout, io.dx = g.data_ptr(), dx.data_ptr()
             io.dw1, io.db1, io.dg, io.dbeta, io.dw2, io.db2 = (dw1.data_ptr(), db1.data_ptr(), dg.data_ptr(),
                                                                dbeta.data_ptr(), dw2.data_ptr(), db2.data_ptr())
-            io.ws = ws.data_ptr()
-            call("tt_proj_head_bwd", dtype_code(HEAD_DT), ctypes.byref(io), 1, B, h, LN_EPS, st)
+            io.ws = ws.data_ptr() + (ti * wsz if one_call else 0)
+            if not one_call:
+                call("tt_proj_head_bwd", dtype_code(HEAD_DT), ctypes.byref(io), 1, B, h, LN_EPS, st)
             head_grads[ti] = [dw1, db1, dg, dbeta, dw2, db2]
             dhcat.append(dx)
+        if cfg.head == "proj2" and one_call:
+            call("tt_proj_head_bwd", dtype_code(HEAD_DT), ios, n, B, h, LN_EPS, st)
         dG1, dbih1, dbhh1 = _gru_layer_bwd(cfg, 1, B, T, S1, Y1, None, dhcat, packs, yprev=yp1)
         Xl1 = X1 if X1 is not None else Y0
         red = dist.OverlapReducer(ctx.group[0]) if ctx.group is not None else None
@@ -663,7 +686,7 @@
     for ti in range(len(gl)):
         for d, sfx in enumerate(("", "_reverse")):
             w = dWih[ti][d]
-            if layer == 0 and Ep != E:
+            if layer == 0 and w.shape[1] != E:
                 w = w[:, :E].contiguous()
             gl[ti][f"weight_ih_l{layer}{sfx}"] = w
             gl[ti][f"weight_hh_l{layer}{sfx}"] = dWhh[ti][d]
```

Result: no change. 163,200 pairs/s, median of 6 (+0.7%).
